# pranoyr/attention-models

Hardware: AMD Instinct MI355X
Metric: ViTVQGAN 256px train-step images/sec (higher is better)
Workload: dtype f32; 1 GPU; BASELINE.json configs[2]: ViTVQGAN dim=256 patch=8 img=256 depth=6+6 h=8 d=64 mlp=2048 (SwiGLU), codebook 8192x32; GAN train step (D phase + G phase, gradient penalty, per_loss_weight=0), Adam, clip 1.0; global_batch=32, batch_per_gpu=32, parallelism=dp1

## Files before the change

attention-models_amd/amk/lib.py:

```python
import ctypes
import os
import re

_HERE = os.path.dirname(os.path.abspath(__file__))
LIB_PATH = os.environ.get("AMK_LIB") or os.path.join(_HERE, "libamk.so")
HEADER_PATH = os.path.normpath(os.path.join(_HERE, "..", "..", "include", "amk.h"))

AMK_OK = 0

_c = ctypes
_P = _c.c_void_p
_I = _c.c_int
_L = _c.c_int64
_F = _c.c_float



class GemmDesc(_c.Structure):
    _fields_ = [("op", _c.c_int32), ("epilogue", _c.c_int32), ("m", _L),
                ("n", _c.c_int32), ("k", _c.c_int32), ("split", _c.c_int32), ("reserved", _c.c_int32),
                ("a", _P), ("a2", _P), ("w", _P), ("w2", _P), ("c", _P), ("c2", _P),
                ("lda", _L), ("lda2", _L), ("ldw", _L), ("ldw2", _L), ("ldc", _L), ("ldc2", _L),
                ("bias", _P), ("bias2", _P), ("resid", _P), ("ldr", _L),
                ("ln_mean", _P), ("ln_rstd", _P), ("ln_gamma", _P), ("ln_beta", _P),
                ("ab", _P), ("ldab", _L), ("gate", _P), ("ldg", _L), ("dbias", _P)]


GEMM_NT, GEMM_NN, GEMM_TN = 0, 1, 2
EPI_BIAS, EPI_RESID, EPI_SWIGLU, EPI_SWIGLU_BWD = 0, 1, 2, 3

SIGNATURES = {
    "amk_version": (_I, []),
    "amk_arch": (_c.c_char_p, []),
    "amk_last_error": (_c.c_char_p, []),
    "amk_attn_fwd": (_I, [_P] * 7 + [_I] * 5 + [_L] * 12 + [_F, _P]),
    "amk_attn_scores_bytes": (_L, [_I, _I, _I, _I]),
    "amk_attn_fwd_keep": (_I, [_P] * 8 + [_I] * 5 + [_L] * 12 + [_F, _P]),
    "amk_attn_fwd_x6_ws_bytes": (_L, [_I, _I, _I]),
    "amk_attn_fwd_x6": (_I, [_P] * 8 + [_I] * 5 + [_L] * 12 + [_F, _P]),
    "amk_attn_bwd_ws_floats": (_L, [_I, _I, _I, _I, _I]),
    "amk_attn_bwd": (_I, [_P] * 12 + [_I] * 5 + [_L] * 24 + [_F, _I, _P]),
    "amk_attn_bwd_kept": (_I, [_P] * 13 + [_I] * 5 + [_L] * 24 + [_F, _I, _P]),
    "amk_vq_num_partials": (_L, [_L]),
    "amk_vq_lookup_fwd": (_I, [_P, _P, _L, _I, _I, _I] + [_P] * 9 + [_P]),
    "amk_vq_lookup_bwd": (_I, [_P] * 7 + [_F, _L, _I, _I, _P, _P, _P]),
    "amk_vq_lookup_bwd_rows": (_I, [_P] * 7 + [_F, _L, _I, _I, _P, _P, _P]),
    "amk_vq_padded_codes": (_I, [_I, _I]),
    "amk_vq_gather": (_I, [_P, _P, _L, _I, _I, _P, _P, _P]),
    "amk_agent_num_chunks": (_I, [_I]),
    "amk_agent_ws_floats": (_L, [_I, _I, _I, _I, _I]),
    "amk_agent_num_chunks_dh": (_I, [_I, _I]),
    "amk_agent_ws_floats_dh": (_L, [_I, _I, _I, _I, _I, _I]),
    "amk_agent_attn_fwd": (_I, [_P] * 10 + [_I] * 5 + [_L] * 12 + [_F, _P]),
    "amk_agent_attn_bwd": (_I, [_P] * 14 + [_I] * 5 + [_L] * 21 + [_F, _P]),
    "amk_agent_conv_grad_reduce": (_I, [_P, _P, _L, _I, _P, _P, _P]),
    "amk_rowsum_num_partials": (_I, [_L]),
    "amk_add_layernorm_fwd": (_I, [_P, _P, _P, _P, _L, _I, _F, _P, _P, _P, _P, _P]),
    "amk_add_layernorm_bwd": (_I, [_P, _P, _P, _P, _P, _P, _L, _I, _P, _P, _P]),
    "amk_colsum": (_I, [_P, _L, _I, _P, _P]),
    "amk_swiglu_fwd": (_I, [_P, _L, _I, _P, _P]),
    "amk_swiglu_bwd": (_I, [_P, _P, _L, _I, _P, _P]),
    "amk_geglu_fwd": (_I, [_P, _L, _I, _P, _P]),
    "amk_geglu_bwd": (_I, [_P, _P, _L, _I, _P, _P]),
    "amk_opt_num_partials": (_I, []),
    "amk_sumsq_partials": (_I, [_P, _L, _P, _P]),
    "amk_adam_flat_step": (_I, [_P] * 4 + [_L, _P, _P, _P, _I] + [_F] * 6 + [_I, _P, _P]),
    "amk_adam_flat_step_shadow": (_I, [_P] * 4 + [_L, _P, _P, _P, _I] + [_F] * 6 + [_I, _P, _P, _P]),
    "amk_gemm_x6_planes_bytes": (_L, [_I, _I]),
    "amk_gemm_x6_split": (_I, [_P, _L, _I, _I, _P, _P]),
    "amk_gemm_x6_nt": (_I, [_P, _L, _P, _P, _P, _L, _I, _I, _I, _P]),
    "amk_gemm_f32_ws_bytes": (_L, [_c.POINTER(GemmDesc)]),
    "amk_gemm_f32": (_I, [_c.POINTER(GemmDesc), _P, _L, _P]),
    "amk_row_stats": (_I, [_P, _L, _I, _F, _P, _P, _P]),
    "amk_attn_bf16_fwd": (_I, [_P] * 7 + [_I] * 5 + [_L] * 12 + [_F, _P]),
    "amk_attn_bf16_bwd_ws_floats": (_L, [_I, _I, _I, _I]),
    "amk_attn_bf16_bwd": (_I, [_P] * 12 + [_I] * 5 + [_L] * 24 + [_F, _P]),
    "amk_swiglu_bf16_fwd": (_I, [_P, _L, _I, _P, _P]),
    "amk_swiglu_bf16_bwd": (_I, [_P, _P, _L, _I, _P, _P]),
    "amk_add_layernorm_mixed_fwd": (_I, [_P, _I, _P, _P, _P, _L, _I, _F, _P, _P, _P, _P, _P]),
    "amk_add_layernorm_mixed_bwd": (_I, [_P, _I, _P, _P, _P, _P, _P, _L, _I, _P, _P, _P, _P]),
    "amk_gemm_bf16": (_I, [_I, _I, _P, _L, _P, _L, _P, _P, _L, _P, _L, _L, _I, _I, _P]),
    "amk_gemm_bf16_swiglu_bwd": (_I, [_P, _L, _P, _L, _P, _L, _P, _L, _L, _I, _I, _P]),
    "amk_gemm_tn_bf16_ws_bytes": (_L, [_L, _I, _I]),
    "amk_gemm_tn_bf16": (_I, [_P, _L, _P, _L, _P, _L, _P, _L, _I, _I, _P, _L, _P]),
    "amk_sample_step": (_I, [_P, _P, _F, _P, _c.c_uint64, _c.c_uint64, _F, _L, _I, _I, _P, _F, _P, _P, _P]),
    "amk_moe_route_ws_ints": (_L, [_L, _I, _I]),
    "amk_moe_route": (_I, [_P, _L, _I, _I] + [_P] * 8),
    "amk_grouped_gemm_nt": (_I, [_P, _L, _I, _P, _P, _P, _P, _L, _I, _I, _I, _P, _P]),
    "amk_grouped_gemm_nn": (_I, [_P, _L, _I, _P, _P, _P, _P, _L, _I, _I, _I, _P, _P]),
    "amk_grouped_gemm_nt_acc": (_I, [_P, _L, _I, _P, _P, _P, _P, _L, _I, _I, _I, _P, _I, _P]),
    "amk_grouped_gemm_nn_acc": (_I, [_P, _L, _I, _P, _P, _P, _P, _L, _I, _I, _I, _P, _I, _P]),
    "amk_grouped_gemm_wgrad": (_I, [_P, _L, _I, _P, _L, _I, _P, _P, _P, _L, _I, _I, _I, _P, _P, _P]),
    "amk_moe_combine": (_I, [_P, _P, _P, _L, _I, _I, _I, _P, _P]),
    "amk_moe_expert_sums": (_I, [_P, _L, _I, _P, _P, _L, _I, _I, _I, _P, _P]),
    "amk_moe_topk": (_I, [_P, _L, _I, _I, _P, _P, _P]),
    "amk_moe_route_distinct": (_I, [_P, _L, _I, _I, _P, _P, _P, _P]),
    "amk_moe_combine_rows": (_I, [_P, _P, _P, _L, _I, _I, _I, _I, _I, _P, _P]),
    "amk_moe_gate_grad_rows": (_I, [_P, _P, _P, _P, _L, _I, _I, _I, _I, _I, _P, _P]),
    "amk_moe_gate_grad": (_I, [_P, _P, _P, _P, _L, _I, _I, _I, _I, _P, _P]),
    "amk_bnact_ws_floats": (_L, [_I, _I, _L]),
    "amk_bnact_fwd": (_I, [_P, _P, _P, _I, _I, _L, _F, _F, _F] + [_P] * 7),
    "amk_bnact_bwd": (_I, [_P] * 6 + [_I, _I, _L, _F] + [_P] * 6),
    "amk_bnact_bwd_bwd": (_I, [_P] * 10 + [_I, _I, _L, _F] + [_P] * 5),
}

_lib = None


def declared_symbols(header_path=HEADER_PATH):
    text = open(header_path).read()
    text = re.sub(r"/\*.*?\*/", "", text, flags=re.S)
    return sorted(set(re.findall(r"\b(amk_[a-z0-9_]+)\s*\(", text)))


def load():
    global _lib
    if _lib is not None:
        return _lib
    if not os.path.exists(LIB_PATH):
        raise RuntimeError(
            f"{LIB_PATH} is missing: build it with `python -c 'import __graft_entry__ as g; g.build()'` "
            "(hipcc --offload-arch=gfx950). amk has no CPU or eager fallback."
        )
    lib = ctypes.CDLL(LIB_PATH)
    for name, (res, args) in SIGNATURES.items():
        fn = getattr(lib, name)
        fn.restype = res
        fn.argtypes = args
    arch = lib.amk_arch().decode()
    if arch != "gfx950":
        raise RuntimeError(f"libamk.so was built for {arch}, expected gfx950")
    _lib = lib
    return lib


def check(rc, what):
    if rc != AMK_OK:
        msg = load().amk_last_error().decode()
        raise RuntimeError(f"{what} failed with code {rc}: {msg}")
```

attention-models_amd/amk/models/discriminator.py:

```python
import contextlib

import torch
import torch.nn as nn
import torch.nn.functional as F
from torch.nn.grad import conv2d_input, conv2d_weight

from .. import ops

_INPUT_GRAD_ONLY = False


@contextlib.contextmanager
def input_grad_only():
    global _INPUT_GRAD_ONLY
    old, _INPUT_GRAD_ONLY = _INPUT_GRAD_ONLY, True
    try:
        yield
    finally:
        _INPUT_GRAD_ONLY = old


def input_grad_only_active():
    return _INPUT_GRAD_ONLY


class _ConvDataGrad(torch.autograd.Function):

    @staticmethod
    def forward(ctx, gy, weight, x_shape, stride, padding):
        ctx.save_for_backward(gy, weight)
        ctx.cfg = (stride, padding)
        return conv2d_input(x_shape, weight, gy, stride=stride, padding=padding)

    @staticmethod
    def backward(ctx, ggx):
        gy, weight = ctx.saved_tensors
        stride, padding = ctx.cfg
        ggx = ggx.contiguous()
        ggy = F.conv2d(ggx, weight, None, stride, padding) if ctx.needs_input_grad[0] else None
        gw = conv2d_weight(ggx, weight.shape, gy, stride=stride, padding=padding) if ctx.needs_input_grad[1] else None
        return ggy, gw, None, None, None


class _Conv(torch.autograd.Function):
    @staticmethod
    def forward(ctx, x, weight, bias, stride, padding):
        ctx.save_for_backward(x, weight)
        ctx.cfg = (stride, padding, bias is not None)
        return F.conv2d(x, weight, bias, stride, padding)

    @staticmethod
    def backward(ctx, gy):
        x, weight = ctx.saved_tensors
        stride, padding, has_bias = ctx.cfg
        gy = gy.contiguous()
        gx = _ConvDataGrad.apply(gy, weight, x.shape, stride, padding) if ctx.needs_input_grad[0] else None
        gw = gb = None
        if not _INPUT_GRAD_ONLY:
            if ctx.needs_input_grad[1]:
                gw = conv2d_weight(x, weight.shape, gy, stride=stride, padding=padding)
            if has_bias and ctx.needs_input_grad[2]:
                gb = gy.sum((0, 2, 3))
        return gx, gw, gb, None, None


class Conv2d(nn.Conv2d):

    def forward(self, x):
        if self.groups != 1 or self.dilation != (1, 1) or self.padding_mode != "zeros" or isinstance(self.padding, str):
            return super().forward(x)
        if torch.is_autocast_enabled():
            if self.in_channels < 8 and x.is_cuda:
                with torch.autocast("cuda", enabled=False):
                    return _Conv.apply(x.float(), self.weight, self.bias, self.stride, self.padding)
            return super().forward(x)
        return _Conv.apply(x, self.weight, self.bias, self.stride, self.padding)


class NLayerDiscriminator(nn.Module):
    def __init__(self, input_nc=3, ndf=64, n_layers=3):
        super().__init__()
        widths = [ndf * min(2 ** i, 8) for i in range(n_layers + 1)]
        layers = [Conv2d(input_nc, widths[0], 4, stride=2, padding=1), nn.LeakyReLU(0.2, True)]
        for i in range(1, n_layers + 1):
            stride = 2 if i < n_layers else 1
            layers += [
                Conv2d(widths[i - 1], widths[i], 4, stride=stride, padding=1, bias=False),
                nn.BatchNorm2d(widths[i]),
                nn.LeakyReLU(0.2, True),
            ]
        layers.append(Conv2d(widths[-1], 1, 4, stride=1, padding=1))
        self.model = nn.Sequential(*layers)

    def forward(self, x):
        if ops.discr_norm_mode() != "amk":
            return self.model(x)
        layers = list(self.model)
        i = 0
        while i < len(layers):
            m = layers[i]
            nxt = layers[i + 1] if i + 1 < len(layers) else None
            if isinstance(m, nn.BatchNorm2d) and isinstance(nxt, nn.LeakyReLU) and ops.bn_leaky_relu_ok(m, x):
                x = ops.bn_leaky_relu(x, m, nxt.negative_slope)
                i += 2
            else:
                x = m(x)
                i += 1
        return x
```

attention-models_amd/amk/ops.py:

```python
import ctypes
import os
import weakref

import torch
from torch.autograd.function import once_differentiable

from . import lib as _lib

_NULL = ctypes.c_void_p(0)


def _ptr(t):
    return ctypes.c_void_p(t.data_ptr()) if t is not None else _NULL


def _stream():
    return ctypes.c_void_p(torch.cuda.current_stream().cuda_stream)


KERNEL_EVENTS = None


class _timed:

    def __init__(self, name):
        self.name = name

    def __enter__(self):
        if KERNEL_EVENTS is not None:
            self.a = torch.cuda.Event(enable_timing=True)
            self.b = torch.cuda.Event(enable_timing=True)
            self.a.record()
        return self

    def __exit__(self, *exc):
        if KERNEL_EVENTS is not None:
            self.b.record()
            KERNEL_EVENTS.setdefault(self.name, []).append((self.a, self.b))
        return False


def kernel_event_summary(events):
    out = {}
    for name, pairs in events.items():
        ms = [a.elapsed_time(b) for a, b in pairs]
        out[name] = (len(ms), sum(ms) / len(ms))
    return out


def _require_device(*tensors):
    for t in tensors:
        if t is None:
            continue
        if not t.is_cuda:
            raise RuntimeError(
                "amk ops run only on MI355X (HIP) tensors; got a CPU tensor. There is no CPU fallback."
            )
        if t.is_floating_point() and t.dtype != torch.float32:
            raise RuntimeError(f"amk kernels compute in fp32; got {t.dtype}")


def _strides4(t):
    return (t.stride(0), t.stride(2), t.stride(1))


def _kernel_view_ok(t):
    return (
        t.stride(3) == 1
        and t.data_ptr() % 16 == 0
        and all(s % 4 == 0 for s in (t.stride(0), t.stride(1), t.stride(2)))
    )


def _as_kernel_view(t):
    if _kernel_view_ok(t):
        return t
    B, H, T, D = t.shape
    return t.permute(0, 2, 1, 3).contiguous().permute(0, 2, 1, 3)


def _new_bthd(B, H, T, D, like):
    return torch.empty((B, T, H, D), device=like.device, dtype=torch.float32).permute(0, 2, 1, 3)


def _mask_u8(mask, shape, what):
    if mask is None:
        return None
    m = mask
    while m.dim() > len(shape) and m.shape[0] == 1:
        m = m[0]
    if m.dim() != len(shape):
        raise RuntimeError(f"{what} must have {len(shape)} dims (got shape {tuple(mask.shape)})")
    m = m.expand(*shape)
    return m.to(torch.uint8).contiguous()


ATTENTION_FORWARD = os.environ.get("AMK_ATTENTION_FORWARD", "f32")

ATTENTION_KEEP_SCORES = os.environ.get("AMK_ATTN_KEEP_SCORES", "1") == "1"
ATTENTION_KEEP_SCORES_MAX_BYTES = 8 << 30
ATTENTION_KEEP_SCORES_BUDGET_BYTES = int(os.environ.get("AMK_ATTN_KEEP_BUDGET", "0")) or None
_kept_scores_bytes = [0]


def _keep_budget(device):
    if ATTENTION_KEEP_SCORES_BUDGET_BYTES is not None:
        return ATTENTION_KEEP_SCORES_BUDGET_BYTES
    return torch.cuda.get_device_properties(device).total_memory // 4


def _release_kept(nbytes):
    _kept_scores_bytes[0] -= nbytes
ATTENTION_BACKWARD_KEYS = int(os.environ.get("AMK_ATTN_BWD_KEYS", "0"))


def _attn_forward(q, k, v, key_mask, causal_mask, scale, keep_scores=False):
    B, H, I, D = q.shape
    J = k.shape[2]
    _require_device(q, k, v, key_mask, causal_mask)
    if k.shape != (B, H, J, D) or v.shape != (B, H, J, D):
        raise RuntimeError(f"attention shapes disagree: q {tuple(q.shape)} k {tuple(k.shape)} v {tuple(v.shape)}")
    q, k, v = _as_kernel_view(q), _as_kernel_view(k), _as_kernel_view(v)
    o = _new_bthd(B, H, I, D, q)
    stats = torch.empty((B, H, I, 2), device=q.device, dtype=torch.float32)
    L = _lib.load()
    x6 = ATTENTION_FORWARD == "bf16x6" and D == 64
    ws = torch.empty((L.amk_attn_fwd_x6_ws_bytes(B, H, J),), device=q.device, dtype=torch.uint8) if x6 else None
    scores = None
    det = DETERMINISTIC_ATTENTION_BACKWARD or torch.are_deterministic_algorithms_enabled()
    keepable = D == 64 or (D == 128 and key_mask is None and causal_mask is None and not det)
    if (keep_scores and keepable and not x6 and ATTENTION_KEEP_SCORES
            and not ATTENTION_BACKWARD_TWO_KERNEL):
        nbytes = L.amk_attn_scores_bytes(B, H, I, J)
        if nbytes <= ATTENTION_KEEP_SCORES_MAX_BYTES and _kept_scores_bytes[0] + nbytes <= _keep_budget(q.device):
            scores = torch.empty((nbytes // 4,), device=q.device, dtype=torch.float32)
            _kept_scores_bytes[0] += nbytes
            weakref.finalize(scores.untyped_storage(), _release_kept, nbytes)
    with _timed("attn_fwd_keep_kernel" if scores is not None else "attn_fwd_kernel"):
        if scores is not None:
            rc = L.amk_attn_fwd_keep(
                _ptr(q), _ptr(k), _ptr(v), _ptr(o), _ptr(stats), _ptr(scores), _ptr(key_mask), _ptr(causal_mask),
                B, H, I, J, D, *_strides4(q), *_strides4(k), *_strides4(v), *_strides4(o),
                float(scale), _stream(),
            )
        elif x6:
            rc = L.amk_attn_fwd_x6(
                _ptr(q), _ptr(k), _ptr(v), _ptr(o), _ptr(stats), _ptr(ws), _ptr(key_mask), _ptr(causal_mask),
                B, H, I, J, D, *_strides4(q), *_strides4(k), *_strides4(v), *_strides4(o),
                float(scale), _stream(),
            )
        else:
            rc = L.amk_attn_fwd(
                _ptr(q), _ptr(k), _ptr(v), _ptr(o), _ptr(stats), _ptr(key_mask), _ptr(causal_mask),
                B, H, I, J, D, *_strides4(q), *_strides4(k), *_strides4(v), *_strides4(o),
                float(scale), _stream(),
            )
    _lib.check(rc, "amk_attn_fwd")
    return q, k, v, o, stats, scores


DETERMINISTIC_ATTENTION_BACKWARD = os.environ.get("AMK_DETERMINISTIC", "0") == "1"
ATTENTION_BACKWARD_TWO_KERNEL = False


def _attn_backward(q, k, v, o, stats, d_o, dq, dk, dv, key_mask, causal_mask, scale, stages=None, delta=None,
                   scores=None):
    if stages is None:
        det = DETERMINISTIC_ATTENTION_BACKWARD or torch.are_deterministic_algorithms_enabled()
        stages = 7 if ATTENTION_BACKWARD_TWO_KERNEL else (73 if det else 9)
    if stages & 8 and not stages & 48:
        stages |= {128: 16, 256: 32}.get(ATTENTION_BACKWARD_KEYS, 0)
    if not stages & 8:
        scores = None
    B, H, I, D = q.shape
    if D != 64 and stages & 64:
        scores = None
    J = k.shape[2]
    d_o = _as_kernel_view(d_o)
    L = _lib.load()
    need = L.amk_attn_bwd_ws_floats(B, H, I, J, int(stages))
    if delta is None or delta.numel() < need:
        delta = torch.empty((need,), device=q.device, dtype=torch.float32)

    def call(st):
        fn, head = (L.amk_attn_bwd_kept, (_ptr(scores),)) if scores is not None and st & 8 else (L.amk_attn_bwd, ())
        rc = fn(
            *head, _ptr(q), _ptr(k), _ptr(v), _ptr(o), _ptr(stats), _ptr(d_o),
            _ptr(dq), _ptr(dk), _ptr(dv), _ptr(delta), _ptr(key_mask), _ptr(causal_mask),
            B, H, I, J, D,
            *_strides4(q), *_strides4(k), *_strides4(v), *_strides4(o), *_strides4(d_o),
            *_strides4(dq), *_strides4(dk), *_strides4(dv),
            float(scale), int(st), _stream(),
        )
        _lib.check(rc, "amk_attn_bwd")

    if KERNEL_EVENTS is not None and (stages & 1) and (stages & ~1):
        call(1)
        name = "attn_bwd_dkdv+dq" if not stages & 8 else ("attn_bwd_fused_kernel(kept scores)" if scores is not None
                                                            else "attn_bwd_fused_kernel")
        with _timed(name):
            call(stages & ~1)
    else:
        call(stages)


_amp_fwd = torch.amp.custom_fwd(device_type="cuda", cast_inputs=torch.float32)
_amp_bwd = torch.amp.custom_bwd(device_type="cuda")


class _AttnCore(torch.autograd.Function):

    @staticmethod
    @_amp_fwd
    def forward(ctx, q, k, v, key_mask, causal_mask, scale):
        need = any(ctx.needs_input_grad[:3])
        q, k, v, o, stats, scores = _attn_forward(q, k, v, key_mask, causal_mask, scale, keep_scores=need)
        ctx.save_for_backward(q, k, v, o, stats, key_mask, causal_mask, scores)
        ctx.scale = scale
        return o

    @staticmethod
    @once_differentiable
    @_amp_bwd
    def backward(ctx, d_o):
        q, k, v, o, stats, key_mask, causal_mask, scores = ctx.saved_tensors
        B, H, I, D = q.shape
        J = k.shape[2]
        dq = _new_bthd(B, H, I, D, q)
        dk = _new_bthd(B, H, J, D, q)
        dv = _new_bthd(B, H, J, D, q)
        _attn_backward(q, k, v, o, stats, d_o, dq, dk, dv, key_mask, causal_mask, ctx.scale, scores=scores)
        return dq, dk, dv, None, None, None


class _AttnFusedKV(torch.autograd.Function):

    @staticmethod
    @_amp_fwd
    def forward(ctx, q2, kv2, key_mask, causal_mask, H, D, scale):
        B, I, _ = q2.shape
        J = kv2.shape[1]
        q2 = q2.contiguous()
        kv2 = kv2.contiguous()
        q = q2.view(B, I, H, D).permute(0, 2, 1, 3)
        kv = kv2.view(B, J, 2, H, D)
        k = kv[:, :, 0].permute(0, 2, 1, 3)
        v = kv[:, :, 1].permute(0, 2, 1, 3)
        need = any(ctx.needs_input_grad[:2])
        q, k, v, o, stats, scores = _attn_forward(q, k, v, key_mask, causal_mask, scale, keep_scores=need)
        ctx.save_for_backward(q, k, v, o, stats, key_mask, causal_mask, scores)
        ctx.scale = scale
        return o.permute(0, 2, 1, 3).reshape(B, I, H * D)

    @staticmethod
    @once_differentiable
    @_amp_bwd
    def backward(ctx, d_o2):
        q, k, v, o, stats, key_mask, causal_mask, scores = ctx.saved_tensors
        B, H, I, D = q.shape
        J = k.shape[2]
        d_o = d_o2.contiguous().view(B, I, H, D).permute(0, 2, 1, 3)
        dq2 = torch.empty((B, I, H * D), device=q.device, dtype=torch.float32)
        dkv2 = torch.empty((B, J, 2 * H * D), device=q.device, dtype=torch.float32)
        dq = dq2.view(B, I, H, D).permute(0, 2, 1, 3)
        dkv = dkv2.view(B, J, 2, H, D)
        dk = dkv[:, :, 0].permute(0, 2, 1, 3)
        dv = dkv[:, :, 1].permute(0, 2, 1, 3)
        _attn_backward(q, k, v, o, stats, d_o, dq, dk, dv, key_mask, causal_mask, ctx.scale, scores=scores)
        return dq2, dkv2, None, None, None, None, None


ATTENTION_BF16 = os.environ.get("AMK_ATTENTION_BF16", "1") == "1"


class _AttnFusedKVBF16(torch.autograd.Function):

    @staticmethod
    @torch.amp.custom_fwd(device_type="cuda")
    def forward(ctx, q2, kv2, H, scale, key_mask=None, causal_mask=None):
        B, I, _ = q2.shape
        J = kv2.shape[1]
        D = 64
        q2 = q2.contiguous()
        kv2 = kv2.contiguous()
        o2 = torch.empty((B, I, H * D), device=q2.device, dtype=torch.bfloat16)
        stats = torch.empty((B, H, I, 2), device=q2.device, dtype=torch.float32)
        L = _lib.load()
        qs, kvs = (I * H * D, H * D, D), (J * 2 * H * D, 2 * H * D, D)
        masked = key_mask is not None or causal_mask is not None
        with _timed("attn_bf16_fwd_kernel<masked>" if masked else "attn_bf16_fwd_kernel"):
            rc = L.amk_attn_bf16_fwd(_ptr(q2), _ptr(kv2), ctypes.c_void_p(kv2.data_ptr() + 2 * H * D), _ptr(o2), _ptr(stats),
                                     _ptr(key_mask), _ptr(causal_mask),
                                     B, H, I, J, D, *qs, *kvs, *kvs, *qs, float(scale), _stream())
        _lib.check(rc, "amk_attn_bf16_fwd")
        ctx.save_for_backward(q2, kv2, o2, stats, key_mask, causal_mask)
        ctx.cfg = (H, scale)
        return o2

    @staticmethod
    @once_differentiable
    @_amp_bwd
    def backward(ctx, d_o2):
        q2, kv2, o2, stats, key_mask, causal_mask = ctx.saved_tensors
        H, scale = ctx.cfg
        B, I, _ = q2.shape
        J = kv2.shape[1]
        D = 64
        d_o2 = d_o2.to(torch.bfloat16).contiguous()
        dq2 = torch.empty_like(q2)
        dkv2 = torch.empty_like(kv2)
        L = _lib.load()
        ws = torch.empty((L.amk_attn_bf16_bwd_ws_floats(B, H, I, J),), device=q2.device, dtype=torch.float32)
        qs, kvs = (I * H * D, H * D, D), (J * 2 * H * D, 2 * H * D, D)
        masked = key_mask is not None or causal_mask is not None
        with _timed("attn_bf16_bwd_kernel<masked>" if masked else "attn_bf16_bwd_kernel"):
            rc = L.amk_attn_bf16_bwd(_ptr(q2), _ptr(kv2), ctypes.c_void_p(kv2.data_ptr() + 2 * H * D), _ptr(o2), _ptr(stats), _ptr(d_o2),
                                     _ptr(dq2), _ptr(dkv2), ctypes.c_void_p(dkv2.data_ptr() + 2 * H * D), _ptr(ws),
                                     _ptr(key_mask), _ptr(causal_mask),
                                     B, H, I, J, D, *qs, *kvs, *kvs, *qs, *qs, *qs, *kvs, *kvs, float(scale), _stream())
        _lib.check(rc, "amk_attn_bf16_bwd")
        return dq2, dkv2, None, None, None, None


def attention(q, k, v, scale, key_mask=None, causal_mask=None):
    B, H, I, D = q.shape
    J = k.shape[2]
    km = _mask_u8(key_mask, (B, J), "context_mask")
    cm = _mask_u8(causal_mask, (I, J), "causal_mask")
    return _AttnCore.apply(q, k, v, km, cm, scale)


def attention_fused_kv(q2, kv2, num_heads, dim_head, scale, key_mask=None, causal_mask=None):
    B, I, _ = q2.shape
    J = kv2.shape[1]
    km = _mask_u8(key_mask, (B, J), "context_mask")
    cm = _mask_u8(causal_mask, (I, J), "causal_mask")
    if ATTENTION_BF16 and q2.dtype == torch.bfloat16 and kv2.dtype == torch.bfloat16 and q2.is_cuda and dim_head == 64:
        return _AttnFusedKVBF16.apply(q2, kv2, num_heads, scale, km, cm)
    return _AttnFusedKV.apply(q2, kv2, km, cm, num_heads, dim_head, scale)


CHECK_INDICES = os.environ.get("AMK_CHECK_INDICES", "1") == "1"


def vq_nsplit(N, K):
    row_blocks = (N + 127) // 128
    nsplit = 1
    while row_blocks * nsplit < 4096 and K // (2 * nsplit) >= 1024:
        nsplit *= 2
    return nsplit


class _VQLookup(torch.autograd.Function):
    @staticmethod
    @_amp_fwd
    def forward(ctx, z, codebook, beta):
        _require_device(z, codebook)
        C = z.shape[-1]
        K = codebook.shape[0]
        zf = z.contiguous().view(-1, C)
        cb = codebook.contiguous()
        N = zf.shape[0]
        dev = z.device
        L = _lib.load()
        nsplit = vq_nsplit(N, K)
        f32 = dict(device=dev, dtype=torch.float32)
        kp = L.amk_vq_padded_codes(K, nsplit)
        en = torch.empty((kp, C), **f32)
        ee = torch.empty((kp,), **f32)
        pmin = torch.empty((N, nsplit), **f32)
        pidx = torch.empty((N, nsplit), device=dev, dtype=torch.int32)
        idx = torch.empty((N,), device=dev, dtype=torch.int64)
        out = torch.empty((N, C), **f32)
        zq = torch.empty((N, C), **f32)
        zn = torch.empty((N, C), **f32)
        partial = torch.empty((L.amk_vq_num_partials(N),), **f32)
        with _timed("vq_lookup_fwd"):
            rc = L.amk_vq_lookup_fwd(
                _ptr(zf), _ptr(cb), N, K, C, nsplit, _ptr(en), _ptr(ee), _ptr(pmin), _ptr(pidx),
                _ptr(idx), _ptr(out), _ptr(zq), _ptr(zn), _ptr(partial), _stream(),
            )
        _lib.check(rc, "amk_vq_lookup_fwd")
        mean_sq = partial.sum() / float(N * C)
        loss = beta * mean_sq + mean_sq
        ctx.save_for_backward(zf, cb, zn, zq, idx)
        ctx.beta = beta
        ctx.z_shape = z.shape
        idx_v = idx.view(z.shape[:-1])
        ctx.mark_non_differentiable(idx_v)
        return out.view(z.shape), idx_v, loss

    @staticmethod
    @once_differentiable
    @_amp_bwd
    def backward(ctx, g_out, _g_idx, g_loss):
        zf, cb, zn, zq, idx = ctx.saved_tensors
        N, C = zf.shape
        K = cb.shape[0]
        if g_out is None:
            g_out = torch.zeros_like(zf)
        if g_loss is None:
            g_loss = torch.zeros((), device=zf.device, dtype=torch.float32)
        g_out = g_out.contiguous().view(N, C)
        g_loss = g_loss.contiguous().to(torch.float32)
        dz = torch.empty_like(zf)
        L = _lib.load()
        if DETERMINISTIC_ATTENTION_BACKWARD or torch.are_deterministic_algorithms_enabled():
            ge = torch.empty_like(zf)
            rc = L.amk_vq_lookup_bwd_rows(
                _ptr(zf), _ptr(cb), _ptr(zn), _ptr(zq), _ptr(idx), _ptr(g_out), _ptr(g_loss),
                float(ctx.beta), N, K, C, _ptr(dz), _ptr(ge), _stream(),
            )
            _lib.check(rc, "amk_vq_lookup_bwd_rows")
            flat_idx = idx.clamp(0, K - 1)
            srt, order = torch.sort(flat_idx, stable=True)
            bounds = torch.searchsorted(srt, torch.arange(K + 1, device=srt.device, dtype=srt.dtype))
            dcb = torch.segment_reduce(ge.index_select(0, order), "sum", offsets=bounds, axis=0, unsafe=True)
            return dz.view(ctx.z_shape), dcb, None
        dcb = torch.empty_like(cb)
        rc = L.amk_vq_lookup_bwd(
            _ptr(zf), _ptr(cb), _ptr(zn), _ptr(zq), _ptr(idx), _ptr(g_out), _ptr(g_loss),
            float(ctx.beta), N, K, C, _ptr(dz), _ptr(dcb), _stream(),
        )
        _lib.check(rc, "amk_vq_lookup_bwd")
        return dz.view(ctx.z_shape), dcb, None


def vq_lookup(z, codebook, beta):
    return _VQLookup.apply(z, codebook, beta)


def vq_gather(indices, codebook):
    _require_device(indices, codebook)
    K, C = codebook.shape
    flat = indices.contiguous().view(-1).to(torch.int64)
    N = flat.shape[0]
    out = torch.empty((N, C), device=codebook.device, dtype=torch.float32)
    bad = torch.zeros((1,), device=codebook.device, dtype=torch.int32)
    L = _lib.load()
    rc = L.amk_vq_gather(_ptr(flat), _ptr(codebook.detach().contiguous()), N, K, C, _ptr(out), _ptr(bad), _stream())
    _lib.check(rc, "amk_vq_gather")
    if CHECK_INDICES and int(bad.item()):
        raise IndexError(f"vq_gather: {int(bad.item())} of {N} indices are outside the codebook [0, {K})")
    return out.view(*indices.shape, C)


_SAMPLE_CALLS = 0


def sample_step(logits, ids, mask=None, null_logits=None, cfg_scale=3.0, tau=1.0, p=0.9, gumbel=None, seed=None,
                unmasked_score=None, generator=None):
    import math

    global _SAMPLE_CALLS
    _require_device(logits, null_logits, gumbel)
    B, T, V = logits.shape
    logits = logits.contiguous()
    null_logits = null_logits.contiguous() if null_logits is not None else None
    gumbel = gumbel.contiguous() if gumbel is not None else None
    if ids.dtype != torch.int64 or not ids.is_contiguous():
        raise RuntimeError("sample_step: ids must be a contiguous int64 tensor (updated in place)")
    m8 = mask.to(torch.uint8).contiguous() if mask is not None else None
    scores = torch.empty((B, T), device=logits.device, dtype=torch.float32)
    if seed is not None:
        _SAMPLE_CALLS += 1
        offset = _SAMPLE_CALLS
    else:
        gen = generator if generator is not None else torch.cuda.default_generators[logits.device.index or 0]
        seed = int(gen.initial_seed()) & ((1 << 63) - 1)
        offset = int(gen.get_offset())
        gen.set_offset(offset + 4 * ((B * T * V + 3) // 4))
    L = _lib.load()
    rc = L.amk_sample_step(_ptr(logits), _ptr(null_logits), float(cfg_scale), _ptr(gumbel), seed, offset, float(tau),
                           B * T, V, math.ceil((1 - p) * V), _ptr(m8), -1.0 if unmasked_score is None else float(unmasked_score),
                           _ptr(ids), _ptr(scores), _stream())
    _lib.check(rc, "amk_sample_step")
    return scores


def _i32(n, dev):
    return torch.empty((n,), device=dev, dtype=torch.int32)


def moe_route(logits2, k):
    _require_device(logits2)
    U, E = logits2.shape
    dev = logits2.device
    ids = torch.empty((U, k), device=dev, dtype=torch.int64)
    gate = torch.empty((U, k), device=dev, dtype=torch.float32)
    L = _lib.load()
    counts, rank = _i32(E, dev), _i32(U * k, dev)
    blockhist = _i32(L.amk_moe_route_ws_ints(U, E, k), dev)
    offsets, perm = _i32(E + 1, dev), _i32(U * k, dev)
    rc = L.amk_moe_route(_ptr(logits2.contiguous()), U, E, k, _ptr(ids), _ptr(gate), _ptr(counts), _ptr(rank),
                         _ptr(blockhist), _ptr(offsets), _ptr(perm), _stream())
    _lib.check(rc, "amk_moe_route")
    return dict(ids=ids, gate=gate, offsets=offsets, perm=perm)


MOE_SUM_IN_GEMM = os.environ.get("AMK_MOE_SUM_IN_GEMM", "0") == "1"


MOE_DENSE_Z = os.environ.get("AMK_MOE_DENSE_Z", "1") != "0"


def _moe_dense_z(width, depth, fan, E):
    return MOE_DENSE_Z and E <= 2 * fan and width >= 256 and width >= 4 * depth and depth % 4 == 0


def _expert_sums(a2, a_div, ids, scale, G, fan, E, d):
    Z = torch.empty((G, E * d), device=a2.device, dtype=torch.float32)
    with _timed(f"moe_expert_sums G{G} fan{fan} E{E} d{d}"):
        rc = _lib.load().amk_moe_expert_sums(_ptr(a2), a2.stride(0), a_div, _ptr(ids), scale, G, fan, E, d, _ptr(Z), _stream())
    _lib.check(rc, "amk_moe_expert_sums")
    return Z


def _moe_sum_in_gemm(width, depth, fan):
    if not MOE_SUM_IN_GEMM or DETERMINISTIC_ATTENTION_BACKWARD or torch.are_deterministic_algorithms_enabled():
        return False
    return fan >= 4 and width >= 128 and depth % 32 == 0


class _RoutedLinear(torch.autograd.Function):

    @staticmethod
    @_amp_fwd
    def forward(ctx, x2, logits2, W, bias, k, x_div, weighted, outer):
        _require_device(x2, logits2, W, bias)
        x2 = x2.contiguous()
        W = W.contiguous()
        U, E = logits2.shape
        N, Kd = W.shape[1], W.shape[2]
        P = U * k
        dev = x2.device
        if x2.shape != (P // x_div, Kd) or U % outer:
            raise RuntimeError(f"routed linear shapes disagree: x {tuple(x2.shape)} U {U} k {k} x_div {x_div} W {tuple(W.shape)}")
        with _timed(f"moe_route U{U} E{E} k{k}"):
            r = moe_route(logits2.detach(), k)
        L = _lib.load()
        G = U // outer
        if not weighted and bias is None and _moe_dense_z(N, Kd, outer * k, E):
            Y = None
            Z = _expert_sums(x2, x_div, r["ids"], _NULL, G, outer * k, E, Kd)
            with _timed(f"dense_z_gemm M{G} N{N} K{E * Kd}"):
                out = Z @ W.permute(0, 2, 1).reshape(E * Kd, N)
        elif not weighted and _moe_sum_in_gemm(N, Kd, outer * k):
            Y = None
            out = torch.zeros((G, N), device=dev, dtype=torch.float32)
            with _timed(f"grouped_nt_acc P{P} N{N} K{Kd}"):
                rc = L.amk_grouped_gemm_nt_acc(_ptr(x2), Kd, x_div, _ptr(W), _ptr(bias), _ptr(r["offsets"]), _ptr(r["perm"]),
                                               P, E, N, Kd, _ptr(out), outer * k, _stream())
            _lib.check(rc, "amk_grouped_gemm_nt_acc")
        else:
            Y = torch.empty((P, N), device=dev, dtype=torch.float32)
            with _timed(f"grouped_nt P{P} N{N} K{Kd}"):
                rc = L.amk_grouped_gemm_nt(_ptr(x2), Kd, x_div, _ptr(W), _ptr(bias), _ptr(r["offsets"]), _ptr(r["perm"]),
                                           P, E, N, Kd, _ptr(Y), _stream())
            _lib.check(rc, "amk_grouped_gemm_nt")
            out = torch.empty((G, N), device=dev, dtype=torch.float32)
            with _timed(f"moe_combine G{G} N{N} x{outer * k}"):
                rc = L.amk_moe_combine(_ptr(Y), _ptr(r["ids"]), _ptr(r["gate"]) if weighted else _NULL, G, outer, k, N,
                                       _ptr(out), _stream())
            _lib.check(rc, "amk_moe_combine")
        ctx.save_for_backward(x2, W, Y, r["ids"], r["gate"], r["offsets"], r["perm"])
        ctx.cfg = (k, x_div, weighted, outer, E, bias is not None)
        ctx.mark_non_differentiable(r["ids"])
        ctx.set_materialize_grads(False)
        return out, r["ids"]

    @staticmethod
    @once_differentiable
    @_amp_bwd
    def backward(ctx, d_out, _d_ids):
        if d_out is None:
            return (None,) * 8
        x2, W, Y, ids, gate, offsets, perm = ctx.saved_tensors
        k, x_div, weighted, outer, E, has_bias = ctx.cfg
        N, Kd = W.shape[1], W.shape[2]
        P = ids.numel()
        U = P // k
        dev = x2.device
        d_out = d_out.contiguous()
        g_div = outer * k
        scale = _ptr(gate) if weighted else _NULL
        L = _lib.load()
        dlogits = None
        if weighted:
            dlogits = torch.empty((U, E), device=dev, dtype=torch.float32)
            rc = L.amk_moe_gate_grad(_ptr(d_out), _ptr(Y), _ptr(ids), _ptr(gate), P, k, E, N, g_div, _ptr(dlogits), _stream())
            _lib.check(rc, "amk_moe_gate_grad")
        if not ctx.needs_input_grad[0]:
            dx = None
        elif _moe_dense_z(Kd, N, x_div, E):
            Z = _expert_sums(d_out, g_div, ids, scale, x2.shape[0], x_div, E, N)
            with _timed(f"dense_z_gemm M{x2.shape[0]} N{Kd} K{E * N}"):
                dx = Z @ W.view(E * N, Kd)
        elif _moe_sum_in_gemm(Kd, N, x_div):
            dx = torch.zeros_like(x2)
            with _timed(f"grouped_nn_acc P{P} N{N} K{Kd}"):
                rc = L.amk_grouped_gemm_nn_acc(_ptr(d_out), N, g_div, _ptr(W), scale, _ptr(offsets), _ptr(perm), P, E, N, Kd,
                                               _ptr(dx), x_div, _stream())
            _lib.check(rc, "amk_grouped_gemm_nn_acc")
        else:
            dxp = torch.empty((P, Kd), device=dev, dtype=torch.float32)
            with _timed(f"grouped_nn P{P} N{N} K{Kd}"):
                rc = L.amk_grouped_gemm_nn(_ptr(d_out), N, g_div, _ptr(W), scale, _ptr(offsets), _ptr(perm), P, E, N, Kd,
                                           _ptr(dxp), _stream())
            _lib.check(rc, "amk_grouped_gemm_nn")
            dx = torch.empty_like(x2)
            rc = L.amk_moe_combine(_ptr(dxp), _ptr(ids), _NULL, x2.shape[0], x_div // k, k, Kd, _ptr(dx), _stream())
            _lib.check(rc, "amk_moe_combine")
        dW = torch.empty_like(W)
        db = torch.empty((E, N), device=dev, dtype=torch.float32) if has_bias else None
        with _timed(f"grouped_wgrad P{P} N{N} K{Kd}"):
            rc = L.amk_grouped_gemm_wgrad(_ptr(d_out), N, g_div, _ptr(x2), Kd, x_div, scale, _ptr(offsets), _ptr(perm),
                                          P, E, N, Kd, _ptr(dW), _ptr(db), _stream())
        _lib.check(rc, "amk_grouped_gemm_wgrad")
        return dx, dlogits, dW, db, None, None, None, None


def routed_linear(x2, logits2, W, bias, k, x_div, weighted=True, outer=1):
    return _RoutedLinear.apply(x2, logits2, W, bias, k, x_div, weighted, outer)


def _topk(logits2, k):
    U, E = logits2.shape
    ids = torch.empty((U, k), device=logits2.device, dtype=torch.int64)
    gate = torch.empty((U, k), device=logits2.device, dtype=torch.float32)
    _lib.check(_lib.load().amk_moe_topk(_ptr(logits2.contiguous()), U, E, k, _ptr(ids), _ptr(gate), _stream()), "amk_moe_topk")
    return ids, gate


def _route_distinct(ids, G, fan, E):
    dev = ids.device
    mask = torch.empty((G,), device=dev, dtype=torch.int64)
    offsets, perm = _i32(E + 1, dev), _i32(G * min(fan, E), dev)
    _lib.check(_lib.load().amk_moe_route_distinct(_ptr(ids), G, fan, E, _ptr(mask), _ptr(offsets), _ptr(perm), _stream()),
               "amk_moe_route_distinct")
    return offsets, perm


def distinct_experts_ok(dim, d, fan, E, *weights):
    return E <= 64 and _moe_dense_z(dim, d, fan, E) and dim % 4 == 0 and all(w.is_cuda for w in weights)


class _SharedRowExperts(torch.autograd.Function):

    @staticmethod
    @_amp_fwd
    def forward(ctx, x2, logits2, W, k, H):
        _require_device(x2, logits2, W)
        x2, W = x2.contiguous(), W.contiguous()
        U, E = logits2.shape
        N, Kd = W.shape[1], W.shape[2]
        G, fan = U // H, H * k
        if x2.shape != (G, Kd) or U % H:
            raise RuntimeError(f"shared-row experts: shapes disagree: x {tuple(x2.shape)} U {U} H {H} W {tuple(W.shape)}")
        L = _lib.load()
        with _timed(f"moe_topk U{U} E{E} k{k} + distinct lists"):
            ids, gate = _topk(logits2.detach(), k)
            offsets, perm = _route_distinct(ids, G, fan, E)
        V = torch.empty((G * E, N), device=x2.device, dtype=torch.float32)
        with _timed(f"grouped_nt P{U * k} N{N} K{Kd} (distinct rows)"):
            _lib.check(L.amk_grouped_gemm_nt(_ptr(x2), Kd, E, _ptr(W), _NULL, _ptr(offsets), _ptr(perm), G * E, E, N, Kd, _ptr(V),
                                             _stream()), "amk_grouped_gemm_nt")
        out = torch.empty((U, N), device=x2.device, dtype=torch.float32)
        _lib.check(L.amk_moe_combine_rows(_ptr(V), _ptr(ids), _ptr(gate), U, 1, k, N, fan, E, _ptr(out), _stream()),
                   "amk_moe_combine_rows")
        ctx.save_for_backward(x2, W, V, ids, gate, offsets, perm)
        ctx.cfg = (k, H)
        ctx.mark_non_differentiable(ids)
        ctx.set_materialize_grads(False)
        return out, ids

    @staticmethod
    @once_differentiable
    @_amp_bwd
    def backward(ctx, d_out, _d_ids):
        if d_out is None:
            return (None,) * 5
        x2, W, V, ids, gate, offsets, perm = ctx.saved_tensors
        k, H = ctx.cfg
        E, N, Kd = W.shape
        G, fan = x2.shape[0], H * k
        U = G * H
        d_out = d_out.contiguous()
        L = _lib.load()
        dlogits = torch.empty((U, E), device=x2.device, dtype=torch.float32)
        _lib.check(L.amk_moe_gate_grad_rows(_ptr(d_out), _ptr(V), _ptr(ids), _ptr(gate), U * k, k, E, N, k, fan, _ptr(dlogits),
                                            _stream()), "amk_moe_gate_grad_rows")
        Z = _expert_sums(d_out, k, ids, _ptr(gate), G, fan, E, N)
        dx = None
        if ctx.needs_input_grad[0]:
            with _timed(f"dense_z_gemm M{G} N{Kd} K{E * N}"):
                dx = Z @ W.view(E * N, Kd)
        dW = torch.empty_like(W)
        with _timed(f"grouped_wgrad P{U * k} N{N} K{Kd} (distinct rows)"):
            _lib.check(L.amk_grouped_gemm_wgrad(_ptr(Z), N, 1, _ptr(x2), Kd, E, _NULL, _ptr(offsets), _ptr(perm), G * E, E, N, Kd,
                                                _ptr(dW), _NULL, _stream()), "amk_grouped_gemm_wgrad")
        return dx, dlogits, dW, None, None


class _SummedExperts(torch.autograd.Function):

    @staticmethod
    @_amp_fwd
    def forward(ctx, a2, logits2, W, k, H):
        _require_device(a2, logits2, W)
        a2, W = a2.contiguous(), W.contiguous()
        U, E = logits2.shape
        N, Kd = W.shape[1], W.shape[2]
        G, fan = U // H, H * k
        if a2.shape != (U, Kd) or U % H:
            raise RuntimeError(f"summed experts: shapes disagree: a {tuple(a2.shape)} U {U} H {H} W {tuple(W.shape)}")
        with _timed(f"moe_topk U{U} E{E} k{k}"):
            ids, _gate = _topk(logits2.detach(), k)
        Z = _expert_sums(a2, k, ids, _NULL, G, fan, E, Kd)
        with _timed(f"dense_z_gemm M{G} N{N} K{E * Kd}"):
            out = Z @ W.permute(0, 2, 1).reshape(E * Kd, N)
        ctx.save_for_backward(W, Z, ids)
        ctx.cfg = (k, H)
        ctx.mark_non_differentiable(ids)
        ctx.set_materialize_grads(False)
        return out, ids

    @staticmethod
    @once_differentiable
    @_amp_bwd
    def backward(ctx, d_out, _d_ids):
        if d_out is None:
            return (None,) * 5
        W, Z, ids = ctx.saved_tensors
        k, H = ctx.cfg
        E, N, Kd = W.shape
        G, fan = Z.shape[0], H * k
        U = G * H
        d_out = d_out.contiguous()
        L = _lib.load()
        offsets, perm = _route_distinct(ids, G, fan, E)
        da = None
        if ctx.needs_input_grad[0]:
            D = torch.empty((G * E, Kd), device=W.device, dtype=torch.float32)
            with _timed(f"grouped_nn P{U * k} N{N} K{Kd} (distinct rows)"):
                _lib.check(L.amk_grouped_gemm_nn(_ptr(d_out), N, E, _ptr(W), _NULL, _ptr(offsets), _ptr(perm), G * E, E, N, Kd, _ptr(D),
                                                 _stream()), "amk_grouped_gemm_nn")
            da = torch.empty((U, Kd), device=W.device, dtype=torch.float32)
            _lib.check(L.amk_moe_combine_rows(_ptr(D), _ptr(ids), _NULL, U, 1, k, Kd, fan, E, _ptr(da), _stream()),
                       "amk_moe_combine_rows")
        dW = torch.empty_like(W)
        with _timed(f"grouped_wgrad P{U * k} N{N} K{Kd} (distinct rows)"):
            _lib.check(L.amk_grouped_gemm_wgrad(_ptr(d_out), N, E, _ptr(Z), Kd, 1, _NULL, _ptr(offsets), _ptr(perm), G * E, E, N, Kd,
                                                _ptr(dW), _NULL, _stream()), "amk_grouped_gemm_wgrad")
        return da, None, dW, None, None


def shared_row_experts(x2, logits2, W, k, H):
    return _SharedRowExperts.apply(x2, logits2, W, k, H)


def summed_experts(a2, logits2, W, k, H):
    return _SummedExperts.apply(a2, logits2, W, k, H)


class _AgentAttn(torch.autograd.Function):

    @staticmethod
    @_amp_fwd
    def forward(ctx, qkv2, conv_w, conv_b, H, D, P, scale):
        _require_device(qkv2, conv_w, conv_b)
        B, T, _ = qkv2.shape
        qkv2 = qkv2.contiguous()
        qkv = qkv2.view(B, T, 3, H, D)
        q, k, v = (qkv[:, :, j].permute(0, 2, 1, 3) for j in range(3))
        dev = qkv2.device
        o = _new_bthd(B, H, T, D, qkv2)
        agents = torch.empty((B, H, P, D), device=dev, dtype=torch.float32)
        vagent = torch.empty_like(agents)
        stats1 = torch.empty((B, H, P, 2), device=dev, dtype=torch.float32)
        cw, cb = conv_w.contiguous(), conv_b.contiguous()
        L = _lib.load()
        ws = torch.empty((max(L.amk_agent_ws_floats_dh(B, H, T, P, D, 0), 1),), device=dev, dtype=torch.float32)
        rc = L.amk_agent_attn_fwd(_ptr(q), _ptr(k), _ptr(v), _ptr(cw), _ptr(cb), _ptr(o), _ptr(agents), _ptr(vagent),
                                  _ptr(stats1), _ptr(ws), B, H, T, D, P, *_strides4(q), *_strides4(k), *_strides4(v), *_strides4(o),
                                  float(scale), _stream())
        _lib.check(rc, "amk_agent_attn_fwd")
        ctx.save_for_backward(qkv2, cw, agents, vagent, stats1)
        ctx.cfg = (H, D, P, scale)
        return o.permute(0, 2, 1, 3).reshape(B, T, H * D)

    @staticmethod
    @once_differentiable
    @_amp_bwd
    def backward(ctx, d_o2):
        qkv2, cw, agents, vagent, stats1 = ctx.saved_tensors
        H, D, P, scale = ctx.cfg
        B, T, _ = qkv2.shape
        dev = qkv2.device
        qkv = qkv2.view(B, T, 3, H, D)
        q, k, v = (qkv[:, :, j].permute(0, 2, 1, 3) for j in range(3))
        d_o = d_o2.contiguous().view(B, T, H, D).permute(0, 2, 1, 3)
        dqkv2 = torch.empty_like(qkv2)
        dqkv = dqkv2.view(B, T, 3, H, D)
        dq, dk, dv = (dqkv[:, :, j].permute(0, 2, 1, 3) for j in range(3))
        L = _lib.load()
        cells = B * H * L.amk_agent_num_chunks_dh(T, D)
        ws = torch.empty((max(L.amk_agent_ws_floats_dh(B, H, T, P, D, 1), 1),), device=dev, dtype=torch.float32)
        dw_part = torch.empty((cells, 9, D), device=dev, dtype=torch.float32)
        db_part = torch.empty((cells, D), device=dev, dtype=torch.float32)
        rc = L.amk_agent_attn_bwd(_ptr(q), _ptr(k), _ptr(v), _ptr(cw), _ptr(d_o), _ptr(agents), _ptr(vagent), _ptr(stats1),
                                  _ptr(dq), _ptr(dk), _ptr(dv), _ptr(ws), _ptr(dw_part), _ptr(db_part),
                                  B, H, T, D, P, *_strides4(q), *_strides4(k), *_strides4(v), *_strides4(d_o),
                                  *_strides4(dq), *_strides4(dk), *_strides4(dv), float(scale), _stream())
        _lib.check(rc, "amk_agent_attn_bwd")
        dconv_w = torch.empty((D, 1, 3, 3), device=dev, dtype=torch.float32)
        dconv_b = torch.empty((D,), device=dev, dtype=torch.float32)
        _lib.check(L.amk_agent_conv_grad_reduce(_ptr(dw_part), _ptr(db_part), cells, D, _ptr(dconv_w), _ptr(dconv_b), _stream()),
                   "amk_agent_conv_grad_reduce")
        return dqkv2, dconv_w, dconv_b, None, None, None, None


def agent_attention(qkv2, conv_w, conv_b, num_heads, dim_head, pool, scale):
    return _AgentAttn.apply(qkv2, conv_w, conv_b, num_heads, dim_head, pool, scale)


class _SwiGLU(torch.autograd.Function):
    FWD, BWD = "amk_swiglu_fwd", "amk_swiglu_bwd"

    @classmethod
    def forward(cls, ctx, ab):
        _require_device(ab)
        H = ab.shape[-1] // 2
        ab2 = ab.contiguous().view(-1, 2 * H)
        M = ab2.shape[0]
        out = torch.empty((M, H), device=ab.device, dtype=torch.float32)
        L = _lib.load()
        _lib.check(getattr(L, cls.FWD)(_ptr(ab2), M, H, _ptr(out), _stream()), cls.FWD)
        ctx.save_for_backward(ab2)
        ctx.shape = ab.shape
        return out.view(*ab.shape[:-1], H)

    @classmethod
    def backward(cls, ctx, d_out):
        (ab2,) = ctx.saved_tensors
        M, H2 = ab2.shape
        d_out = d_out.contiguous().view(M, H2 // 2)
        d_ab = torch.empty_like(ab2)
        L = _lib.load()
        _lib.check(getattr(L, cls.BWD)(_ptr(ab2), _ptr(d_out), M, H2 // 2, _ptr(d_ab), _stream()), cls.BWD)
        return d_ab.view(ctx.shape)


class _GEGLU(_SwiGLU):
    FWD, BWD = "amk_geglu_fwd", "amk_geglu_bwd"


def _f32_outside_autocast(fn, x):
    if torch.is_autocast_enabled():
        with torch.autocast("cuda", enabled=False):
            return fn(x.float())
    return fn(x)


class _SwiGLUBF16(torch.autograd.Function):

    @staticmethod
    def forward(ctx, ab):
        H = ab.shape[-1] // 2
        ab2 = ab.contiguous().view(-1, 2 * H)
        M = ab2.shape[0]
        out = torch.empty((M, H), device=ab.device, dtype=torch.bfloat16)
        _lib.check(_lib.load().amk_swiglu_bf16_fwd(_ptr(ab2), M, H, _ptr(out), _stream()), "amk_swiglu_bf16_fwd")
        ctx.save_for_backward(ab2)
        ctx.shape = ab.shape
        return out.view(*ab.shape[:-1], H)

    @staticmethod
    @once_differentiable
    def backward(ctx, d_out):
        (ab2,) = ctx.saved_tensors
        M, H2 = ab2.shape
        d_out = d_out.to(torch.bfloat16).contiguous().view(M, H2 // 2)
        d_ab = torch.empty_like(ab2)
        _lib.check(_lib.load().amk_swiglu_bf16_bwd(_ptr(ab2), _ptr(d_out), M, H2 // 2, _ptr(d_ab), _stream()), "amk_swiglu_bf16_bwd")
        return d_ab.view(ctx.shape)


MIXED_ELEMENTWISE = os.environ.get("AMK_MIXED_ELEMENTWISE", "1") == "1"


def swiglu(ab):
    if MIXED_ELEMENTWISE and ab.dtype == torch.bfloat16 and ab.is_cuda and ab.shape[-1] % 8 == 0:
        with torch.autocast("cuda", enabled=False):
            return _SwiGLUBF16.apply(ab)
    return _f32_outside_autocast(_SwiGLU.apply, ab)


def geglu(ab):
    return _f32_outside_autocast(_GEGLU.apply, ab)


def _ln_supported(D):
    return 0 < D <= 4096 and D % 4 == 0


def _ln_param_grads(part, params):
    weight, bias = params if params is not None else (None, None)
    (wr, wv), (br, bv) = _claim_late(weight), _claim_late(bias)
    if wv is None and bv is None:
        dgb = part.sum(0)
        return dgb[0], dgb[1]
    dw = db = None
    if wv is not None:
        torch.sum(part[:, 0], dim=0, out=wv)
        wr.wrote(weight)
    else:
        dw = part[:, 0].sum(0)
    if bv is not None:
        torch.sum(part[:, 1], dim=0, out=bv)
        br.wrote(bias)
    else:
        db = part[:, 1].sum(0)
    return dw, db


def _claim_late(p):
    return _claim(p)


def _ln_backward(dy, h, dh_in, weight, mean, rstd, params=None):
    M, D = h.shape
    L = _lib.load()
    dh = torch.empty_like(h)
    part = torch.empty((L.amk_rowsum_num_partials(M), 2, D), device=h.device, dtype=torch.float32)
    _lib.check(L.amk_add_layernorm_bwd(_ptr(dy), _ptr(h), _ptr(dh_in), _ptr(weight), _ptr(mean), _ptr(rstd),
                                       M, D, _ptr(dh), _ptr(part), _stream()), "amk_add_layernorm_bwd")
    dw, db = _ln_param_grads(part, params)
    return dh, dw, db


class _LayerNorm(torch.autograd.Function):
    @staticmethod
    @_amp_fwd
    def forward(ctx, x, weight, bias, eps):
        _require_device(x, weight, bias)
        D = x.shape[-1]
        x2 = x.contiguous().view(-1, D)
        M = x2.shape[0]
        y = torch.empty_like(x2)
        mean = torch.empty((M,), device=x.device, dtype=torch.float32)
        rstd = torch.empty_like(mean)
        w, b = weight.contiguous(), bias.contiguous()
        L = _lib.load()
        _lib.check(L.amk_add_layernorm_fwd(_ptr(x2), _NULL, _ptr(w), _ptr(b), M, D, float(eps), _NULL, _ptr(y),
                                           _ptr(mean), _ptr(rstd), _stream()), "amk_add_layernorm_fwd")
        ctx.save_for_backward(x2, w, mean, rstd)
        ctx.shape = x.shape
        ctx.params = (weight, bias)
        return y.view(x.shape)

    @staticmethod
    @once_differentiable
    @_amp_bwd
    def backward(ctx, dy):
        x2, w, mean, rstd = ctx.saved_tensors
        dx, dw, db = _ln_backward(dy.contiguous().view(x2.shape), x2, None, w, mean, rstd, ctx.params)
        return dx.view(ctx.shape), dw, db, None


class _AddLayerNorm(torch.autograd.Function):

    @staticmethod
    @_amp_fwd
    def forward(ctx, x, res, weight, bias, eps):
        _require_device(x, res, weight, bias)
        D = x.shape[-1]
        x2 = x.contiguous().view(-1, D)
        r2 = res.contiguous().view(-1, D)
        M = x2.shape[0]
        h = torch.empty_like(x2)
        y = torch.empty_like(x2)
        mean = torch.empty((M,), device=x.device, dtype=torch.float32)
        rstd = torch.empty_like(mean)
        w, b = weight.contiguous(), bias.contiguous()
        L = _lib.load()
        _lib.check(L.amk_add_layernorm_fwd(_ptr(x2), _ptr(r2), _ptr(w), _ptr(b), M, D, float(eps), _ptr(h), _ptr(y),
                                           _ptr(mean), _ptr(rstd), _stream()), "amk_add_layernorm_fwd")
        ctx.save_for_backward(h, w, mean, rstd)
        ctx.shape = x.shape
        ctx.params = (weight, bias)
        ctx.set_materialize_grads(False)
        return h.view(x.shape), y.view(x.shape)

    @staticmethod
    @once_differentiable
    @_amp_bwd
    def backward(ctx, dh_in, dy):
        h, w, mean, rstd = ctx.saved_tensors
        if dy is None:
            if dh_in is None:
                return None, None, None, None, None
            return dh_in, dh_in, None, None, None
        dh2 = dh_in.contiguous().view(h.shape) if dh_in is not None else None
        dh, dw, db = _ln_backward(dy.contiguous().view(h.shape), h, dh2, w, mean, rstd, ctx.params)
        dh = dh.view(ctx.shape)
        return dh, dh, dw, db, None


class _AddLayerNormMixed(torch.autograd.Function):

    @staticmethod
    def forward(ctx, x, res, weight, bias, eps):
        _require_device(res, weight, bias)
        D = x.shape[-1]
        x2 = x.contiguous().view(-1, D)
        M = x2.shape[0]
        xb = x2.dtype == torch.bfloat16
        if not xb and x2.dtype != torch.float32:
            raise RuntimeError(f"mixed LayerNorm takes f32 or bf16 inputs, got {x2.dtype}")
        r2 = res.contiguous().view(-1, D) if res is not None else None
        need_h = r2 is not None or xb
        h = torch.empty((M, D), device=x.device, dtype=torch.float32) if need_h else None
        y = torch.empty((M, D), device=x.device, dtype=torch.bfloat16)
        mean = torch.empty((M,), device=x.device, dtype=torch.float32)
        rstd = torch.empty_like(mean)
        w, b = weight.contiguous(), bias.contiguous()
        _lib.check(_lib.load().amk_add_layernorm_mixed_fwd(_ptr(x2), 1 if xb else 0, _ptr(r2), _ptr(w), _ptr(b), M, D, float(eps),
                                                          _ptr(h), _ptr(y), _ptr(mean), _ptr(rstd), _stream()),
                   "amk_add_layernorm_mixed_fwd")
        hs = h if need_h else x2
        ctx.save_for_backward(hs, w, mean, rstd)
        ctx.cfg = (x.shape, xb, res is not None)
        ctx.params = (weight, bias)
        ctx.set_materialize_grads(False)
        return hs.view(x.shape), y.view(x.shape)

    @staticmethod
    @once_differentiable
    def backward(ctx, dh_in, dy):
        h, w, mean, rstd = ctx.saved_tensors
        shape, xb, has_res = ctx.cfg
        M, D = h.shape
        if dy is None:
            if dh_in is None:
                return None, None, None, None, None
            dx = dh_in.to(torch.bfloat16) if xb else dh_in
            return dx, (dh_in if has_res else None), None, None, None
        dyb = dy.dtype == torch.bfloat16
        dy2 = (dy if dyb else dy.float()).contiguous().view(M, D)
        dh2 = dh_in.float().contiguous().view(M, D) if dh_in is not None else None
        L = _lib.load()
        dh = torch.empty((M, D), device=h.device, dtype=torch.float32)
        dh16 = torch.empty((M, D), device=h.device, dtype=torch.bfloat16) if xb else None
        part = torch.empty((L.amk_rowsum_num_partials(M), 2, D), device=h.device, dtype=torch.float32)
        _lib.check(L.amk_add_layernorm_mixed_bwd(_ptr(dy2), 1 if dyb else 0, _ptr(h), _ptr(dh2), _ptr(w), _ptr(mean), _ptr(rstd),
                                                 M, D, _ptr(dh), _ptr(dh16), _ptr(part), _stream()), "amk_add_layernorm_mixed_bwd")
        dw, db = _ln_param_grads(part, ctx.params)
        dhv = dh.view(shape)
        dx = dh16.view(shape) if xb else dhv
        return dx, (dhv if has_res else None), dw, db, None


def _mixed_ln():
    return (MIXED_ELEMENTWISE and torch.is_autocast_enabled() and torch.get_autocast_dtype("cuda") == torch.bfloat16)


def layer_norm(x, weight, bias, eps=1e-5, branch=False):
    if not _ln_supported(x.shape[-1]) or x.numel() == 0 or not x.is_cuda:
        return torch.nn.functional.layer_norm(x, (x.shape[-1],), weight, bias, eps)
    if branch and _mixed_ln():
        with torch.autocast("cuda", enabled=False):
            return _AddLayerNormMixed.apply(x, None, weight, bias, eps)[1]
    return _LayerNorm.apply(x, weight, bias, eps)


def add_layer_norm(x, res, weight, bias, eps=1e-5, branch=False):
    if not _ln_supported(x.shape[-1]) or x.numel() == 0 or not x.is_cuda:
        h = x + res
        return h, torch.nn.functional.layer_norm(h, (h.shape[-1],), weight, bias, eps)
    if branch and _mixed_ln():
        with torch.autocast("cuda", enabled=False):
            return _AddLayerNormMixed.apply(x, res.float(), weight, bias, eps)
    return _AddLayerNorm.apply(x, res, weight, bias, eps)


def colsum(x2):
    M, N = x2.shape
    if N % 4 != 0 or N > 1024:
        return x2.sum(0)
    L = _lib.load()
    part = torch.empty((L.amk_rowsum_num_partials(M), N), device=x2.device, dtype=torch.float32)
    _lib.check(L.amk_colsum(_ptr(x2), M, N, _ptr(part), _stream()), "amk_colsum")
    return part.sum(0)


class _BiasLinear(torch.autograd.Function):

    @staticmethod
    def forward(ctx, x, weight, bias):
        _require_device(x, weight, bias)
        ctx.save_for_backward(x, weight)
        return torch.nn.functional.linear(x, weight, bias)

    @staticmethod
    @once_differentiable
    def backward(ctx, dy):
        x, weight = ctx.saved_tensors
        dy2 = dy.contiguous().view(-1, dy.shape[-1])
        dx = dy2.mm(weight).view(x.shape) if ctx.needs_input_grad[0] else None
        dw = dy2.t().mm(x.reshape(-1, x.shape[-1])) if ctx.needs_input_grad[1] else None
        db = colsum(dy2) if ctx.needs_input_grad[2] else None
        return dx, dw, db


GEMM_MODE = os.environ.get("AMK_GEMM", "f32")


def gemm_x6_nt(a2, b2, bias=None):
    _require_device(a2, b2, bias)
    if a2.stride(1) != 1:
        a2 = a2.contiguous()
    if b2.stride(1) != 1:
        b2 = b2.contiguous()
    M, K = a2.shape
    N = b2.shape[0]
    L = _lib.load()
    planes = torch.empty((L.amk_gemm_x6_planes_bytes(N, K),), device=a2.device, dtype=torch.uint8)
    c = torch.empty((M, N), device=a2.device, dtype=torch.float32)
    with _timed(f"gemm_x6_nt M{M} N{N} K{K}"):
        _lib.check(L.amk_gemm_x6_split(_ptr(b2), b2.stride(0), N, K, _ptr(planes), _stream()), "amk_gemm_x6_split")
        rc = L.amk_gemm_x6_nt(_ptr(a2), a2.stride(0), _ptr(planes), _ptr(bias), _ptr(c), N, M, N, K, _stream())
    _lib.check(rc, "amk_gemm_x6_nt")
    return c


def _x6_ok(x, weight):
    K = weight.shape[1]
    if K % 4 or x.numel() == 0 or x.data_ptr() % 16 or weight.data_ptr() % 16:
        return False
    if x.stride(-1) != 1 or (x.dim() >= 2 and x.stride(-2) % 4):
        return False
    return x.numel() * 4 < 0x7ffffff0 and weight.numel() * 8 < 0x7ffffff0


class _LinearX6(torch.autograd.Function):

    @staticmethod
    def forward(ctx, x, weight, bias):
        _require_device(x, weight, bias)
        x2 = x.reshape(-1, x.shape[-1])
        ctx.save_for_backward(x2, weight)
        ctx.x_shape = x.shape
        ctx.has_bias = bias is not None
        return gemm_x6_nt(x2, weight, bias).view(*x.shape[:-1], weight.shape[0])

    @staticmethod
    @once_differentiable
    def backward(ctx, dy):
        x2, weight = ctx.saved_tensors
        dy2 = dy.contiguous().view(-1, dy.shape[-1])
        dx = dw = db = None
        if ctx.needs_input_grad[0]:
            N = weight.shape[0]
            if N % 4 == 0:
                dx = gemm_x6_nt(dy2, weight.t().contiguous()).view(ctx.x_shape)
            else:
                dx = dy2.mm(weight).view(ctx.x_shape)
        if ctx.needs_input_grad[1]:
            dw = dy2.t().mm(x2)
        if ctx.has_bias and ctx.needs_input_grad[2]:
            db = colsum(dy2)
        return dx, dw, db


DENSE_MODE = os.environ.get("AMK_DENSE", "auto")


DENSE_AUTO_MAX_K = int(os.environ.get("AMK_DENSE_MAX_K", "512"))


def _dense_ok(x, *weights):
    if DENSE_MODE == "lib" or torch.is_autocast_enabled() or not x.is_cuda or x.dtype != torch.float32 or x.numel() == 0:
        return False
    if x.shape[-1] % 4 or x.shape[-1] < 128:
        return False
    if DENSE_MODE == "auto" and x.shape[-1] > DENSE_AUTO_MAX_K:
        return False
    return all(w.dtype == torch.float32 and w.shape[0] % 4 == 0 and w.shape[0] >= 128 and w.is_contiguous() for w in weights)


def _nn_plain(dy2, weight):
    from . import dense

    if DENSE_MODE == "amk":
        return dense.gemm_nn(dy2, weight)
    return dy2.mm(weight)


def _claim(p):
    ref = getattr(p, "_amk_reducer", None) if p is not None else None
    red = ref() if ref is not None else None
    if red is None:
        return None, None
    view = red.claim(p)
    return (red, view) if view is not None else (None, None)


class _DenseLinear(torch.autograd.Function):

    @staticmethod
    def forward(ctx, x, weight, bias):
        from . import dense

        x2 = x.reshape(-1, x.shape[-1])
        ctx.save_for_backward(x2, weight)
        ctx.x_shape = x.shape
        ctx.has_bias = bias is not None
        ctx.params = (weight, bias)
        if DENSE_MODE == "auto" and weight.shape[0] < 512:
            return torch.nn.functional.linear(x, weight, bias)
        return dense.gemm_nt(x2, weight, bias).view(*x.shape[:-1], weight.shape[0])

    @staticmethod
    @once_differentiable
    def backward(ctx, dy):
        from . import dense

        x2, weight = ctx.saved_tensors
        dy2 = dy.reshape(-1, dy.shape[-1])
        dx = dw = db = None
        if ctx.needs_input_grad[0]:
            dx = _nn_plain(dy2, weight).view(ctx.x_shape)
        if ctx.needs_input_grad[1] or (ctx.has_bias and ctx.needs_input_grad[2]):
            want_b = ctx.has_bias and ctx.needs_input_grad[2]
            (wr, wv), (br, bv) = _claim(ctx.params[0]), (_claim(ctx.params[1]) if want_b else (None, None))
            dw, _, db = dense.gemm_tn(dy2, x2, want_bias=want_b, out=wv, bias_out=bv)
            if wv is not None:
                wr.wrote(ctx.params[0])
                dw = None
            if bv is not None:
                br.wrote(ctx.params[1])
                db = None
        return dx, dw, db


def _tn_into(tn, y, x, weight, bias):
    (wr, wv), (br, bv) = _claim(weight), _claim(bias)
    res = tn(y, x, want_bias=bias is not None, out=wv, bias_out=bv)
    dw, db = res[0], res[-1]
    if wv is not None:
        wr.wrote(weight)
        dw = None
    if bv is not None:
        br.wrote(bias)
        db = None
    return dw, db


class _DenseLinear2(torch.autograd.Function):

    @staticmethod
    def forward(ctx, x, wa, wb):
        from . import dense

        x2 = x.reshape(-1, x.shape[-1])
        ctx.save_for_backward(x2, wa, wb)
        ctx.x_shape = x.shape
        ctx.params = (wa, wb)
        a, b = dense.gemm_nt(x2, wa, None, w2=wb)
        return a.view(*x.shape[:-1], wa.shape[0]), b.view(*x.shape[:-1], wb.shape[0])

    @staticmethod
    @once_differentiable
    def backward(ctx, da, db_):
        from . import dense

        x2, wa, wb = ctx.saved_tensors
        da2 = da.reshape(-1, da.shape[-1])
        db2 = db_.reshape(-1, db_.shape[-1])
        dx = dense.gemm_nn(da2, wa, a2=db2, w2=wb).view(ctx.x_shape) if ctx.needs_input_grad[0] else None
        dwa = dwb = None
        if ctx.needs_input_grad[1] or ctx.needs_input_grad[2]:
            (ar, av), (br, bv) = _claim(ctx.params[0]), _claim(ctx.params[1])
            dwa, dwb, _ = dense.gemm_tn(da2, x2, y2=db2, out=av, out2=bv)
            if av is not None:
                ar.wrote(ctx.params[0])
                dwa = None
            if bv is not None:
                br.wrote(ctx.params[1])
                dwb = None
        return dx, dwa, dwb


class _SwiGLUFFN(torch.autograd.Function):

    @staticmethod
    def forward(ctx, x, w12, b12, w3, b3):
        from . import dense

        x2 = x.reshape(-1, x.shape[-1])
        need = any(ctx.needs_input_grad)
        gate, ab = dense.gemm_nt_swiglu(x2, w12, b12, keep_ab=need)
        out = dense.gemm_nt(gate, w3, b3)
        if need:
            ctx.save_for_backward(x2, w12, w3, ab, gate)
        ctx.x_shape = x.shape
        ctx.has_bias = (b12 is not None, b3 is not None)
        ctx.params = (w12, b12, w3, b3)
        return out.view(*x.shape[:-1], w3.shape[0])

    @staticmethod
    @once_differentiable
    def backward(ctx, dout):
        from . import dense

        x2, w12, w3, ab, gate = ctx.saved_tensors
        d2 = dout.reshape(-1, dout.shape[-1])
        d_ab = dense.gemm_nn(d2, w3, swiglu_ab=ab)
        dw3, db3 = _tn_into(dense.gemm_tn, d2, gate, ctx.params[2], ctx.params[3] if ctx.has_bias[1] else None)
        dx = _nn_plain(d_ab, w12).view(ctx.x_shape) if ctx.needs_input_grad[0] else None
        dw12, db12 = _tn_into(dense.gemm_tn, d_ab, x2, ctx.params[0], ctx.params[1] if ctx.has_bias[0] else None)
        return dx, dw12, db12, dw3, db3


MIXED_WGRAD = os.environ.get("AMK_MIXED_WGRAD", "1") == "1"


def _w16(t):
    if t is None:
        return None
    shadow = getattr(t, "_amk_bf16", None)
    if shadow is not None and t._version == t._amk_bf16_version:
        return shadow
    return t.to(torch.bfloat16)


class _LinearMixed(torch.autograd.Function):

    @staticmethod
    def forward(ctx, x, weight, bias):
        x16, w16 = x.to(torch.bfloat16), _w16(weight)
        ctx.save_for_backward(x16, w16)
        ctx.has_bias, ctx.x_dtype = bias is not None, x.dtype
        ctx.params = (weight, bias)
        return torch.nn.functional.linear(x16, w16, _w16(bias))

    @staticmethod
    @once_differentiable
    def backward(ctx, dy):
        from . import dense

        x16, w16 = ctx.saved_tensors
        dy2 = dy.reshape(-1, dy.shape[-1])
        dx = dy2.mm(w16).view(x16.shape).to(ctx.x_dtype) if ctx.needs_input_grad[0] else None
        dw, db = _tn_into(dense.gemm_tn_bf16, dy2, x16.reshape(-1, x16.shape[-1]), ctx.params[0], ctx.params[1])
        return dx, dw, db


def _mixed_linear_ok(x, weight):
    return (MIXED_WGRAD and x.is_cuda and torch.get_autocast_dtype("cuda") == torch.bfloat16 and torch.is_grad_enabled()
            and weight.requires_grad and weight.dtype == torch.float32 and x.dtype in (torch.float32, torch.bfloat16)
            and weight.shape[0] % 8 == 0 and weight.shape[1] % 8 == 0 and x.numel() > 0)


def linear(x, weight, bias=None):
    if torch.is_autocast_enabled():
        if _mixed_linear_ok(x, weight):
            return _LinearMixed.apply(x, weight, bias)
        return torch.nn.functional.linear(x, weight, bias)
    if GEMM_MODE == "bf16x6" and _x6_ok(x, weight):
        return _LinearX6.apply(x, weight, bias)
    if _dense_ok(x, weight):
        return _DenseLinear.apply(x, weight, bias)
    if bias is None:
        return torch.nn.functional.linear(x, weight)
    return _BiasLinear.apply(x, weight, bias)


def linear2(x, wa, wb):
    if GEMM_MODE != "bf16x6" and _dense_ok(x, wa, wb) and wa.shape[0] % 128 == 0:
        return _DenseLinear2.apply(x, wa, wb)
    return linear(x, wa), linear(x, wb)


class _SwiGLUFFNMixed(torch.autograd.Function):

    @staticmethod
    def forward(ctx, x, w12, b12, w3, b3):
        from . import dense

        x16 = x.to(torch.bfloat16).reshape(-1, x.shape[-1])
        w12h, w3h = _w16(w12), _w16(w3)
        g, ab = dense.gemm_nt_swiglu_bf16(x16, w12h, b12)
        y = torch.nn.functional.linear(g, w3h, _w16(b3))
        ctx.save_for_backward(x16, ab, g, w12h, w3h)
        ctx.x_shape, ctx.x_dtype, ctx.bias = x.shape, x.dtype, (b12 is not None, b3 is not None)
        ctx.params = (w12, b12, w3, b3)
        return y.view(*x.shape[:-1], w3.shape[0])

    @staticmethod
    @once_differentiable
    def backward(ctx, dy):
        from . import dense

        x16, ab, g, w12h, w3h = ctx.saved_tensors
        dy2 = dy.reshape(-1, dy.shape[-1])
        dw3, db3 = _tn_into(dense.gemm_tn_bf16, dy2, g, ctx.params[2], ctx.params[3])
        dab = dense.gemm_nn_swiglu_bwd_bf16(dy2, w3h, ab)
        dw12, db12 = _tn_into(dense.gemm_tn_bf16, dab, x16, ctx.params[0], ctx.params[1])
        dx = dab.mm(w12h).view(ctx.x_shape).to(ctx.x_dtype) if ctx.needs_input_grad[0] else None
        return dx, dw12, db12, dw3, db3


def swiglu_ffn(x, w12, b12, w3, b3):
    if torch.is_autocast_enabled() and w12.shape[0] % 16 == 0 and w12.shape[0] >= 1024:
        if _mixed_linear_ok(x, w12) and _mixed_linear_ok(x, w3) and w3.requires_grad:
            with torch.autocast("cuda", enabled=False):
                return _SwiGLUFFNMixed.apply(x, w12, b12, w3, b3)
        no_grad = not torch.is_grad_enabled() or not any(
            t is not None and t.requires_grad for t in (x, w12, b12, w3, b3))
        if (MIXED_WGRAD and no_grad and x.is_cuda and torch.get_autocast_dtype("cuda") == torch.bfloat16
                and w12.dtype == torch.float32 and x.dtype in (torch.float32, torch.bfloat16) and w12.shape[1] % 8 == 0 and x.numel()):
            from . import dense

            g, _ = dense.gemm_nt_swiglu_bf16(x.to(torch.bfloat16).reshape(-1, x.shape[-1]), _w16(w12), b12, keep_ab=False)
            return torch.nn.functional.linear(g, _w16(w3), _w16(b3)).view(*x.shape[:-1], w3.shape[0])
    if GEMM_MODE != "bf16x6" and _dense_ok(x, w12) and w3.shape[1] % 4 == 0 and w3.shape[0] % 4 == 0 and w3.is_contiguous():
        return _SwiGLUFFN.apply(x, w12, b12, w3, b3)
    ab = linear(x, w12, b12)
    if ab.shape[-1] % 8 == 0:
        return linear(swiglu(ab), w3, b3)
    a, b = ab.chunk(2, dim=-1)
    return linear(torch.nn.functional.silu(a) * b, w3, b3)


def discr_norm_mode():
    return os.environ.get("AMK_DISCR_NORM", "amk")


def _bn_aligned(t):
    t = t.contiguous()
    return t if t.data_ptr() % 16 == 0 else t.clone()


def _bn_dims(x):
    N, C, H, W = x.shape
    return N, C, H * W


def _bn_ws(x):
    N, C, HW = _bn_dims(x)
    return torch.empty(int(_lib.load().amk_bnact_ws_floats(N, C, HW)), device=x.device, dtype=torch.float32)


class _BNActGrad(torch.autograd.Function):

    @staticmethod
    def forward(ctx, gz, x, weight, bias, mean, rstd, slope):
        gz = _bn_aligned(gz)
        N, C, HW = _bn_dims(x)
        L = _lib.load()
        gx = torch.empty_like(x)
        sums = torch.empty((2, C), device=x.device, dtype=torch.float32)
        dw = torch.empty_like(weight)
        db = torch.empty_like(bias)
        _lib.check(L.amk_bnact_bwd(_ptr(gz), _ptr(x), _ptr(weight), _ptr(bias), _ptr(mean), _ptr(rstd), N, C, HW,
                                   float(slope), _ptr(gx), _ptr(sums), _ptr(dw), _ptr(db), _ptr(_bn_ws(x)), _stream()),
                   "amk_bnact_bwd")
        ctx.save_for_backward(gz, x, weight, bias, mean, rstd, sums)
        ctx.slope = slope
        ctx.set_materialize_grads(False)
        return gx, dw, db

    @staticmethod
    @once_differentiable
    def backward(ctx, ggx, ggw, ggb):
        gz, x, weight, bias, mean, rstd, sums = ctx.saved_tensors
        if ggx is None and ggw is None and ggb is None:
            return None, None, None, None, None, None, None
        ggx = torch.zeros_like(x) if ggx is None else _bn_aligned(ggx)
        N, C, HW = _bn_dims(x)
        g_gz = torch.empty_like(x)
        g_x = torch.empty_like(x)
        g_w = torch.empty_like(weight) if ctx.needs_input_grad[2] else None
        _lib.check(_lib.load().amk_bnact_bwd_bwd(
            _ptr(ggx), _ptr(ggw.contiguous() if ggw is not None else None), _ptr(ggb.contiguous() if ggb is not None else None),
            _ptr(gz), _ptr(x), _ptr(weight), _ptr(bias), _ptr(mean), _ptr(rstd), _ptr(sums), N, C, HW, float(ctx.slope),
            _ptr(g_gz), _ptr(g_x), _ptr(g_w), _ptr(_bn_ws(x)), _stream()), "amk_bnact_bwd_bwd")
        return (g_gz if ctx.needs_input_grad[0] else None, g_x if ctx.needs_input_grad[1] else None, g_w,
                None, None, None, None)


class _BNAct(torch.autograd.Function):

    @staticmethod
    def forward(ctx, x, weight, bias, running_mean, running_var, eps, momentum, slope):
        N, C, HW = _bn_dims(x)
        L = _lib.load()
        z = torch.empty_like(x)
        mean = torch.empty(C, device=x.device, dtype=torch.float32)
        rstd = torch.empty(C, device=x.device, dtype=torch.float32)
        _lib.check(L.amk_bnact_fwd(_ptr(x), _ptr(weight), _ptr(bias), N, C, HW, float(eps), float(momentum), float(slope),
                                   _ptr(z), _ptr(mean), _ptr(rstd), _ptr(running_mean), _ptr(running_var),
                                   _ptr(_bn_ws(x)), _stream()), "amk_bnact_fwd")
        ctx.save_for_backward(x, weight, bias, mean, rstd)
        ctx.slope = slope
        ctx.set_materialize_grads(False)
        return z

    @staticmethod
    def backward(ctx, gz):
        if gz is None:
            return (None,) * 8
        x, weight, bias, mean, rstd = ctx.saved_tensors
        from .models.discriminator import input_grad_only_active

        gx, dw, db = _BNActGrad.apply(gz, x, weight, bias, mean, rstd, ctx.slope)
        if input_grad_only_active():
            dw = db = None
        return (gx if ctx.needs_input_grad[0] else None, dw if ctx.needs_input_grad[1] else None,
                db if ctx.needs_input_grad[2] else None, None, None, None, None, None)


def bn_leaky_relu_ok(bn, x):
    return (bn.training and bn.track_running_stats and bn.affine and bn.momentum is not None
            and bn.running_mean is not None and x.is_cuda and x.dtype == torch.float32 and x.dim() == 4
            and x.is_contiguous() and x.numel() > 0 and x.shape[0] * x.shape[2] * x.shape[3] > 1
            and not torch.is_autocast_enabled() and bn.weight.dtype == torch.float32)


def bn_leaky_relu(x, bn, slope):
    _require_device(x, bn.weight, bn.bias)
    if bn.num_batches_tracked is not None:
        bn.num_batches_tracked.add_(1)
    return _BNAct.apply(_bn_aligned(x), bn.weight, bn.bias, bn.running_mean, bn.running_var, bn.eps, bn.momentum,
                        float(slope))
```

attention-models_amd/amk/train.py:

```python
import math

import torch
import torch.nn.functional as F

from .dp import GradReducer
from .models.discriminator import input_grad_only
from .optim import FlatAdam


def set_requires_grad(module, flag):
    for p in module.parameters():
        p.requires_grad_(flag)


def hinge_d_loss(fake, real):
    return 0.5 * (F.relu(1.0 - real).mean() + F.relu(1.0 + fake).mean())


def g_nonsaturating_loss(fake):
    return F.softplus(-fake).mean()


def cosine_warmup_lr(step, base_lr, t_initial, warmup_t, warmup_lr_init=1e-6, lr_min=5e-5):
    if step < warmup_t:
        return warmup_lr_init + step * (base_lr - warmup_lr_init) / warmup_t
    t = min(step, t_initial)
    return lr_min + 0.5 * (base_lr - lr_min) * (1.0 + math.cos(math.pi * t / t_initial))


def cosine_with_warmup_factor(step, num_warmup_steps, num_training_steps, num_cycles=0.5):
    if step < num_warmup_steps:
        return float(step) / float(max(1, num_warmup_steps))
    progress = float(step - num_warmup_steps) / float(max(1, num_training_steps - num_warmup_steps))
    return max(0.0, 0.5 * (1.0 + math.cos(math.pi * float(num_cycles) * 2.0 * progress)))


def constant_with_warmup_factor(step, num_warmup_steps):
    if step < num_warmup_steps:
        return float(step) / float(max(1.0, num_warmup_steps))
    return 1.0


class SupervisedTrainStep:

    def __init__(self, model, lr=1e-4, betas=(0.9, 0.999), weight_decay=0.01, no_decay=(), decoupled=True,
                 schedule="cosine_with_warmup", warmup_steps=0, total_steps=1, max_grad_norm=1.0, accum_steps=1,
                 autocast=None, capturable=False, bucket_bytes=32 << 20, fused_optimizer=None, direct_grads=None,
                 communicate_when_alone=False, overlap=True):
        self.model = model
        self.base_lr, self.schedule = float(lr), schedule
        self.warmup_steps, self.total_steps = int(warmup_steps), int(total_steps)
        self.max_grad_norm, self.accum_steps, self.autocast = max_grad_norm, int(accum_steps), autocast
        named = [(n, p) for n, p in model.named_parameters() if p.requires_grad]
        on_gpu = named[0][1].is_cuda
        self.red = GradReducer([p for _, p in named], bucket_bytes, communicate_when_alone=communicate_when_alone,
                               overlap=overlap, direct_grads=on_gpu if direct_grads is None else bool(direct_grads))
        skip = [p for n, p in named if any(frag in n for frag in no_decay)]
        self.fused_optimizer = on_gpu if fused_optimizer is None else bool(fused_optimizer)
        if self.fused_optimizer:
            self.optim = FlatAdam(self.red, lr=lr, betas=betas, weight_decay=weight_decay, decoupled=decoupled,
                                  capturable=capturable, bf16_shadow=autocast == torch.bfloat16, no_decay=skip)
        else:
            ids = {id(p) for p in skip}
            groups = [dict(params=[p for _, p in named if id(p) not in ids], weight_decay=weight_decay),
                      dict(params=skip, weight_decay=0.0)]
            cls = torch.optim.AdamW if decoupled else torch.optim.Adam
            kw = dict(capturable=True) if capturable else {}
            self.optim = cls([g for g in groups if g["params"]], betas=betas,
                             lr=torch.tensor(float(lr), device=named[0][1].device) if capturable else lr, **kw)
        self.red.broadcast_parameters()
        if self.fused_optimizer:
            self.optim.refresh_shadow()
        self.global_step = 0
        self._micro = 0
        self._lr_arg = 0
        self._graph = None
        self._accum_graph = None
        self.last_lr = None

    def _loss(self, *batch):
        raise NotImplementedError

    def lr_factor(self, step):
        if self.schedule == "cosine_with_warmup":
            return cosine_with_warmup_factor(step, self.warmup_steps, self.total_steps)
        if self.schedule == "constant_with_warmup":
            return constant_with_warmup_factor(step, self.warmup_steps)
        if self.schedule in (None, "constant"):
            return 1.0
        raise ValueError(f"unknown schedule {self.schedule!r}")

    def _set_lr(self):
        lr = self.last_lr = self.base_lr * self.lr_factor(self._lr_arg)
        if isinstance(self.optim, FlatAdam):
            self.optim.lr = lr
            return
        for g in self.optim.param_groups:
            if torch.is_tensor(g["lr"]):
                g["lr"].fill_(lr)
            else:
                g["lr"] = lr

    def _amp(self):
        import contextlib

        if self.autocast is None:
            return contextlib.nullcontext()
        dev = "cuda" if self.red.on_gpu else "cpu"
        return torch.autocast(dev, dtype=self.autocast)

    def step_body(self, sync, *batch):
        self.red.begin(sync)
        loss = self._loss(*batch)
        (loss if self.accum_steps == 1 else loss / self.accum_steps).backward()
        self.red.finish()
        if sync:
            if isinstance(self.optim, FlatAdam):
                self.optim.step(max_norm=self.max_grad_norm)
            else:
                if self.max_grad_norm:
                    torch.nn.utils.clip_grad_norm_(self.red.params, self.max_grad_norm)
                self.optim.step()
                self.red.zero_grad()
        return loss.detach()

    def step(self, *batch):
        self._micro += 1
        sync = self._micro % self.accum_steps == 0
        if sync:
            self._set_lr()
        g = self._graph
        if g is not None and sync and self.accum_steps == 1 and len(batch) == len(g.static_inputs) and all(
                a.shape == b.shape for a, b in zip(batch, g.static_inputs)):
            loss = g.replay(*batch)
        else:
            loss = self.step_body(sync, *batch)
        if sync:
            self._lr_arg = self.global_step
        self.global_step += 1
        return loss

    def _tick(self):
        self._micro += 1
        self._set_lr()
        self._lr_arg = self.global_step
        self.global_step += 1

    def capture(self, *batch, warmup=2):
        from .graphs import GraphedStep

        if self.accum_steps != 1:
            raise RuntimeError("capture(): gradient accumulation steps run eagerly")
        if not self.red.alone and not self.red.avg_in_collective:
            raise RuntimeError("capture(): only RCCL (backend 'nccl') collectives can be captured into a HIP graph")
        self._graph = None
        self._graph = GraphedStep(lambda *b: self.step_body(True, *b), list(batch), warmup=warmup, before_each=self._tick)

    def release_graph(self):
        self._graph = None
        self._accum_graph = None

    def _accum_body(self, k):
        n = self.accum_steps

        def body(*xs):
            for i in range(n - 1):
                self.step_body(False, *xs[i * k:(i + 1) * k])
            return self.step_body(True, *xs[(n - 1) * k:])
        return body

    def _tick_accum(self):
        n = self.accum_steps
        self._micro += n
        self._set_lr()
        self._lr_arg = self.global_step + n - 1
        self.global_step += n

    def capture_accumulated(self, micro_batches, warmup=2):
        from .graphs import GraphedStep

        if len(micro_batches) != self.accum_steps:
            raise ValueError(f"capture_accumulated: {len(micro_batches)} micro-batches for accum_steps={self.accum_steps}")
        if not self.red.alone and not self.red.avg_in_collective:
            raise RuntimeError("capture_accumulated(): only RCCL (backend 'nccl') collectives can be captured into a HIP graph")
        k = len(micro_batches[0])
        self._accum_graph = None
        self._accum_graph = GraphedStep(self._accum_body(k), [t for mb in micro_batches for t in mb], warmup=warmup,
                                        before_each=self._tick_accum)

    def step_accumulated(self, micro_batches):
        n = self.accum_steps
        if len(micro_batches) != n or self._micro % n != 0:
            raise ValueError("step_accumulated: pass accum_steps micro-batches, starting on an optimizer-step boundary")
        flat = [t for mb in micro_batches for t in mb]
        self._micro += n
        self._set_lr()
        g = getattr(self, "_accum_graph", None)
        if g is not None and len(flat) == len(g.static_inputs) and all(a.shape == b.shape for a, b in zip(flat, g.static_inputs)):
            loss = g.replay(*flat)
        else:
            loss = self._accum_body(len(micro_batches[0]))(*flat)
        self._lr_arg = self.global_step + n - 1
        self.global_step += n
        return loss

    def save_ckpt(self, path, config=None):
        import torch.distributed as dist

        if dist.is_initialized() and dist.get_rank() != 0:
            return
        torch.save({"step": self.global_step, "config": config,
                    "state_dict": {k: v.detach().cpu() for k, v in self.model.state_dict().items()}}, path)


    def resume_from_checkpoint(self, path):
        ckpt = torch.load(path, map_location="cpu", weights_only=True)
        self.global_step = int(ckpt["step"])
        self.model.load_state_dict(ckpt["state_dict"])
        self.red.broadcast_parameters()
        if self.fused_optimizer:
            self.optim.refresh_shadow()
        return ckpt.get("config")


class ClassifierTrainStep(SupervisedTrainStep):

    def _loss(self, imgs, target):
        with self._amp():
            out = self.model(imgs)
        return F.cross_entropy(out, target)


class MaskedTokenTrainStep(SupervisedTrainStep):

    NO_DECAY = ("bias", "layer_norm.weight", "embeddings.weight")

    def __init__(self, model, weight_decay=0.0, no_decay=NO_DECAY, schedule="constant_with_warmup", **kw):
        super().__init__(model, weight_decay=weight_decay, no_decay=no_decay, schedule=schedule, **kw)

    def _loss(self, *batch):
        with self._amp():
            return self.model(*batch)


class VQGANTrainStep:
    def __init__(self, model, discr, lr=1e-4, betas=(0.9, 0.999), weight_decay=0.0,
                 adv_loss_weight=0.1, logit_laplace_weight=1.0, max_grad_norm=1.0,
                 warmup_steps=50000, decay_steps=100000, gp_lambda=10.0, bucket_bytes=32 << 20,
                 share_forward=False, capturable=False, fused_optimizer=None, autocast=None, communicate_when_alone=False,
                 overlap=True):
        self.model, self.discr = model, discr
        self._autocast = autocast
        self.adv_w, self.laplace_w = adv_loss_weight, logit_laplace_weight
        self.max_grad_norm, self.gp_lambda = max_grad_norm, gp_lambda
        self.base_lr, self.warmup_steps, self.decay_steps = lr, warmup_steps, decay_steps
        fused = next(model.parameters()).is_cuda
        self.g_red = GradReducer(model.parameters(), bucket_bytes, direct_grads=fused, communicate_when_alone=communicate_when_alone,
                                 overlap=overlap)
        self.d_red = GradReducer(discr.parameters(), bucket_bytes, communicate_when_alone=communicate_when_alone, overlap=overlap)
        self.fused_optimizer = fused if fused_optimizer is None else bool(fused_optimizer)
        okw = dict(betas=betas, weight_decay=weight_decay, fused=fused)
        self._graph = None
        self._accum_graph = None
        if self.fused_optimizer:
            self.g_optim = FlatAdam(self.g_red, lr=lr, betas=betas, weight_decay=weight_decay, capturable=capturable,
                                    bf16_shadow=autocast == torch.bfloat16)
            self.d_optim = FlatAdam(self.d_red, lr=lr, betas=betas, weight_decay=weight_decay, capturable=capturable)
        elif capturable:
            dev = next(model.parameters()).device
            okw.update(capturable=True)
            self.g_optim = torch.optim.Adam(model.parameters(), lr=torch.tensor(float(lr), device=dev), **okw)
            self.d_optim = torch.optim.Adam(discr.parameters(), lr=torch.tensor(float(lr), device=dev), **okw)
        else:
            self.g_optim = torch.optim.Adam(model.parameters(), lr=lr, **okw)
            self.d_optim = torch.optim.Adam(discr.parameters(), lr=lr, **okw)
        self.g_red.broadcast_parameters()
        self.d_red.broadcast_parameters()
        if self.fused_optimizer:
            self.g_optim.refresh_shadow()
        self.global_step = 0
        self.share_forward = bool(share_forward)

    @property
    def autocast(self):
        return self._autocast

    @autocast.setter
    def autocast(self, dtype):
        self._autocast = dtype
        if self.fused_optimizer:
            if dtype == torch.bfloat16:
                self.g_optim.enable_shadow()
            else:
                self.g_optim.disable_shadow()

    def _amp(self):
        import contextlib

        if self.autocast is None:
            return contextlib.nullcontext()
        return torch.autocast("cuda", dtype=self.autocast)

    def gradient_penalty(self, real, fake, eta=None):
        if eta is None:
            eta = torch.rand(real.shape[0], 1, 1, 1, device=real.device)
        mixed = (eta * real + (1.0 - eta) * fake).detach().requires_grad_(True)
        pred = self.discr(mixed)
        with input_grad_only():
            (grad,) = torch.autograd.grad(pred, mixed, grad_outputs=torch.ones_like(pred),
                                          create_graph=True, retain_graph=True)
        return ((grad.norm(2, dim=1) - 1.0) ** 2).mean() * self.gp_lambda

    def _set_lr(self):
        lr = cosine_warmup_lr(max(self.global_step - 1, 0), self.base_lr, self.decay_steps, self.warmup_steps)
        for opt in (self.g_optim, self.d_optim):
            if isinstance(opt, FlatAdam):
                opt.lr = lr
                continue
            for g in opt.param_groups:
                if torch.is_tensor(g["lr"]):
                    g["lr"].fill_(lr)
                else:
                    g["lr"] = lr

    def step(self, img, sync=True, accum_steps=1, eta=None):
        self._set_lr()
        if self._graph is not None and sync and accum_steps == 1 and eta is None and img.shape == self._graph.static_inputs[0].shape:
            logs = self._graph.replay(img)
        else:
            logs = self.step_body(img, sync, accum_steps, eta)
        self.global_step += 1
        return logs

    def capture(self, img, warmup=2):
        from .graphs import GraphedStep

        self._check_capturable("capture")
        self._graph = None
        self._graph = GraphedStep(lambda x: self.step_body(x), [img], warmup=warmup, before_each=self._tick)

    def _check_capturable(self, what):
        for red in (self.g_red, self.d_red):
            if not red.alone and not red.avg_in_collective:
                raise RuntimeError(f"VQGANTrainStep.{what}: only RCCL (backend 'nccl') collectives can be captured into a "
                                   "HIP graph; over gloo the data-parallel step runs eagerly")

    def release_graph(self):
        self._graph = None
        self._accum_graph = None

    def capture_accumulated(self, micro_batches, warmup=2):
        from .graphs import GraphedStep

        self._check_capturable("capture_accumulated")
        n = len(micro_batches)

        def body(*xs):
            for x in xs[:-1]:
                self.step_body(x, False, n, None)
            return self.step_body(xs[-1], True, n, None)

        self._accum_graph = None
        self._accum_graph = GraphedStep(body, list(micro_batches), warmup=warmup, before_each=lambda: self._tick(n))

    def _tick(self, n=1):
        self.global_step += n - 1
        self._set_lr()
        self.global_step += 1

    def step_accumulated(self, micro_batches):
        self.global_step += len(micro_batches) - 1
        self._set_lr()
        self.global_step -= len(micro_batches) - 1
        g = getattr(self, "_accum_graph", None)
        if g is not None and len(micro_batches) == len(g.static_inputs) and all(
                a.shape == b.shape for a, b in zip(micro_batches, g.static_inputs)):
            logs = g.replay(*micro_batches)
        else:
            n = len(micro_batches)
            for x in micro_batches[:-1]:
                self.step_body(x, False, n, None)
            logs = self.step_body(micro_batches[-1], True, n, None)
        self.global_step += len(micro_batches)
        return logs

    def _optim_step(self, opt, red, module):
        if isinstance(opt, FlatAdam):
            opt.step(max_norm=self.max_grad_norm)
            return
        if self.max_grad_norm:
            torch.nn.utils.clip_grad_norm_(module.parameters(), self.max_grad_norm)
        opt.step()
        red.zero_grad()

    def d_phase(self, img, sync=True, accum_steps=1, eta=None, rec=None):
        model, discr = self.model, self.discr
        if rec is None:
            set_requires_grad(model, False)
        set_requires_grad(discr, True)
        self.d_red.begin(sync)
        with self._amp():
            if rec is None:
                rec, _ = model(img)
            d_loss = hinge_d_loss(discr(rec), discr(img)) + self.gradient_penalty(img, rec, eta)
        (d_loss if accum_steps == 1 else d_loss / accum_steps).backward()
        self.d_red.finish()
        if sync:
            self._optim_step(self.d_optim, self.d_red, discr)
        return d_loss.detach()

    def g_phase(self, img, sync=True, accum_steps=1, shared=None):
        model, discr = self.model, self.discr
        set_requires_grad(model, True)
        set_requires_grad(discr, False)
        self.g_red.begin(sync)
        with self._amp():
            rec, codebook_loss = shared if shared is not None else model(img)
            l1 = F.l1_loss(rec, img)
            l2 = F.mse_loss(rec, img)
            g_loss = g_nonsaturating_loss(discr(rec))
            loss = codebook_loss + self.adv_w * g_loss + self.laplace_w * l1 + l2
        (loss if accum_steps == 1 else loss / accum_steps).backward()
        self.g_red.finish()
        if sync:
            self._optim_step(self.g_optim, self.g_red, model)
        return dict(g_loss=g_loss.detach(), l1=l1.detach(), l2=l2.detach(),
                    codebook_loss=codebook_loss.detach(), loss=loss.detach())

    def step_body(self, img, sync=True, accum_steps=1, eta=None):
        shared = None
        if self.share_forward:
            set_requires_grad(self.model, True)
            with self._amp():
                shared = self.model(img)
        d_loss = self.d_phase(img, sync, accum_steps, eta, rec=shared[0].detach() if shared is not None else None)
        logs = self.g_phase(img, sync, accum_steps, shared)
        logs["d_loss"] = d_loss
        return logs

    def save_ckpt(self, path, config=None):
        import torch.distributed as dist

        if dist.is_initialized() and dist.get_rank() != 0:
            return
        ckpt = {"step": self.global_step,
                "state_dict": {k: v.detach().cpu() for k, v in self.model.state_dict().items()},
                "config": config}
        torch.save(ckpt, path)

    def resume_from_checkpoint(self, path):
        import pickle

        try:
            ckpt = torch.load(path, map_location="cpu", weights_only=True)
        except pickle.UnpicklingError as e:
            raise RuntimeError(
                f"{path}: not loadable with weights_only=True ({e}). A reference-written checkpoint must have its "
                "'config' entry converted to a plain dict (or dropped) first; only tensors and plain containers "
                "are loaded here.") from e
        self.global_step = int(ckpt["step"])
        self.model.load_state_dict(ckpt["state_dict"])
        self.g_red.broadcast_parameters()
        if self.fused_optimizer:
            self.g_optim.refresh_shadow()
        return ckpt.get("config")
```

attention-models_amd/csrc/discr_norm.hip:

```cpp
#include "amk_common.h"

namespace amk_bn {

constexpr int BLOCK = 256;
constexpr int WAVES = BLOCK / 64;
constexpr int64_t SEG = 4096;

struct Geo {
  int N, C;
  int64_t HW;
  int PP;
  int Q;
  int64_t L;
  int S;
};

static Geo make_geo(int N, int C, int64_t HW) {
  Geo g;
  g.N = N; g.C = C; g.HW = HW;
  if (HW <= SEG) {
    g.PP = (int)(SEG / HW);
    if (g.PP > N) g.PP = N;
    g.Q = 1; g.L = HW;
    g.S = (N + g.PP - 1) / g.PP;
  } else {
    g.PP = 1;
    g.Q = (int)((HW + SEG - 1) / SEG);
    g.L = (((HW + g.Q - 1) / g.Q) + 3) & ~(int64_t)3;
    g.S = N * g.Q;
  }
  return g;
}

struct Seg {
  int p0, p1;
  int64_t e0, e1;
};

__device__ __forceinline__ Seg seg_of(const Geo& g, int s) {
  Seg r;
  if (g.Q == 1) {
    r.p0 = s * g.PP; r.p1 = min(g.N, r.p0 + g.PP);
    r.e0 = 0; r.e1 = g.HW;
  } else {
    r.p0 = s / g.Q; r.p1 = r.p0 + 1;
    r.e0 = min(g.HW, (int64_t)(s % g.Q) * g.L);
    r.e1 = min(g.HW, r.e0 + g.L);
  }
  return r;
}

__device__ __forceinline__ float seg_count(const Geo& g, int s) {
  const Seg r = seg_of(g, s);
  return (float)((int64_t)(r.p1 - r.p0) * (r.e1 - r.e0));
}

template <int W> struct Width { static constexpr int value = W; };

template <int W>
__device__ __forceinline__ void ld(const float* p, float (&v)[W]) {
  if constexpr (W == 4) {
    const float4 t = *reinterpret_cast<const float4*>(p);
    v[0] = t.x; v[1] = t.y; v[2] = t.z; v[3] = t.w;
  } else {
    v[0] = *p;
  }
}

template <int W>
__device__ __forceinline__ void st(float* p, const float (&v)[W]) {
  if constexpr (W == 4) *reinterpret_cast<float4*>(p) = make_float4(v[0], v[1], v[2], v[3]);
  else *p = v[0];
}

template <class F>
__device__ __forceinline__ void seg_walk(const Geo& g, int c, int s, F&& f) {
  const Seg r = seg_of(g, s);
  const int64_t len = r.e1 - r.e0;
  const int t = threadIdx.x;
  for (int p = r.p0; p < r.p1; ++p) {
    const int64_t base = ((int64_t)p * g.C + c) * g.HW + r.e0;
    const int head = (int)min((int64_t)((4 - (base & 3)) & 3), len);
    const int64_t nv = (len - head) >> 2;
    const int tail = (int)(len - head - 4 * nv);
    for (int64_t i = t; i < nv; i += BLOCK) f(Width<4>{}, base + head + 4 * i);
    if (t < head) f(Width<1>{}, base + t);
    else if (t < head + tail) f(Width<1>{}, base + 4 * nv + t);
  }
}

struct Sum {
  template <int K>
  __device__ __forceinline__ void operator()(float (&a)[K], const float (&b)[K]) const {
#pragma unroll
    for (int k = 0; k < K; ++k) a[k] += b[k];
  }
};

struct Chan {
  __device__ __forceinline__ void operator()(float (&a)[3], const float (&b)[3]) const {
    const float n = a[0] + b[0];
    if (b[0] == 0.f) return;
    if (a[0] == 0.f) { a[0] = b[0]; a[1] = b[1]; a[2] = b[2]; return; }
    const float d = b[1] - a[1], f = b[0] / n;
    a[1] += d * f;
    a[2] += b[2] + d * d * a[0] * f;
    a[0] = n;
  }
};

template <int K, class Op>
__device__ __forceinline__ void block_reduce(float (&v)[K], Op op, float* lds) {
  const int lane = threadIdx.x & 63, wave = threadIdx.x >> 6;
#pragma unroll
  for (int o = 32; o >= 1; o >>= 1) {
    float w[K];
#pragma unroll
    for (int k = 0; k < K; ++k) w[k] = __shfl_xor(v[k], o, 64);
    op(v, w);
  }
  if (lane == 0) {
#pragma unroll
    for (int k = 0; k < K; ++k) lds[wave * K + k] = v[k];
  }
  __syncthreads();
#pragma unroll
  for (int k = 0; k < K; ++k) v[k] = lds[k];
#pragma unroll
  for (int w = 1; w < WAVES; ++w) {
    float u[K];
#pragma unroll
    for (int k = 0; k < K; ++k) u[k] = lds[w * K + k];
    op(v, u);
  }
  __syncthreads();
}

template <int K>
__device__ __forceinline__ void fold_sums(const float* __restrict__ part, const Geo& g, int c, float (&v)[K],
                                          float* lds) {
#pragma unroll
  for (int k = 0; k < K; ++k) v[k] = 0.f;
  for (int j = threadIdx.x; j < g.S; j += BLOCK) {
#pragma unroll
    for (int k = 0; k < K; ++k) v[k] += part[((int64_t)c * g.S + j) * K + k];
  }
  block_reduce<K>(v, Sum{}, lds);
}

__global__ __launch_bounds__(BLOCK) void stats_kernel(const float* __restrict__ x, Geo g, float* __restrict__ part) {
  __shared__ float lds[WAVES * 3];
  const int s = blockIdx.x, c = blockIdx.y;
  float v[1] = {0.f};
  seg_walk(g, c, s, [&](auto w, int64_t off) {
    constexpr int W = decltype(w)::value;
    float xv[W];
    ld<W>(x + off, xv);
#pragma unroll
    for (int k = 0; k < W; ++k) v[0] += xv[k];
  });
  block_reduce<1>(v, Sum{}, lds);
  const float cnt = seg_count(g, s);
  const float mean = cnt > 0.f ? v[0] / cnt : 0.f;
  float q[1] = {0.f};
  seg_walk(g, c, s, [&](auto w, int64_t off) {
    constexpr int W = decltype(w)::value;
    float xv[W];
    ld<W>(x + off, xv);
#pragma unroll
    for (int k = 0; k < W; ++k) { const float d = xv[k] - mean; q[0] += d * d; }
  });
  block_reduce<1>(q, Sum{}, lds);
  if (threadIdx.x == 0) {
    part[((int64_t)c * g.S + s) * 2] = mean;
    part[((int64_t)c * g.S + s) * 2 + 1] = q[0];
  }
}

__global__ __launch_bounds__(BLOCK) void fwd_apply_kernel(
    const float* __restrict__ x, const float* __restrict__ gamma, const float* __restrict__ beta, Geo g,
    const float* __restrict__ part, float eps, float momentum, float slope, float* __restrict__ z,
    float* __restrict__ mean_out, float* __restrict__ rstd_out, float* __restrict__ run_mean,
    float* __restrict__ run_var) {
  __shared__ float lds[WAVES * 3];
  const int s = blockIdx.x, c = blockIdx.y;
  float a[3] = {0.f, 0.f, 0.f};
  for (int j = threadIdx.x; j < g.S; j += BLOCK) {
    const float b[3] = {seg_count(g, j), part[((int64_t)c * g.S + j) * 2], part[((int64_t)c * g.S + j) * 2 + 1]};
    Chan{}(a, b);
  }
  block_reduce<3>(a, Chan{}, lds);
  const float n = a[0], mu = a[1], var = a[2] / n;
  const float r = rsqrtf(var + eps);
  const float scale = gamma[c] * r, shift = beta[c] - mu * scale;
  if (s == 0 && threadIdx.x == 0) {
    mean_out[c] = mu;
    rstd_out[c] = r;
    if (run_mean) run_mean[c] = (1.f - momentum) * run_mean[c] + momentum * mu;
    if (run_var) run_var[c] = (1.f - momentum) * run_var[c] + momentum * (a[2] / (n - 1.f));
  }
  seg_walk(g, c, s, [&](auto w, int64_t off) {
    constexpr int W = decltype(w)::value;
    float xv[W];
    ld<W>(x + off, xv);
#pragma unroll
    for (int k = 0; k < W; ++k) {
      const float y = fmaf(xv[k], scale, shift);
      xv[k] = y > 0.f ? y : slope * y;
    }
    st<W>(z + off, xv);
  });
}

struct Chn {
  float mu, r, scale, shift;
};

__device__ __forceinline__ Chn chn(const float* gamma, const float* beta, const float* mean, const float* rstd, int c) {
  Chn h;
  h.mu = mean[c]; h.r = rstd[c];
  h.scale = gamma[c] * h.r;
  h.shift = beta[c] - h.mu * h.scale;
  return h;
}

__global__ __launch_bounds__(BLOCK) void bwd_reduce_kernel(
    const float* __restrict__ gz, const float* __restrict__ x, const float* __restrict__ gamma,
    const float* __restrict__ beta, const float* __restrict__ mean, const float* __restrict__ rstd, Geo g, float slope,
    float* __restrict__ part) {
  __shared__ float lds[WAVES * 3];
  const int s = blockIdx.x, c = blockIdx.y;
  const Chn h = chn(gamma, beta, mean, rstd, c);
  float v[2] = {0.f, 0.f};
  seg_walk(g, c, s, [&](auto w, int64_t off) {
    constexpr int W = decltype(w)::value;
    float xv[W], gv[W];
    ld<W>(x + off, xv);
    ld<W>(gz + off, gv);
#pragma unroll
    for (int k = 0; k < W; ++k) {
      const float gy = fmaf(xv[k], h.scale, h.shift) > 0.f ? gv[k] : slope * gv[k];
      v[0] += gy;
      v[1] += gy * ((xv[k] - h.mu) * h.r);
    }
  });
  block_reduce<2>(v, Sum{}, lds);
  if (threadIdx.x == 0) {
    part[((int64_t)c * g.S + s) * 2] = v[0];
    part[((int64_t)c * g.S + s) * 2 + 1] = v[1];
  }
}

__global__ __launch_bounds__(BLOCK) void bwd_apply_kernel(
    const float* __restrict__ gz, const float* __restrict__ x, const float* __restrict__ gamma,
    const float* __restrict__ beta, const float* __restrict__ mean, const float* __restrict__ rstd, Geo g, float slope,
    const float* __restrict__ part, float* __restrict__ gx, float* __restrict__ sums, float* __restrict__ dgamma,
    float* __restrict__ dbeta) {
  __shared__ float lds[WAVES * 3];
  const int s = blockIdx.x, c = blockIdx.y;
  const Chn h = chn(gamma, beta, mean, rstd, c);
  float v[2];
  fold_sums<2>(part, g, c, v, lds);
  if (s == 0 && threadIdx.x == 0) {
    sums[c] = v[0];
    sums[g.C + c] = v[1];
    if (dbeta) dbeta[c] = v[0];
    if (dgamma) dgamma[c] = v[1];
  }
  const float inv_n = 1.f / (float)((double)g.N * (double)g.HW);
  const float A = v[0] * inv_n, B = v[1] * inv_n;
  seg_walk(g, c, s, [&](auto w, int64_t off) {
    constexpr int W = decltype(w)::value;
    float xv[W], gv[W];
    ld<W>(x + off, xv);
    ld<W>(gz + off, gv);
#pragma unroll
    for (int k = 0; k < W; ++k) {
      const float gy = fmaf(xv[k], h.scale, h.shift) > 0.f ? gv[k] : slope * gv[k];
      const float xh = (xv[k] - h.mu) * h.r;
      xv[k] = h.scale * (gy - A - xh * B);
    }
    st<W>(gx + off, xv);
  });
}

__global__ __launch_bounds__(BLOCK) void bwd_bwd_reduce_kernel(
    const float* __restrict__ ggx, const float* __restrict__ gz, const float* __restrict__ x,
    const float* __restrict__ gamma, const float* __restrict__ beta, const float* __restrict__ mean,
    const float* __restrict__ rstd, Geo g, float slope, float* __restrict__ part) {
  __shared__ float lds[WAVES * 3];
  const int s = blockIdx.x, c = blockIdx.y;
  const Chn h = chn(gamma, beta, mean, rstd, c);
  float v[3] = {0.f, 0.f, 0.f};
  seg_walk(g, c, s, [&](auto w, int64_t off) {
    constexpr int W = decltype(w)::value;
    float xv[W], gv[W], qv[W];
    ld<W>(x + off, xv);
    ld<W>(gz + off, gv);
    ld<W>(ggx + off, qv);
#pragma unroll
    for (int k = 0; k < W; ++k) {
      const float gy = fmaf(xv[k], h.scale, h.shift) > 0.f ? gv[k] : slope * gv[k];
      v[0] += qv[k];
      v[1] += qv[k] * ((xv[k] - h.mu) * h.r);
      v[2] += qv[k] * gy;
    }
  });
  block_reduce<3>(v, Sum{}, lds);
  if (threadIdx.x == 0) {
#pragma unroll
    for (int k = 0; k < 3; ++k) part[((int64_t)c * g.S + s) * 3 + k] = v[k];
  }
}

__global__ __launch_bounds__(BLOCK) void bwd_bwd_apply_kernel(
    const float* __restrict__ ggx, const float* __restrict__ gg_gamma, const float* __restrict__ gg_beta,
    const float* __restrict__ gz, const float* __restrict__ x, const float* __restrict__ gamma,
    const float* __restrict__ beta, const float* __restrict__ mean, const float* __restrict__ rstd,
    const float* __restrict__ sums, Geo g, float slope, const float* __restrict__ part, float* __restrict__ g_gz,
    float* __restrict__ g_x, float* __restrict__ g_gamma) {
  __shared__ float lds[WAVES * 3];
  const int s = blockIdx.x, c = blockIdx.y;
  const Chn h = chn(gamma, beta, mean, rstd, c);
  float v[3];
  fold_sums<3>(part, g, c, v, lds);
  const float n = (float)((double)g.N * (double)g.HW), inv_n = 1.f / n;
  const float A = sums[c] * inv_n, B = sums[g.C + c] * inv_n;
  const float Cc = v[0] * inv_n, D = v[1] * inv_n, E = v[2] * inv_n;
  const float ggg = gg_gamma ? gg_gamma[c] : 0.f, ggb = gg_beta ? gg_beta[c] : 0.f;
  if (s == 0 && threadIdx.x == 0 && g_gamma) g_gamma[c] = n * h.r * (E - A * Cc - B * D);
  const float k1 = E - A * Cc - 3.f * B * D;
  const float gr2 = h.scale * h.r;
  const float gr = ggg * h.r;
  seg_walk(g, c, s, [&](auto w, int64_t off) {
    constexpr int W = decltype(w)::value;
    float xv[W], gv[W], qv[W];
    ld<W>(x + off, xv);
    ld<W>(gz + off, gv);
    ld<W>(ggx + off, qv);
#pragma unroll
    for (int k = 0; k < W; ++k) {
      const bool pos = fmaf(xv[k], h.scale, h.shift) > 0.f;
      const float gy = pos ? gv[k] : slope * gv[k];
      const float xh = (xv[k] - h.mu) * h.r;
      const float q = qv[k] - Cc;
      const float t = h.scale * (q - xh * D) + ggg * xh + ggb;
      gv[k] = pos ? t : slope * t;
      xv[k] = gr * (gy - A - xh * B) - gr2 * (xh * k1 + B * q + D * (gy - A));
    }
    st<W>(g_gz + off, gv);
    st<W>(g_x + off, xv);
  });
}

}

using namespace amk_bn;

static bool a16(const void* p) { return (reinterpret_cast<uintptr_t>(p) & 15) == 0; }

#define AMK_BN_SHAPE(what)                                                                       \
  AMK_CHECK_ARG(N > 0 && C > 0 && HW > 0, what ": non-positive size");                           \
  AMK_CHECK_SUPPORTED(C <= 65535 && (int64_t)N * HW <= ((int64_t)1 << 31),                       \
                      what ": shape N %d C %d HW %lld not supported", N, C, (long long)HW)

extern "C" int64_t amk_bnact_ws_floats(int N, int C, int64_t HW) {
  if (N <= 0 || C <= 0 || HW <= 0) return 0;
  return (int64_t)C * make_geo(N, C, HW).S * 3;
}

extern "C" int amk_bnact_fwd(const float* x, const float* gamma, const float* beta, int N, int C, int64_t HW,
                             float eps, float momentum, float slope, float* z, float* mean, float* rstd,
                             float* running_mean, float* running_var, float* ws, void* stream) {
  AMK_CHECK_ARG(x && gamma && beta && z && mean && rstd && ws, "amk_bnact_fwd: null pointer");
  AMK_BN_SHAPE("amk_bnact_fwd");
  AMK_CHECK_ARG(N * HW > 1, "amk_bnact_fwd: a channel needs more than one value");
  AMK_CHECK_ARG(a16(x) && a16(z), "amk_bnact_fwd: x and z must be 16-byte aligned");
  hipStream_t st = static_cast<hipStream_t>(stream);
  const Geo g = make_geo(N, C, HW);
  const dim3 grid(g.S, C), block(BLOCK);
  hipLaunchKernelGGL(stats_kernel, grid, block, 0, st, x, g, ws);
  hipLaunchKernelGGL(fwd_apply_kernel, grid, block, 0, st, x, gamma, beta, g, ws, eps, momentum, slope, z, mean, rstd,
                     running_mean, running_var);
  AMK_CHECK_LAUNCH("amk_bnact_fwd");
  return AMK_OK;
}

extern "C" int amk_bnact_bwd(const float* gz, const float* x, const float* gamma, const float* beta,
                             const float* mean, const float* rstd, int N, int C, int64_t HW, float slope, float* gx,
                             float* sums, float* dgamma, float* dbeta, float* ws, void* stream) {
  AMK_CHECK_ARG(gz && x && gamma && beta && mean && rstd && gx && sums && ws, "amk_bnact_bwd: null pointer");
  AMK_BN_SHAPE("amk_bnact_bwd");
  AMK_CHECK_ARG(a16(gz) && a16(x) && a16(gx), "amk_bnact_bwd: gz, x and gx must be 16-byte aligned");
  hipStream_t st = static_cast<hipStream_t>(stream);
  const Geo g = make_geo(N, C, HW);
  const dim3 grid(g.S, C), block(BLOCK);
  hipLaunchKernelGGL(bwd_reduce_kernel, grid, block, 0, st, gz, x, gamma, beta, mean, rstd, g, slope, ws);
  hipLaunchKernelGGL(bwd_apply_kernel, grid, block, 0, st, gz, x, gamma, beta, mean, rstd, g, slope, ws, gx, sums,
                     dgamma, dbeta);
  AMK_CHECK_LAUNCH("amk_bnact_bwd");
  return AMK_OK;
}

extern "C" int amk_bnact_bwd_bwd(const float* ggx, const float* gg_gamma, const float* gg_beta, const float* gz,
                                 const float* x, const float* gamma, const float* beta, const float* mean,
                                 const float* rstd, const float* sums, int N, int C, int64_t HW, float slope,
                                 float* g_gz, float* g_x, float* g_gamma, float* ws, void* stream) {
  AMK_CHECK_ARG(ggx && gz && x && gamma && beta && mean && rstd && sums && g_gz && g_x && ws,
                "amk_bnact_bwd_bwd: null pointer");
  AMK_BN_SHAPE("amk_bnact_bwd_bwd");
  AMK_CHECK_ARG(a16(ggx) && a16(gz) && a16(x) && a16(g_gz) && a16(g_x),
                "amk_bnact_bwd_bwd: ggx, gz, x, g_gz and g_x must be 16-byte aligned");
  hipStream_t st = static_cast<hipStream_t>(stream);
  const Geo g = make_geo(N, C, HW);
  const dim3 grid(g.S, C), block(BLOCK);
  hipLaunchKernelGGL(bwd_bwd_reduce_kernel, grid, block, 0, st, ggx, gz, x, gamma, beta, mean, rstd, g, slope, ws);
  hipLaunchKernelGGL(bwd_bwd_apply_kernel, grid, block, 0, st, ggx, gg_gamma, gg_beta, gz, x, gamma, beta, mean, rstd,
                     sums, g, slope, ws, g_gz, g_x, g_gamma);
  AMK_CHECK_LAUNCH("amk_bnact_bwd_bwd");
  return AMK_OK;
}
```

include/amk.h:

```cpp
#ifndef AMK_H_
#define AMK_H_

#include <stdint.h>

#ifdef __cplusplus
extern "C" {
#endif

#define AMK_VERSION 140

enum {
  AMK_OK = 0,
  AMK_EINVAL = -1,
  AMK_EUNSUPPORTED = -2,
  AMK_ELAUNCH = -3
};

int amk_version(void);
const char* amk_arch(void);
const char* amk_last_error(void);

int amk_attn_fwd(const float* q, const float* k, const float* v, float* o, float* stats,
                 const uint8_t* key_mask, const uint8_t* causal_mask,
                 int B, int H, int I, int J, int D,
                 int64_t q_sb, int64_t q_st, int64_t q_sh,
                 int64_t k_sb, int64_t k_st, int64_t k_sh,
                 int64_t v_sb, int64_t v_st, int64_t v_sh,
                 int64_t o_sb, int64_t o_st, int64_t o_sh,
                 float scale, void* stream);

int64_t amk_attn_scores_bytes(int B, int H, int I, int J);
int amk_attn_fwd_keep(const float* q, const float* k, const float* v, float* o, float* stats, float* scores,
                      const uint8_t* key_mask, const uint8_t* causal_mask,
                      int B, int H, int I, int J, int D,
                      int64_t q_sb, int64_t q_st, int64_t q_sh,
                      int64_t k_sb, int64_t k_st, int64_t k_sh,
                      int64_t v_sb, int64_t v_st, int64_t v_sh,
                      int64_t o_sb, int64_t o_st, int64_t o_sh,
                      float scale, void* stream);

int64_t amk_attn_fwd_x6_ws_bytes(int B, int H, int J);
int amk_attn_fwd_x6(const float* q, const float* k, const float* v, float* o, float* stats, void* ws,
                    const uint8_t* key_mask, const uint8_t* causal_mask,
                    int B, int H, int I, int J, int D,
                    int64_t q_sb, int64_t q_st, int64_t q_sh,
                    int64_t k_sb, int64_t k_st, int64_t k_sh,
                    int64_t v_sb, int64_t v_st, int64_t v_sh,
                    int64_t o_sb, int64_t o_st, int64_t o_sh,
                    float scale, void* stream);

#define AMK_ATTN_BWD_DELTA 1
#define AMK_ATTN_BWD_DKDV 2
#define AMK_ATTN_BWD_DQ 4
#define AMK_ATTN_BWD_FUSED 8
#define AMK_ATTN_BWD_ALL 7
#define AMK_ATTN_BWD_FAST 9
#define AMK_ATTN_BWD_KEYS128 16
#define AMK_ATTN_BWD_KEYS256 32
#define AMK_ATTN_BWD_DQ_REPRO 64
#define AMK_ATTN_BWD_FAST_REPRO 73
int64_t amk_attn_bwd_ws_floats(int B, int H, int I, int J, int stages);
int amk_attn_bwd(const float* q, const float* k, const float* v, const float* o,
                 const float* stats, const float* d_o,
                 float* dq, float* dk, float* dv, float* delta_ws,
                 const uint8_t* key_mask, const uint8_t* causal_mask,
                 int B, int H, int I, int J, int D,
                 int64_t q_sb, int64_t q_st, int64_t q_sh,
                 int64_t k_sb, int64_t k_st, int64_t k_sh,
                 int64_t v_sb, int64_t v_st, int64_t v_sh,
                 int64_t o_sb, int64_t o_st, int64_t o_sh,
                 int64_t do_sb, int64_t do_st, int64_t do_sh,
                 int64_t dq_sb, int64_t dq_st, int64_t dq_sh,
                 int64_t dk_sb, int64_t dk_st, int64_t dk_sh,
                 int64_t dv_sb, int64_t dv_st, int64_t dv_sh,
                 float scale, int stages, void* stream);
int amk_attn_bwd_kept(const float* scores, const float* q, const float* k, const float* v, const float* o,
                      const float* stats, const float* d_o,
                      float* dq, float* dk, float* dv, float* delta_ws,
                      const uint8_t* key_mask, const uint8_t* causal_mask,
                      int B, int H, int I, int J, int D,
                      int64_t q_sb, int64_t q_st, int64_t q_sh,
                      int64_t k_sb, int64_t k_st, int64_t k_sh,
                      int64_t v_sb, int64_t v_st, int64_t v_sh,
                      int64_t o_sb, int64_t o_st, int64_t o_sh,
                      int64_t do_sb, int64_t do_st, int64_t do_sh,
                      int64_t dq_sb, int64_t dq_st, int64_t dq_sh,
                      int64_t dk_sb, int64_t dk_st, int64_t dk_sh,
                      int64_t dv_sb, int64_t dv_st, int64_t dv_sh,
                      float scale, int stages, void* stream);

int64_t amk_vq_num_partials(int64_t N);
int amk_vq_padded_codes(int K, int nsplit);
int amk_vq_lookup_fwd(const float* z, const float* codebook, int64_t N, int K, int C, int nsplit,
                      float* en_ws, float* ee_ws, float* pmin_ws, int32_t* pidx_ws,
                      int64_t* idx, float* out, float* zq, float* zn, float* sqerr_partial,
                      void* stream);

int amk_vq_lookup_bwd(const float* z, const float* codebook, const float* zn, const float* zq,
                      const int64_t* idx, const float* g_out, const float* g_loss, float beta,
                      int64_t N, int K, int C, float* dz, float* dcodebook, void* stream);

int amk_vq_lookup_bwd_rows(const float* z, const float* codebook, const float* zn, const float* zq,
                           const int64_t* idx, const float* g_out, const float* g_loss, float beta,
                           int64_t N, int K, int C, float* dz, float* ge_rows, void* stream);

int amk_vq_gather(const int64_t* idx, const float* codebook, int64_t N, int K, int C,
                  float* out, int32_t* bad_count, void* stream);


int64_t amk_moe_route_ws_ints(int64_t U, int E, int k);
int amk_moe_route(const float* logits, int64_t U, int E, int k,
                  int64_t* ids, float* gate, int32_t* counts, int32_t* rank, int32_t* blockhist,
                  int32_t* offsets, int32_t* perm, void* stream);

int amk_grouped_gemm_nt(const float* A, int64_t lda, int a_div, const float* W, const float* bias,
                        const int32_t* offsets, const int32_t* perm, int64_t P, int E, int N, int Kd,
                        float* Y, void* stream);

int amk_grouped_gemm_nn(const float* A, int64_t lda, int a_div, const float* W, const float* scale,
                        const int32_t* offsets, const int32_t* perm, int64_t P, int E, int N, int Kd,
                        float* Y, void* stream);

int amk_grouped_gemm_nt_acc(const float* A, int64_t lda, int a_div, const float* W, const float* bias,
                            const int32_t* offsets, const int32_t* perm, int64_t P, int E, int N, int Kd,
                            float* Y, int y_div, void* stream);
int amk_grouped_gemm_nn_acc(const float* A, int64_t lda, int a_div, const float* W, const float* scale,
                            const int32_t* offsets, const int32_t* perm, int64_t P, int E, int N, int Kd,
                            float* Y, int y_div, void* stream);

int amk_grouped_gemm_wgrad(const float* G, int64_t ldg, int g_div, const float* X, int64_t ldx, int x_div,
                           const float* scale, const int32_t* offsets, const int32_t* perm,
                           int64_t P, int E, int N, int Kd, float* dW, float* dbias, void* stream);

int amk_moe_combine(const float* Y, const int64_t* ids, const float* scale, int64_t G, int outer, int k,
                    int N, float* out, void* stream);

int amk_moe_topk(const float* logits, int64_t U, int E, int k, int64_t* ids, float* gate, void* stream);

int amk_moe_route_distinct(const int64_t* ids, int64_t G, int fan, int E, uint64_t* mask,
                           int32_t* offsets, int32_t* perm, void* stream);

int amk_moe_combine_rows(const float* Y, const int64_t* ids, const float* scale, int64_t G, int outer, int k,
                         int N, int v_div, int E, float* out, void* stream);
int amk_moe_gate_grad_rows(const float* d_out, const float* Y, const int64_t* ids, const float* gate,
                           int64_t P, int k, int E, int N, int g_div, int v_div, float* dlogits, void* stream);

int amk_moe_expert_sums(const float* A, int64_t lda, int a_div, const int64_t* ids, const float* scale,
                        int64_t G, int fan, int E, int d, float* Z, void* stream);

int amk_moe_gate_grad(const float* d_out, const float* Y, const int64_t* ids, const float* gate,
                      int64_t P, int k, int E, int N, int g_div, float* dlogits, void* stream);

int amk_agent_num_chunks(int T);
int64_t amk_agent_ws_floats(int B, int H, int T, int P, int backward);
int amk_agent_num_chunks_dh(int T, int D);
int64_t amk_agent_ws_floats_dh(int B, int H, int T, int P, int D, int backward);

int amk_agent_attn_fwd(const float* q, const float* k, const float* v, const float* conv_w, const float* conv_b,
                       float* o, float* agents, float* vagent, float* stats1, float* ws,
                       int B, int H, int T, int D, int P,
                       int64_t q_sb, int64_t q_st, int64_t q_sh, int64_t k_sb, int64_t k_st, int64_t k_sh,
                       int64_t v_sb, int64_t v_st, int64_t v_sh, int64_t o_sb, int64_t o_st, int64_t o_sh,
                       float scale, void* stream);

int amk_agent_attn_bwd(const float* q, const float* k, const float* v, const float* conv_w, const float* d_o,
                       const float* agents, const float* vagent, const float* stats1,
                       float* dq, float* dk, float* dv, float* ws, float* dconvw_part, float* dconvb_part,
                       int B, int H, int T, int D, int P,
                       int64_t q_sb, int64_t q_st, int64_t q_sh, int64_t k_sb, int64_t k_st, int64_t k_sh,
                       int64_t v_sb, int64_t v_st, int64_t v_sh, int64_t do_sb, int64_t do_st, int64_t do_sh,
                       int64_t dq_sb, int64_t dq_st, int64_t dq_sh, int64_t dk_sb, int64_t dk_st, int64_t dk_sh,
                       int64_t dv_sb, int64_t dv_st, int64_t dv_sh, float scale, void* stream);

int amk_agent_conv_grad_reduce(const float* dconvw_part, const float* dconvb_part, int64_t rows, int D,
                               float* dconvw, float* dconvb, void* stream);

int amk_rowsum_num_partials(int64_t M);
int amk_add_layernorm_fwd(const float* x, const float* res, const float* gamma, const float* beta,
                          int64_t M, int D, float eps, float* h, float* y, float* mean, float* rstd, void* stream);
int amk_add_layernorm_bwd(const float* dy, const float* h, const float* dh_in, const float* gamma,
                          const float* mean, const float* rstd, int64_t M, int D, float* dh, float* dgb_part,
                          void* stream);
int amk_colsum(const float* x, int64_t M, int N, float* part, void* stream);

int amk_swiglu_fwd(const float* ab, int64_t M, int H, float* out, void* stream);
int amk_swiglu_bwd(const float* ab, const float* d_out, int64_t M, int H, float* d_ab, void* stream);

int amk_geglu_fwd(const float* ab, int64_t M, int H, float* out, void* stream);
int amk_geglu_bwd(const float* ab, const float* d_out, int64_t M, int H, float* d_ab, void* stream);

int amk_opt_num_partials(void);
int amk_sumsq_partials(const float* x, int64_t n, float* partials, void* stream);
int amk_adam_flat_step(float* param, float* grad, float* exp_avg, float* exp_avg_sq, int64_t n,
                       const int32_t* seg_param, const float* param_tab,
                       const float* partials, int n_partials,
                       float max_norm, float lr, float beta1, float beta2, float eps, float weight_decay,
                       int decoupled, float* norm_out, void* stream);
int amk_adam_flat_step_shadow(float* param, float* grad, float* exp_avg, float* exp_avg_sq, int64_t n,
                              const int32_t* seg_param, const float* param_tab,
                              const float* partials, int n_partials,
                              float max_norm, float lr, float beta1, float beta2, float eps, float weight_decay,
                              int decoupled, float* norm_out, void* param_bf16, void* stream);

int amk_sample_step(const float* logits, const float* null_logits, float cfg_scale,
                    const float* gumbel, uint64_t seed, uint64_t offset, float tau,
                    int64_t R, int V, int keep, const uint8_t* mask, float unmasked_score,
                    int64_t* ids, float* scores, void* stream);

int64_t amk_gemm_x6_planes_bytes(int N, int K);
int amk_gemm_x6_split(const float* W, int64_t ldw, int N, int K, void* planes, void* stream);
int amk_gemm_x6_nt(const float* A, int64_t lda, const void* w_planes, const float* bias,
                   float* C, int64_t ldc, int M, int N, int K, void* stream);

enum { AMK_GEMM_NT = 0, AMK_GEMM_NN = 1, AMK_GEMM_TN = 2 };
enum { AMK_EPI_BIAS = 0, AMK_EPI_RESID = 1, AMK_EPI_SWIGLU = 2, AMK_EPI_SWIGLU_BWD = 3 };
typedef struct amk_gemm_desc {
  int32_t op, epilogue;
  int64_t m;
  int32_t n, k, split, reserved;
  const float *a, *a2, *w, *w2;
  float *c, *c2;
  int64_t lda, lda2, ldw, ldw2, ldc, ldc2;
  const float *bias, *bias2, *resid;
  int64_t ldr;
  const float *ln_mean, *ln_rstd, *ln_gamma, *ln_beta;
  const float* ab;
  int64_t ldab;
  float* gate;
  int64_t ldg;
  float* dbias;
} amk_gemm_desc;
int64_t amk_gemm_f32_ws_bytes(const amk_gemm_desc* d);
int amk_gemm_f32(const amk_gemm_desc* d, void* workspace, int64_t ws_bytes, void* stream);
int amk_row_stats(const float* x, int64_t M, int D, float eps, float* mean, float* rstd, void* stream);

int amk_attn_bf16_fwd(const void* q, const void* k, const void* v, void* o, float* stats,
                      const uint8_t* key_mask, const uint8_t* causal_mask,
                      int B, int H, int I, int J, int D,
                      int64_t q_sb, int64_t q_st, int64_t q_sh, int64_t k_sb, int64_t k_st, int64_t k_sh,
                      int64_t v_sb, int64_t v_st, int64_t v_sh, int64_t o_sb, int64_t o_st, int64_t o_sh,
                      float scale, void* stream);
int64_t amk_attn_bf16_bwd_ws_floats(int B, int H, int I, int J);
int amk_attn_bf16_bwd(const void* q, const void* k, const void* v, const void* o, const float* stats, const void* d_o,
                      void* dq, void* dk, void* dv, float* ws,
                      const uint8_t* key_mask, const uint8_t* causal_mask,
                      int B, int H, int I, int J, int D,
                      int64_t q_sb, int64_t q_st, int64_t q_sh, int64_t k_sb, int64_t k_st, int64_t k_sh,
                      int64_t v_sb, int64_t v_st, int64_t v_sh, int64_t o_sb, int64_t o_st, int64_t o_sh,
                      int64_t do_sb, int64_t do_st, int64_t do_sh, int64_t dq_sb, int64_t dq_st, int64_t dq_sh,
                      int64_t dk_sb, int64_t dk_st, int64_t dk_sh, int64_t dv_sb, int64_t dv_st, int64_t dv_sh,
                      float scale, void* stream);

int amk_swiglu_bf16_fwd(const void* ab, int64_t M, int H, void* out, void* stream);
int amk_swiglu_bf16_bwd(const void* ab, const void* d_out, int64_t M, int H, void* d_ab, void* stream);
int amk_add_layernorm_mixed_fwd(const void* x, int x_is_bf16, const float* res, const float* gamma, const float* beta,
                                int64_t M, int D, float eps, float* h, void* y_bf16, float* mean, float* rstd, void* stream);
int amk_add_layernorm_mixed_bwd(const void* dy, int dy_is_bf16, const float* h, const float* dh_in, const float* gamma,
                                const float* mean, const float* rstd, int64_t M, int D, float* dh, void* dh_bf16,
                                float* dgb_part, void* stream);

int64_t amk_gemm_tn_bf16_ws_bytes(int64_t M, int N, int K);
int amk_gemm_tn_bf16(const void* y, int64_t ldy, const void* x, int64_t ldx, float* c, int64_t ldc, float* dbias,
                     int64_t M, int N, int K, void* workspace, int64_t ws_bytes, void* stream);

int amk_gemm_bf16(int op, int epi, const void* a, int64_t lda, const void* w, int64_t ldw, const float* bias,
                  void* c, int64_t ldc, void* g, int64_t ldg, int64_t M, int N, int K, void* stream);

int amk_gemm_bf16_swiglu_bwd(const void* dy, int64_t lddy, const void* w3, int64_t ldw, const void* ab, int64_t ldab,
                             void* dab, int64_t lddab, int64_t M, int H, int K, void* stream);

int64_t amk_bnact_ws_floats(int N, int C, int64_t HW);
int amk_bnact_fwd(const float* x, const float* gamma, const float* beta, int N, int C, int64_t HW, float eps,
                  float momentum, float slope, float* z, float* mean, float* rstd, float* running_mean,
                  float* running_var, float* ws, void* stream);
int amk_bnact_bwd(const float* gz, const float* x, const float* gamma, const float* beta, const float* mean,
                  const float* rstd, int N, int C, int64_t HW, float slope, float* gx, float* sums, float* dgamma,
                  float* dbeta, float* ws, void* stream);
int amk_bnact_bwd_bwd(const float* ggx, const float* gg_gamma, const float* gg_beta, const float* gz, const float* x,
                      const float* gamma, const float* beta, const float* mean, const float* rstd, const float* sums,
                      int N, int C, int64_t HW, float slope, float* g_gz, float* g_x, float* g_gamma, float* ws,
                      void* stream);

#ifdef __cplusplus
}
#endif
#endif
```

Before: 307.0 images/s.

## Add channels-last discriminator head conv kernels, NHWC BN-act kernels, and skip leaf input grads

Adds custom HIP kernels for the discriminator's final 4x4 single-output-channel conv (forward, data grad, weight grad) that operate on channels-last inputs. It also adds NHWC variants of the fused BatchNorm+LeakyReLU forward, backward and double-backward kernels, and threads a layout flag through the custom conv autograd functions. By default only the head conv is routed to channels-last, replacing MIOpen calls for this thin conv across the gradient-penalty double-backward. During the D-phase backward, the input gradient of leaf inputs is skipped. The layout conversions this introduces add copies and could offset the kernel savings.

```diff
diff --git a/attention-models_amd/amk/lib.py b/attention-models_amd/amk/lib.py
--- a/attention-models_amd/amk/lib.py
+++ b/attention-models_amd/amk/lib.py
@@ -102,6 +102,14 @@
     "amk_bnact_fwd": (_I, [_P, _P, _P, _I, _I, _L, _F, _F, _F] + [_P] * 7),
     "amk_bnact_bwd": (_I, [_P] * 6 + [_I, _I, _L, _F] + [_P] * 6),
     "amk_bnact_bwd_bwd": (_I, [_P] * 10 + [_I, _I, _L, _F] + [_P] * 5),
+    "amk_bnact_nhwc_ws_floats": (_L, [_I, _I, _L]),
+    "amk_bnact_nhwc_fwd": (_I, [_P, _P, _P, _I, _I, _L, _F, _F, _F] + [_P] * 7),
+    "amk_bnact_nhwc_bwd": (_I, [_P] * 6 + [_I, _I, _L, _F] + [_P] * 6),
+    "amk_bnact_nhwc_bwd_bwd": (_I, [_P] * 10 + [_I, _I, _L, _F] + [_P] * 5),
+    "amk_conv_c1_ws_floats": (_L, [_I, _I, _I, _I]),
+    "amk_conv_c1_fwd": (_I, [_P, _P, _P, _I, _I, _I, _I, _P, _P, _P]),
+    "amk_conv_c1_bwd_data": (_I, [_P, _P, _I, _I, _I, _I, _P, _P]),
+    "amk_conv_c1_wgrad": (_I, [_P, _P, _I, _I, _I, _I, _P, _P, _P, _P]),
 }
 
 _lib = None
diff --git a/attention-models_amd/amk/models/discriminator.py b/attention-models_amd/amk/models/discriminator.py
--- a/attention-models_amd/amk/models/discriminator.py
+++ b/attention-models_amd/amk/models/discriminator.py
@@ -1,4 +1,5 @@
 import contextlib
+import os
 
 import torch
 import torch.nn as nn
@@ -8,6 +9,12 @@
 from .. import ops
 
 _INPUT_GRAD_ONLY = False
+_SKIP_LEAF_INPUT_GRAD = False
+_CL = torch.channels_last
+
+
+def discr_layout():
+    return os.environ.get("AMK_DISCR_LAYOUT", "head")
 
 
 @contextlib.contextmanager
@@ -24,44 +31,84 @@
     return _INPUT_GRAD_ONLY
 
 
+@contextlib.contextmanager
+def skip_leaf_input_grad():
+    global _SKIP_LEAF_INPUT_GRAD
+    old, _SKIP_LEAF_INPUT_GRAD = _SKIP_LEAF_INPUT_GRAD, True
+    try:
+        yield
+    finally:
+        _SKIP_LEAF_INPUT_GRAD = old
+
+
+def _as(t, nhwc):
+    return t.contiguous(memory_format=_CL) if nhwc else t.contiguous()
+
+
+def _head_ok(x_shape, weight, stride, padding):
+    return (tuple(weight.shape[2:]) == (4, 4) and weight.shape[0] == 1 and tuple(stride) == (1, 1)
+            and tuple(padding) == (1, 1) and ops.conv_c1_ok(x_shape))
+
+
 class _ConvDataGrad(torch.autograd.Function):
 
     @staticmethod
-    def forward(ctx, gy, weight, x_shape, stride, padding):
-        ctx.save_for_backward(gy, weight)
-        ctx.cfg = (stride, padding)
-        return conv2d_input(x_shape, weight, gy, stride=stride, padding=padding)
+    def forward(ctx, gy, weight, w_img, x_shape, stride, padding, nhwc):
+        gy = _as(gy, nhwc)
+        ctx.save_for_backward(gy, weight, w_img)
+        ctx.cfg = (stride, padding, nhwc, tuple(x_shape))
+        if nhwc and _head_ok(x_shape, weight, stride, padding):
+            return ops.conv_c1_bwd_data(gy, w_img, x_shape)
+        return _as(conv2d_input(x_shape, w_img, gy, stride=stride, padding=padding), nhwc)
 
     @staticmethod
     def backward(ctx, ggx):
-        gy, weight = ctx.saved_tensors
-        stride, padding = ctx.cfg
-        ggx = ggx.contiguous()
-        ggy = F.conv2d(ggx, weight, None, stride, padding) if ctx.needs_input_grad[0] else None
-        gw = conv2d_weight(ggx, weight.shape, gy, stride=stride, padding=padding) if ctx.needs_input_grad[1] else None
-        return ggy, gw, None, None, None
+        gy, weight, w_img = ctx.saved_tensors
+        stride, padding, nhwc, x_shape = ctx.cfg
+        ggx = _as(ggx, nhwc)
+        head = nhwc and _head_ok(x_shape, weight, stride, padding)
+        ggy = gw = None
+        if ctx.needs_input_grad[0]:
+            ggy = ops.conv_c1_fwd(ggx, w_img, None) if head else _as(F.conv2d(ggx, w_img, None, stride, padding), nhwc)
+        if ctx.needs_input_grad[1]:
+            gw = (ops.conv_c1_wgrad(ggx, gy, False)[0] if head
+                  else conv2d_weight(ggx, weight.shape, gy, stride=stride, padding=padding))
+        return ggy, gw, None, None, None, None, None
 
 
 class _Conv(torch.autograd.Function):
+
     @staticmethod
-    def forward(ctx, x, weight, bias, stride, padding):
-        ctx.save_for_backward(x, weight)
-        ctx.cfg = (stride, padding, bias is not None)
-        return F.conv2d(x, weight, bias, stride, padding)
+    def forward(ctx, x, weight, bias, stride, padding, nhwc):
+        ctx.x_leaf = x.is_leaf
+        if nhwc:
+            x = x.contiguous(memory_format=_CL)
+        w_img = weight.contiguous(memory_format=_CL) if nhwc else weight
+        ctx.save_for_backward(x, weight, w_img)
+        ctx.cfg = (stride, padding, bias is not None, nhwc)
+        if nhwc and _head_ok(x.shape, weight, stride, padding):
+            return ops.conv_c1_fwd(x, w_img, bias)
+        return _as(F.conv2d(x, w_img, bias, stride, padding), nhwc) if nhwc else F.conv2d(x, weight, bias, stride, padding)
 
     @staticmethod
     def backward(ctx, gy):
-        x, weight = ctx.saved_tensors
-        stride, padding, has_bias = ctx.cfg
-        gy = gy.contiguous()
-        gx = _ConvDataGrad.apply(gy, weight, x.shape, stride, padding) if ctx.needs_input_grad[0] else None
-        gw = gb = None
+        x, weight, w_img = ctx.saved_tensors
+        stride, padding, has_bias, nhwc = ctx.cfg
+        gy = _as(gy, nhwc)
+        gx = gw = gb = None
+        if ctx.needs_input_grad[0] and not (_SKIP_LEAF_INPUT_GRAD and ctx.x_leaf):
+            gx = _ConvDataGrad.apply(gy, weight, w_img, x.shape, stride, padding, nhwc)
         if not _INPUT_GRAD_ONLY:
-            if ctx.needs_input_grad[1]:
-                gw = conv2d_weight(x, weight.shape, gy, stride=stride, padding=padding)
-            if has_bias and ctx.needs_input_grad[2]:
-                gb = gy.sum((0, 2, 3))
-        return gx, gw, gb, None, None
+            want_b = has_bias and ctx.needs_input_grad[2]
+            if nhwc and _head_ok(x.shape, weight, stride, padding) and (ctx.needs_input_grad[1] or want_b):
+                gw, gb = ops.conv_c1_wgrad(x, gy, want_b)
+                gw = gw if ctx.needs_input_grad[1] else None
+            else:
+                if ctx.needs_input_grad[1]:
+                    gw = conv2d_weight(x, weight.shape, gy, stride=stride, padding=padding)
+                if want_b:
+                    gb = gy.sum((0, 2, 3))
+        return gx, gw, gb, None, None, None
 
 
 class Conv2d(nn.Conv2d):
@@ -72,9 +119,15 @@
         if torch.is_autocast_enabled():
             if self.in_channels < 8 and x.is_cuda:
                 with torch.autocast("cuda", enabled=False):
-                    return _Conv.apply(x.float(), self.weight, self.bias, self.stride, self.padding)
+                    return _Conv.apply(x.float(), self.weight, self.bias, self.stride, self.padding, False)
             return super().forward(x)
-        return _Conv.apply(x, self.weight, self.bias, self.stride, self.padding)
+        layout = discr_layout()
+        if layout == "nhwc":
+            os.environ.setdefault("PYTORCH_MIOPEN_SUGGEST_NHWC", "1")
+        nhwc = (self.training and x.is_cuda and x.dtype == torch.float32 and x.dim() == 4
+                and self.weight.dtype == torch.float32 and ops.discr_norm_mode() == "amk"
+                and (layout == "nhwc" or (layout == "head" and _head_ok(x.shape, self.weight, self.stride, self.padding))))
+        return _Conv.apply(x, self.weight, self.bias, self.stride, self.padding, nhwc)
 
 
 class NLayerDiscriminator(nn.Module):
diff --git a/attention-models_amd/amk/ops.py b/attention-models_amd/amk/ops.py
--- a/attention-models_amd/amk/ops.py
+++ b/attention-models_amd/amk/ops.py
@@ -1438,9 +1438,14 @@
     return os.environ.get("AMK_DISCR_NORM", "amk")
 
 
-def _bn_aligned(t):
-    t = t.contiguous()
-    return t if t.data_ptr() % 16 == 0 else t.clone()
+def _bn_nhwc(x):
+    return (x.dim() == 4 and x.shape[1] % 4 == 0 and not x.is_contiguous()
+            and x.is_contiguous(memory_format=torch.channels_last))
+
+
+def _bn_aligned(t, nhwc=False):
+    t = t.contiguous(memory_format=torch.channels_last if nhwc else torch.contiguous_format)
+    return t if t.data_ptr() % 16 == 0 else t.clone(memory_format=torch.preserve_format)
 
 
 def _bn_dims(x):
@@ -1448,25 +1453,29 @@
     return N, C, H * W
 
 
-def _bn_ws(x):
+def _bn_fn(name, nhwc):
+    return getattr(_lib.load(), ("amk_bnact_nhwc_" if nhwc else "amk_bnact_") + name)
+
+
+def _bn_ws(x, nhwc=False):
     N, C, HW = _bn_dims(x)
-    return torch.empty(int(_lib.load().amk_bnact_ws_floats(N, C, HW)), device=x.device, dtype=torch.float32)
+    return torch.empty(int(_bn_fn("ws_floats", nhwc)(N, C, HW)), device=x.device, dtype=torch.float32)
 
 
 class _BNActGrad(torch.autograd.Function):
 
     @staticmethod
     def forward(ctx, gz, x, weight, bias, mean, rstd, slope):
-        gz = _bn_aligned(gz)
+        nhwc = _bn_nhwc(x)
+        gz = _bn_aligned(gz, nhwc)
         N, C, HW = _bn_dims(x)
-        L = _lib.load()
         gx = torch.empty_like(x)
         sums = torch.empty((2, C), device=x.device, dtype=torch.float32)
         dw = torch.empty_like(weight)
         db = torch.empty_like(bias)
-        _lib.check(L.amk_bnact_bwd(_ptr(gz), _ptr(x), _ptr(weight), _ptr(bias), _ptr(mean), _ptr(rstd), N, C, HW,
-                                   float(slope), _ptr(gx), _ptr(sums), _ptr(dw), _ptr(db), _ptr(_bn_ws(x)), _stream()),
-                   "amk_bnact_bwd")
+        _lib.check(_bn_fn("bwd", nhwc)(_ptr(gz), _ptr(x), _ptr(weight), _ptr(bias), _ptr(mean), _ptr(rstd), N, C, HW,
+                                       float(slope), _ptr(gx), _ptr(sums), _ptr(dw), _ptr(db), _ptr(_bn_ws(x, nhwc)),
+                                       _stream()), "amk_bnact_bwd")
         ctx.save_for_backward(gz, x, weight, bias, mean, rstd, sums)
         ctx.slope = slope
         ctx.set_materialize_grads(False)
@@ -1478,15 +1487,16 @@
         gz, x, weight, bias, mean, rstd, sums = ctx.saved_tensors
         if ggx is None and ggw is None and ggb is None:
             return None, None, None, None, None, None, None
-        ggx = torch.zeros_like(x) if ggx is None else _bn_aligned(ggx)
+        nhwc = _bn_nhwc(x)
+        ggx = torch.zeros_like(x) if ggx is None else _bn_aligned(ggx, nhwc)
         N, C, HW = _bn_dims(x)
         g_gz = torch.empty_like(x)
         g_x = torch.empty_like(x)
         g_w = torch.empty_like(weight) if ctx.needs_input_grad[2] else None
-        _lib.check(_lib.load().amk_bnact_bwd_bwd(
+        _lib.check(_bn_fn("bwd_bwd", nhwc)(
             _ptr(ggx), _ptr(ggw.contiguous() if ggw is not None else None), _ptr(ggb.contiguous() if ggb is not None else None),
             _ptr(gz), _ptr(x), _ptr(weight), _ptr(bias), _ptr(mean), _ptr(rstd), _ptr(sums), N, C, HW, float(ctx.slope),
-            _ptr(g_gz), _ptr(g_x), _ptr(g_w), _ptr(_bn_ws(x)), _stream()), "amk_bnact_bwd_bwd")
+            _ptr(g_gz), _ptr(g_x), _ptr(g_w), _ptr(_bn_ws(x, nhwc)), _stream()), "amk_bnact_bwd_bwd")
         return (g_gz if ctx.needs_input_grad[0] else None, g_x if ctx.needs_input_grad[1] else None, g_w,
                 None, None, None, None)
 
@@ -1495,14 +1505,14 @@
 
     @staticmethod
     def forward(ctx, x, weight, bias, running_mean, running_var, eps, momentum, slope):
+        nhwc = _bn_nhwc(x)
         N, C, HW = _bn_dims(x)
-        L = _lib.load()
         z = torch.empty_like(x)
         mean = torch.empty(C, device=x.device, dtype=torch.float32)
         rstd = torch.empty(C, device=x.device, dtype=torch.float32)
-        _lib.check(L.amk_bnact_fwd(_ptr(x), _ptr(weight), _ptr(bias), N, C, HW, float(eps), float(momentum), float(slope),
-                                   _ptr(z), _ptr(mean), _ptr(rstd), _ptr(running_mean), _ptr(running_var),
-                                   _ptr(_bn_ws(x)), _stream()), "amk_bnact_fwd")
+        _lib.check(_bn_fn("fwd", nhwc)(_ptr(x), _ptr(weight), _ptr(bias), N, C, HW, float(eps), float(momentum),
+                                       float(slope), _ptr(z), _ptr(mean), _ptr(rstd), _ptr(running_mean),
+                                       _ptr(running_var), _ptr(_bn_ws(x, nhwc)), _stream()), "amk_bnact_fwd")
         ctx.save_for_backward(x, weight, bias, mean, rstd)
         ctx.slope = slope
         ctx.set_materialize_grads(False)
@@ -1525,7 +1535,7 @@
 def bn_leaky_relu_ok(bn, x):
     return (bn.training and bn.track_running_stats and bn.affine and bn.momentum is not None
             and bn.running_mean is not None and x.is_cuda and x.dtype == torch.float32 and x.dim() == 4
-            and x.is_contiguous() and x.numel() > 0 and x.shape[0] * x.shape[2] * x.shape[3] > 1
+            and (x.is_contiguous() or _bn_nhwc(x)) and x.numel() > 0 and x.shape[0] * x.shape[2] * x.shape[3] > 1
             and not torch.is_autocast_enabled() and bn.weight.dtype == torch.float32)
 
 
@@ -1533,5 +1543,50 @@
     _require_device(x, bn.weight, bn.bias)
     if bn.num_batches_tracked is not None:
         bn.num_batches_tracked.add_(1)
-    return _BNAct.apply(_bn_aligned(x), bn.weight, bn.bias, bn.running_mean, bn.running_var, bn.eps, bn.momentum,
-                        float(slope))
+    return _BNAct.apply(_bn_aligned(x, _bn_nhwc(x)), bn.weight, bn.bias, bn.running_mean, bn.running_var, bn.eps,
+                        bn.momentum, float(slope))
+
+
+def conv_c1_ok(x_shape):
+    N, C, H, W = x_shape
+    return C % 4 == 0 and 0 < C <= 512 and H >= 2 and W >= 2 and 0 < N <= 65535
+
+
+def _c1_image(t):
+    t = t.contiguous(memory_format=torch.channels_last)
+    return t if t.data_ptr() % 16 == 0 else t.clone(memory_format=torch.preserve_format)
+
+
+def _c1_ws(N, H, W, C, like):
+    return torch.empty(int(_lib.load().amk_conv_c1_ws_floats(N, H, W, C)), device=like.device, dtype=torch.float32)
+
+
+def conv_c1_fwd(x, w_img, bias):
+    _require_device(x, w_img, bias)
+    N, C, H, W = x.shape
+    x, w_img = _c1_image(x), _c1_image(w_img)
+    y = torch.empty((N, 1, H - 1, W - 1), device=x.device, dtype=torch.float32)
+    _lib.check(_lib.load().amk_conv_c1_fwd(_ptr(x), _ptr(w_img), _ptr(bias), N, H, W, C, _ptr(y),
+                                           _ptr(_c1_ws(N, H, W, C, x)), _stream()), "amk_conv_c1_fwd")
+    return y
+
+
+def conv_c1_bwd_data(gy, w_img, x_shape):
+    _require_device(gy, w_img)
+    N, C, H, W = x_shape
+    gy, w_img = gy.contiguous(), _c1_image(w_img)
+    gx = torch.empty((N, C, H, W), device=gy.device, dtype=torch.float32, memory_format=torch.channels_last)
+    _lib.check(_lib.load().amk_conv_c1_bwd_data(_ptr(gy), _ptr(w_img), N, H, W, C, _ptr(gx), _stream()),
+               "amk_conv_c1_bwd_data")
+    return gx
+
+
+def conv_c1_wgrad(x, gy, with_bias):
+    _require_device(x, gy)
+    N, C, H, W = x.shape
+    x, gy = _c1_image(x), gy.contiguous()
+    gw = torch.empty((1, C, 4, 4), device=x.device, dtype=torch.float32)
+    gb = torch.empty(1, device=x.device, dtype=torch.float32) if with_bias else None
+    _lib.check(_lib.load().amk_conv_c1_wgrad(_ptr(x), _ptr(gy), N, H, W, C, _ptr(gw), _ptr(gb),
+                                             _ptr(_c1_ws(N, H, W, C, x)), _stream()), "amk_conv_c1_wgrad")
+    return gw, gb
diff --git a/attention-models_amd/amk/train.py b/attention-models_amd/amk/train.py
--- a/attention-models_amd/amk/train.py
+++ b/attention-models_amd/amk/train.py
@@ -4,7 +4,7 @@
 import torch.nn.functional as F
 
 from .dp import GradReducer
-from .models.discriminator import input_grad_only
+from .models.discriminator import input_grad_only, skip_leaf_input_grad
 from .optim import FlatAdam
 
 
@@ -403,7 +403,8 @@
             if rec is None:
                 rec, _ = model(img)
             d_loss = hinge_d_loss(discr(rec), discr(img)) + self.gradient_penalty(img, rec, eta)
-        (d_loss if accum_steps == 1 else d_loss / accum_steps).backward()
+        with skip_leaf_input_grad():
+            (d_loss if accum_steps == 1 else d_loss / accum_steps).backward()
         self.d_red.finish()
         if sync:
             self._optim_step(self.d_optim, self.d_red, discr)
diff --git a/attention-models_amd/csrc/discr_head.hip b/attention-models_amd/csrc/discr_head.hip
--- /dev/null
+++ b/attention-models_amd/csrc/discr_head.hip
@@ -0,0 +1,278 @@
+#include "amk_common.h"
+
+namespace amk_head {
+
+constexpr int BLOCK = 256;
+constexpr int WAVES = BLOCK / 64;
+constexpr int TAPS = 16;
+constexpr int CHUNK = 256;
+constexpr int MAX_C = 512;
+constexpr int PIX_T = 64;
+constexpr int PIX_B = 32;
+constexpr int CQ = 8;
+constexpr int RT = BLOCK / CQ;
+
+__device__ __forceinline__ float4 ld4(const float* p) { return *reinterpret_cast<const float4*>(p); }
+__device__ __forceinline__ void st4(float* p, float4 v) { *reinterpret_cast<float4*>(p) = v; }
+
+__device__ __forceinline__ void taps_of(const float* __restrict__ gy_n, int i, int j, int Ho, int Wo,
+                                        float (&g)[TAPS]) {
+#pragma unroll
+  for (int ky = 0; ky < 4; ++ky) {
+    const int oi = i + 1 - ky;
+#pragma unroll
+    for (int kx = 0; kx < 4; ++kx) {
+      const int oj = j + 1 - kx;
+      const bool ok = oi >= 0 && oi < Ho && oj >= 0 && oj < Wo;
+      g[ky * 4 + kx] = ok ? gy_n[oi * Wo + oj] : 0.f;
+    }
+  }
+}
+
+template <int M>
+__device__ __forceinline__ void scatter_step(float (&v)[TAPS], int lane, int o) {
+  const bool hi = (lane & o) != 0;
+#pragma unroll
+  for (int i = 0; i < M / 2; ++i) {
+    const float send = hi ? v[i] : v[i + M / 2];
+    const float keep = hi ? v[i + M / 2] : v[i];
+    v[i] = keep + __shfl_xor(send, o, 64);
+  }
+}
+
+__device__ __forceinline__ float tap_reduce(float (&v)[TAPS], int lane) {
+  scatter_step<16>(v, lane, 1);
+  scatter_step<8>(v, lane, 2);
+  scatter_step<4>(v, lane, 4);
+  scatter_step<2>(v, lane, 8);
+  float s = v[0];
+  s += __shfl_xor(s, 16, 64);
+  s += __shfl_xor(s, 32, 64);
+  return s;
+}
+
+__device__ __forceinline__ int tap_of_lane(int lane) {
+  return ((lane & 1) << 3) | ((lane & 2) << 1) | ((lane & 4) >> 1) | ((lane & 8) >> 3);
+}
+
+__global__ __launch_bounds__(BLOCK) void tap_image_kernel(const float* __restrict__ x, const float* __restrict__ w,
+                                                          int64_t P, int C, int chunks, float* __restrict__ T) {
+  extern __shared__ float4 wl[];
+  const int lane = threadIdx.x & 63, wave = threadIdx.x >> 6;
+  for (int idx = threadIdx.x; idx < chunks * TAPS * 64; idx += BLOCK) {
+    const int ch = idx / (TAPS * 64), t = (idx / 64) % TAPS, c = ch * CHUNK + (idx % 64) * 4;
+    wl[idx] = c < C ? ld4(w + (int64_t)t * C + c) : make_float4(0.f, 0.f, 0.f, 0.f);
+  }
+  __syncthreads();
+  const int64_t p0 = (int64_t)blockIdx.x * PIX_T + wave * (PIX_T / WAVES);
+  const int tap = tap_of_lane(lane);
+  for (int k = 0; k < PIX_T / WAVES; k += 2) {
+    const int64_t pa = p0 + k, pb = pa + 1;
+    if (pa >= P) break;
+    float a[TAPS], b[TAPS];
+#pragma unroll
+    for (int t = 0; t < TAPS; ++t) a[t] = b[t] = 0.f;
+    for (int ch = 0; ch < chunks; ++ch) {
+      const int c = ch * CHUNK + lane * 4;
+      const float4 zero = make_float4(0.f, 0.f, 0.f, 0.f);
+      const float4 xa = c < C ? ld4(x + pa * C + c) : zero;
+      const float4 xb = (c < C && pb < P) ? ld4(x + pb * C + c) : zero;
+#pragma unroll
+      for (int t = 0; t < TAPS; ++t) {
+        const float4 w4 = wl[(ch * TAPS + t) * 64 + lane];
+        a[t] = fmaf(xa.w, w4.w, fmaf(xa.z, w4.z, fmaf(xa.y, w4.y, fmaf(xa.x, w4.x, a[t]))));
+        b[t] = fmaf(xb.w, w4.w, fmaf(xb.z, w4.z, fmaf(xb.y, w4.y, fmaf(xb.x, w4.x, b[t]))));
+      }
+    }
+    const float ra = tap_reduce(a, lane), rb = tap_reduce(b, lane);
+    if (lane < TAPS) {
+      T[pa * TAPS + tap] = ra;
+      if (pb < P) T[pb * TAPS + tap] = rb;
+    }
+  }
+}
+
+__global__ __launch_bounds__(BLOCK) void head_gather_kernel(const float* __restrict__ T, const float* __restrict__ bias,
+                                                            int N, int H, int W, float* __restrict__ y) {
+  const int Ho = H - 1, Wo = W - 1;
+  const int64_t idx = (int64_t)blockIdx.x * BLOCK + threadIdx.x;
+  if (idx >= (int64_t)N * Ho * Wo) return;
+  const int n = (int)(idx / (Ho * Wo)), rem = (int)(idx % (Ho * Wo)), oi = rem / Wo, oj = rem % Wo;
+  float s = bias ? bias[0] : 0.f;
+#pragma unroll
+  for (int ky = 0; ky < 4; ++ky) {
+    const int i = oi - 1 + ky;
+#pragma unroll
+    for (int kx = 0; kx < 4; ++kx) {
+      const int j = oj - 1 + kx;
+      if (i >= 0 && i < H && j >= 0 && j < W) s += T[(((int64_t)n * H + i) * W + j) * TAPS + ky * 4 + kx];
+    }
+  }
+  y[idx] = s;
+}
+
+__global__ __launch_bounds__(BLOCK) void head_bwd_data_kernel(const float* __restrict__ gy, const float* __restrict__ w,
+                                                              int N, int H, int W, int C, float* __restrict__ gx) {
+  extern __shared__ float4 wl[];
+  const int cq = C / 4, Ho = H - 1, Wo = W - 1;
+  for (int idx = threadIdx.x; idx < TAPS * cq; idx += BLOCK) wl[idx] = ld4(w + (int64_t)idx * 4);
+  __syncthreads();
+  const int64_t P = (int64_t)N * H * W, p0 = (int64_t)blockIdx.x * PIX_B;
+  const int np = (int)min((int64_t)PIX_B, P - p0);
+  for (int idx = threadIdx.x; idx < np * cq; idx += BLOCK) {
+    const int64_t p = p0 + idx / cq;
+    const int q = idx % cq;
+    const int n = (int)(p / (H * W)), rem = (int)(p % (H * W));
+    float g[TAPS];
+    taps_of(gy + (int64_t)n * Ho * Wo, rem / W, rem % W, Ho, Wo, g);
+    float4 a = make_float4(0.f, 0.f, 0.f, 0.f);
+#pragma unroll
+    for (int t = 0; t < TAPS; ++t) {
+      const float4 w4 = wl[t * cq + q];
+      a.x = fmaf(g[t], w4.x, a.x);
+      a.y = fmaf(g[t], w4.y, a.y);
+      a.z = fmaf(g[t], w4.z, a.z);
+      a.w = fmaf(g[t], w4.w, a.w);
+    }
+    st4(gx + p * C + (int64_t)q * 4, a);
+  }
+}
+
+__global__ __launch_bounds__(BLOCK) void head_wgrad_partial_kernel(const float* __restrict__ x,
+                                                                   const float* __restrict__ gy, int H, int W, int C,
+                                                                   float* __restrict__ part) {
+  __shared__ float lds[WAVES * CQ * TAPS * 4];
+  const int n = blockIdx.x, q = threadIdx.x % CQ, r = threadIdx.x / CQ;
+  const int lane = threadIdx.x & 63, wave = threadIdx.x >> 6;
+  const int c0 = (blockIdx.y * CQ + q) * 4, Ho = H - 1, Wo = W - 1;
+  const bool on = c0 < C;
+  float acc[TAPS][4];
+#pragma unroll
+  for (int t = 0; t < TAPS; ++t)
+#pragma unroll
+    for (int j = 0; j < 4; ++j) acc[t][j] = 0.f;
+  if (on) {
+    const float* gy_n = gy + (int64_t)n * Ho * Wo;
+    const float* x_n = x + (int64_t)n * H * W * C + c0;
+    for (int pix = r; pix < H * W; pix += RT) {
+      float g[TAPS];
+      taps_of(gy_n, pix / W, pix % W, Ho, Wo, g);
+      const float4 xv = ld4(x_n + (int64_t)pix * C);
+#pragma unroll
+      for (int t = 0; t < TAPS; ++t) {
+        acc[t][0] = fmaf(g[t], xv.x, acc[t][0]);
+        acc[t][1] = fmaf(g[t], xv.y, acc[t][1]);
+        acc[t][2] = fmaf(g[t], xv.z, acc[t][2]);
+        acc[t][3] = fmaf(g[t], xv.w, acc[t][3]);
+      }
+    }
+  }
+#pragma unroll
+  for (int o = 32; o >= CQ; o >>= 1)
+#pragma unroll
+    for (int t = 0; t < TAPS; ++t)
+#pragma unroll
+      for (int j = 0; j < 4; ++j) acc[t][j] += __shfl_xor(acc[t][j], o, 64);
+  if (lane < CQ) {
+#pragma unroll
+    for (int t = 0; t < TAPS; ++t)
+#pragma unroll
+      for (int j = 0; j < 4; ++j) lds[((wave * CQ + q) * TAPS + t) * 4 + j] = acc[t][j];
+  }
+  __syncthreads();
+  for (int idx = threadIdx.x; idx < CQ * TAPS * 4; idx += BLOCK) {
+    float s = lds[idx];
+#pragma unroll
+    for (int wv = 1; wv < WAVES; ++wv) s += lds[wv * CQ * TAPS * 4 + idx];
+    const int qq = idx / (TAPS * 4), t = (idx / 4) % TAPS, c = (blockIdx.y * CQ + qq) * 4 + idx % 4;
+    if (c < C) part[((int64_t)n * TAPS + t) * C + c] = s;
+  }
+}
+
+__global__ __launch_bounds__(BLOCK) void head_wgrad_fold_kernel(const float* __restrict__ part,
+                                                                const float* __restrict__ gy, int N, int C, int64_t ngy,
+                                                                float* __restrict__ gw, float* __restrict__ gb) {
+  __shared__ float lds[WAVES];
+  if (blockIdx.x == gridDim.x - 1) {
+    if (!gb) return;
+    float v = 0.f;
+    for (int64_t i = threadIdx.x; i < ngy; i += BLOCK) v += gy[i];
+#pragma unroll
+    for (int o = 32; o >= 1; o >>= 1) v += __shfl_xor(v, o, 64);
+    if ((threadIdx.x & 63) == 0) lds[threadIdx.x >> 6] = v;
+    __syncthreads();
+    if (threadIdx.x == 0) {
+      float s = lds[0];
+#pragma unroll
+      for (int wv = 1; wv < WAVES; ++wv) s += lds[wv];
+      gb[0] = s;
+    }
+    return;
+  }
+  const int idx = blockIdx.x * BLOCK + threadIdx.x;
+  if (idx >= TAPS * C) return;
+  const int t = idx / C, c = idx % C;
+  float s = 0.f;
+  for (int n = 0; n < N; ++n) s += part[((int64_t)n * TAPS + t) * C + c];
+  gw[(int64_t)c * TAPS + t] = s;
+}
+
+}
+
+using namespace amk_head;
+
+static bool aligned16(const void* p) { return (reinterpret_cast<uintptr_t>(p) & 15) == 0; }
+
+#define AMK_HEAD_SHAPE(what)                                                                             \
+  AMK_CHECK_ARG(N > 0 && H > 0 && W > 0 && C > 0, what ": non-positive size");                           \
+  AMK_CHECK_SUPPORTED(H >= 2 && W >= 2 && C % 4 == 0 && C <= MAX_C && (int64_t)N * H * W * C < ((int64_t)1 << 40) \
+                          && (int64_t)N * H * W <= ((int64_t)1 << 30) && N <= 65535,                     \
+                      what ": shape N %d H %d W %d C %d not supported", N, H, W, C)
+
+extern "C" int64_t amk_conv_c1_ws_floats(int N, int H, int W, int C) {
+  if (N <= 0 || H <= 0 || W <= 0 || C <= 0) return 0;
+  const int64_t taps = (int64_t)N * H * W * TAPS, part = (int64_t)N * TAPS * C;
+  return taps > part ? taps : part;
+}
+
+extern "C" int amk_conv_c1_fwd(const float* x, const float* w, const float* bias, int N, int H, int W, int C, float* y,
+                               float* ws, void* stream) {
+  AMK_CHECK_ARG(x && w && y && ws, "amk_conv_c1_fwd: null pointer");
+  AMK_HEAD_SHAPE("amk_conv_c1_fwd");
+  AMK_CHECK_ARG(aligned16(x) && aligned16(w), "amk_conv_c1_fwd: x and w must be 16-byte aligned");
+  hipStream_t st = static_cast<hipStream_t>(stream);
+  const int64_t P = (int64_t)N * H * W, ny = (int64_t)N * (H - 1) * (W - 1);
+  const int chunks = (C + CHUNK - 1) / CHUNK;
+  hipLaunchKernelGGL(tap_image_kernel, dim3((unsigned)((P + PIX_T - 1) / PIX_T)), dim3(BLOCK),
+                     (size_t)chunks * TAPS * 64 * sizeof(float4), st, x, w, P, C, chunks, ws);
+  hipLaunchKernelGGL(head_gather_kernel, dim3((unsigned)((ny + BLOCK - 1) / BLOCK)), dim3(BLOCK), 0, st, ws, bias, N, H,
+                     W, y);
+  AMK_CHECK_LAUNCH("amk_conv_c1_fwd");
+  return AMK_OK;
+}
+
+extern "C" int amk_conv_c1_bwd_data(const float* gy, const float* w, int N, int H, int W, int C, float* gx,
+                                    void* stream) {
+  AMK_CHECK_ARG(gy && w && gx, "amk_conv_c1_bwd_data: null pointer");
+  AMK_HEAD_SHAPE("amk_conv_c1_bwd_data");
+  AMK_CHECK_ARG(aligned16(gx) && aligned16(w), "amk_conv_c1_bwd_data: gx and w must be 16-byte aligned");
+  hipStream_t st = static_cast<hipStream_t>(stream);
+  const int64_t P = (int64_t)N * H * W;
+  hipLaunchKernelGGL(head_bwd_data_kernel, dim3((unsigned)((P + PIX_B - 1) / PIX_B)), dim3(BLOCK),
+                     (size_t)TAPS * C * sizeof(float), st, gy, w, N, H, W, C, gx);
+  AMK_CHECK_LAUNCH("amk_conv_c1_bwd_data");
+  return AMK_OK;
+}
+
+extern "C" int amk_conv_c1_wgrad(const float* x, const float* gy, int N, int H, int W, int C, float* gw, float* gb,
+                                 float* ws, void* stream) {
+  AMK_CHECK_ARG(x && gy && gw && ws, "amk_conv_c1_wgrad: null pointer");
+  AMK_HEAD_SHAPE("amk_conv_c1_wgrad");
+  AMK_CHECK_ARG(aligned16(x), "amk_conv_c1_wgrad: x must be 16-byte aligned");
+  hipStream_t st = static_cast<hipStream_t>(stream);
+  hipLaunchKernelGGL(head_wgrad_partial_kernel, dim3(N, (C / 4 + CQ - 1) / CQ), dim3(BLOCK), 0, st, x, gy, H, W, C, ws);
+  hipLaunchKernelGGL(head_wgrad_fold_kernel, dim3((TAPS * C + BLOCK - 1) / BLOCK + 1), dim3(BLOCK), 0, st, ws, gy, N, C,
+                     (int64_t)N * (H - 1) * (W - 1), gw, gb);
+  AMK_CHECK_LAUNCH("amk_conv_c1_wgrad");
+  return AMK_OK;
+}
diff --git a/attention-models_amd/csrc/discr_norm.hip b/attention-models_amd/csrc/discr_norm.hip
--- a/attention-models_amd/csrc/discr_norm.hip
+++ b/attention-models_amd/csrc/discr_norm.hip
@@ -353,6 +353,371 @@
   });
 }
 
+constexpr int CQ = 8;
+constexpr int RT = BLOCK / CQ;
+constexpr int MAX_S = 128;
+constexpr int MIN_RS = 256;
+
+struct GeoL {
+  int64_t R;
+  int C;
+  int RS;
+  int S;
+};
+
+static GeoL make_geo_l(int N, int C, int64_t HW) {
+  GeoL g;
+  g.R = (int64_t)N * HW;
+  g.C = C;
+  int64_t rs = (g.R + MAX_S - 1) / MAX_S;
+  if (rs < MIN_RS) rs = MIN_RS;
+  rs = (rs + RT - 1) / RT * RT;
+  g.RS = (int)rs;
+  g.S = (int)((g.R + rs - 1) / rs);
+  return g;
+}
+
+__device__ __forceinline__ float seg_rows(const GeoL& g, int s) {
+  const int64_t r0 = (int64_t)s * g.RS;
+  return (float)(min(g.R, r0 + g.RS) - r0);
+}
+
+struct Lane {
+  int r, c0;
+  bool on;
+};
+
+__device__ __forceinline__ Lane lane_of(const GeoL& g) {
+  Lane l;
+  l.r = threadIdx.x / CQ;
+  l.c0 = (blockIdx.y * CQ + threadIdx.x % CQ) * 4;
+  l.on = l.c0 < g.C;
+  return l;
+}
+
+template <class F>
+__device__ __forceinline__ void rows_walk(const GeoL& g, const Lane& l, int s, F&& f) {
+  if (!l.on) return;
+  const int64_t r0 = (int64_t)s * g.RS, r1 = min(g.R, r0 + g.RS);
+#pragma unroll 4
+  for (int64_t row = r0 + l.r; row < r1; row += RT) f(row * g.C + l.c0);
+}
+
+template <int K, class Op>
+__device__ __forceinline__ void rows_reduce(float (&v)[K][4], Op op, float* lds) {
+  const int lane = threadIdx.x & 63, wave = threadIdx.x >> 6, q = threadIdx.x % CQ;
+#pragma unroll
+  for (int o = 32; o >= CQ; o >>= 1) {
+#pragma unroll
+    for (int j = 0; j < 4; ++j) {
+      float a[K], b[K];
+#pragma unroll
+      for (int k = 0; k < K; ++k) { a[k] = v[k][j]; b[k] = __shfl_xor(v[k][j], o, 64); }
+      op(a, b);
+#pragma unroll
+      for (int k = 0; k < K; ++k) v[k][j] = a[k];
+    }
+  }
+  if (lane < CQ) {
+#pragma unroll
+    for (int k = 0; k < K; ++k)
+#pragma unroll
+      for (int j = 0; j < 4; ++j) lds[((wave * CQ + q) * K + k) * 4 + j] = v[k][j];
+  }
+  __syncthreads();
+#pragma unroll
+  for (int j = 0; j < 4; ++j) {
+    float a[K], b[K];
+#pragma unroll
+    for (int k = 0; k < K; ++k) a[k] = lds[(q * K + k) * 4 + j];
+#pragma unroll
+    for (int w = 1; w < WAVES; ++w) {
+#pragma unroll
+      for (int k = 0; k < K; ++k) b[k] = lds[((w * CQ + q) * K + k) * 4 + j];
+      op(a, b);
+    }
+#pragma unroll
+    for (int k = 0; k < K; ++k) v[k][j] = a[k];
+  }
+  __syncthreads();
+}
+
+template <int K>
+__device__ __forceinline__ void put_part(float* __restrict__ part, const GeoL& g, const Lane& l, int s,
+                                         const float (&v)[K][4]) {
+  if (l.r != 0 || !l.on) return;
+#pragma unroll
+  for (int k = 0; k < K; ++k) st<4>(part + ((int64_t)k * g.S + s) * g.C + l.c0, v[k]);
+}
+
+template <int K>
+__device__ __forceinline__ void fold_sums_l(const float* __restrict__ part, const GeoL& g, const Lane& l,
+                                            float (&v)[K][4], float* lds) {
+#pragma unroll
+  for (int k = 0; k < K; ++k)
+#pragma unroll
+    for (int j = 0; j < 4; ++j) v[k][j] = 0.f;
+  if (l.on) {
+    for (int s = l.r; s < g.S; s += RT) {
+#pragma unroll
+      for (int k = 0; k < K; ++k) {
+        float p[4];
+        ld<4>(part + ((int64_t)k * g.S + s) * g.C + l.c0, p);
+#pragma unroll
+        for (int j = 0; j < 4; ++j) v[k][j] += p[j];
+      }
+    }
+  }
+  rows_reduce<K>(v, Sum{}, lds);
+}
+
+constexpr int LDS_L = WAVES * CQ * 3 * 4;
+
+__global__ __launch_bounds__(BLOCK) void stats_nhwc_kernel(const float* __restrict__ x, GeoL g,
+                                                           float* __restrict__ part) {
+  __shared__ float lds[LDS_L];
+  const int s = blockIdx.x;
+  const Lane l = lane_of(g);
+  float v[1][4] = {{0.f, 0.f, 0.f, 0.f}};
+  rows_walk(g, l, s, [&](int64_t off) {
+    float xv[4];
+    ld<4>(x + off, xv);
+#pragma unroll
+    for (int j = 0; j < 4; ++j) v[0][j] += xv[j];
+  });
+  rows_reduce<1>(v, Sum{}, lds);
+  const float cnt = seg_rows(g, s);
+  float pm[2][4];
+#pragma unroll
+  for (int j = 0; j < 4; ++j) pm[0][j] = v[0][j] / cnt;
+  float q[1][4] = {{0.f, 0.f, 0.f, 0.f}};
+  rows_walk(g, l, s, [&](int64_t off) {
+    float xv[4];
+    ld<4>(x + off, xv);
+#pragma unroll
+    for (int j = 0; j < 4; ++j) { const float d = xv[j] - pm[0][j]; q[0][j] += d * d; }
+  });
+  rows_reduce<1>(q, Sum{}, lds);
+#pragma unroll
+  for (int j = 0; j < 4; ++j) pm[1][j] = q[0][j];
+  put_part<2>(part, g, l, s, pm);
+}
+
+__global__ __launch_bounds__(BLOCK) void fwd_apply_nhwc_kernel(
+    const float* __restrict__ x, const float* __restrict__ gamma, const float* __restrict__ beta, GeoL g,
+    const float* __restrict__ part, float eps, float momentum, float slope, float* __restrict__ z,
+    float* __restrict__ mean_out, float* __restrict__ rstd_out, float* __restrict__ run_mean,
+    float* __restrict__ run_var) {
+  __shared__ float lds[LDS_L];
+  const int s = blockIdx.x;
+  const Lane l = lane_of(g);
+  float a[3][4];
+#pragma unroll
+  for (int k = 0; k < 3; ++k)
+#pragma unroll
+    for (int j = 0; j < 4; ++j) a[k][j] = 0.f;
+  if (l.on) {
+    for (int t = l.r; t < g.S; t += RT) {
+      float m[4], m2[4];
+      ld<4>(part + (int64_t)t * g.C + l.c0, m);
+      ld<4>(part + ((int64_t)g.S + t) * g.C + l.c0, m2);
+      const float cnt = seg_rows(g, t);
+#pragma unroll
+      for (int j = 0; j < 4; ++j) {
+        float u[3] = {a[0][j], a[1][j], a[2][j]};
+        const float b[3] = {cnt, m[j], m2[j]};
+        Chan{}(u, b);
+        a[0][j] = u[0]; a[1][j] = u[1]; a[2][j] = u[2];
+      }
+    }
+  }
+  rows_reduce<3>(a, Chan{}, lds);
+  float scale[4] = {0.f, 0.f, 0.f, 0.f}, shift[4] = {0.f, 0.f, 0.f, 0.f};
+  if (l.on) {
+#pragma unroll
+    for (int j = 0; j < 4; ++j) {
+      const int c = l.c0 + j;
+      const float n = a[0][j], mu = a[1][j], var = a[2][j] / n;
+      const float r = rsqrtf(var + eps);
+      scale[j] = gamma[c] * r;
+      shift[j] = beta[c] - mu * scale[j];
+      if (s == 0 && l.r == 0) {
+        mean_out[c] = mu;
+        rstd_out[c] = r;
+        if (run_mean) run_mean[c] = (1.f - momentum) * run_mean[c] + momentum * mu;
+        if (run_var) run_var[c] = (1.f - momentum) * run_var[c] + momentum * (a[2][j] / (n - 1.f));
+      }
+    }
+  }
+  rows_walk(g, l, s, [&](int64_t off) {
+    float xv[4];
+    ld<4>(x + off, xv);
+#pragma unroll
+    for (int j = 0; j < 4; ++j) {
+      const float y = fmaf(xv[j], scale[j], shift[j]);
+      xv[j] = y > 0.f ? y : slope * y;
+    }
+    st<4>(z + off, xv);
+  });
+}
+
+struct Chn4 {
+  float mu[4], r[4], scale[4], shift[4];
+};
+
+__device__ __forceinline__ Chn4 chn4(const float* gamma, const float* beta, const float* mean, const float* rstd,
+                                     const Lane& l) {
+  Chn4 h;
+#pragma unroll
+  for (int j = 0; j < 4; ++j) {
+    const Chn t = l.on ? chn(gamma, beta, mean, rstd, l.c0 + j) : Chn{0.f, 0.f, 0.f, 0.f};
+    h.mu[j] = t.mu; h.r[j] = t.r; h.scale[j] = t.scale; h.shift[j] = t.shift;
+  }
+  return h;
+}
+
+__global__ __launch_bounds__(BLOCK) void bwd_reduce_nhwc_kernel(
+    const float* __restrict__ gz, const float* __restrict__ x, const float* __restrict__ gamma,
+    const float* __restrict__ beta, const float* __restrict__ mean, const float* __restrict__ rstd, GeoL g,
+    float slope, float* __restrict__ part) {
+  __shared__ float lds[LDS_L];
+  const int s = blockIdx.x;
+  const Lane l = lane_of(g);
+  const Chn4 h = chn4(gamma, beta, mean, rstd, l);
+  float v[2][4] = {{0.f, 0.f, 0.f, 0.f}, {0.f, 0.f, 0.f, 0.f}};
+  rows_walk(g, l, s, [&](int64_t off) {
+    float xv[4], gv[4];
+    ld<4>(x + off, xv);
+    ld<4>(gz + off, gv);
+#pragma unroll
+    for (int j = 0; j < 4; ++j) {
+      const float gy = fmaf(xv[j], h.scale[j], h.shift[j]) > 0.f ? gv[j] : slope * gv[j];
+      v[0][j] += gy;
+      v[1][j] += gy * ((xv[j] - h.mu[j]) * h.r[j]);
+    }
+  });
+  rows_reduce<2>(v, Sum{}, lds);
+  put_part<2>(part, g, l, s, v);
+}
+
+__global__ __launch_bounds__(BLOCK) void bwd_apply_nhwc_kernel(
+    const float* __restrict__ gz, const float* __restrict__ x, const float* __restrict__ gamma,
+    const float* __restrict__ beta, const float* __restrict__ mean, const float* __restrict__ rstd, GeoL g,
+    float slope, const float* __restrict__ part, float* __restrict__ gx, float* __restrict__ sums,
+    float* __restrict__ dgamma, float* __restrict__ dbeta) {
+  __shared__ float lds[LDS_L];
+  const int s = blockIdx.x;
+  const Lane l = lane_of(g);
+  const Chn4 h = chn4(gamma, beta, mean, rstd, l);
+  float v[2][4];
+  fold_sums_l<2>(part, g, l, v, lds);
+  if (s == 0 && l.r == 0 && l.on) {
+#pragma unroll
+    for (int j = 0; j < 4; ++j) {
+      const int c = l.c0 + j;
+      sums[c] = v[0][j];
+      sums[g.C + c] = v[1][j];
+      if (dbeta) dbeta[c] = v[0][j];
+      if (dgamma) dgamma[c] = v[1][j];
+    }
+  }
+  const float inv_n = 1.f / (float)g.R;
+  float A[4], B[4];
+#pragma unroll
+  for (int j = 0; j < 4; ++j) { A[j] = v[0][j] * inv_n; B[j] = v[1][j] * inv_n; }
+  rows_walk(g, l, s, [&](int64_t off) {
+    float xv[4], gv[4];
+    ld<4>(x + off, xv);
+    ld<4>(gz + off, gv);
+#pragma unroll
+    for (int j = 0; j < 4; ++j) {
+      const float gy = fmaf(xv[j], h.scale[j], h.shift[j]) > 0.f ? gv[j] : slope * gv[j];
+      const float xh = (xv[j] - h.mu[j]) * h.r[j];
+      xv[j] = h.scale[j] * (gy - A[j] - xh * B[j]);
+    }
+    st<4>(gx + off, xv);
+  });
+}
+
+__global__ __launch_bounds__(BLOCK) void bwd_bwd_reduce_nhwc_kernel(
+    const float* __restrict__ ggx, const float* __restrict__ gz, const float* __restrict__ x,
+    const float* __restrict__ gamma, const float* __restrict__ beta, const float* __restrict__ mean,
+    const float* __restrict__ rstd, GeoL g, float slope, float* __restrict__ part) {
+  __shared__ float lds[LDS_L];
+  const int s = blockIdx.x;
+  const Lane l = lane_of(g);
+  const Chn4 h = chn4(gamma, beta, mean, rstd, l);
+  float v[3][4];
+#pragma unroll
+  for (int k = 0; k < 3; ++k)
+#pragma unroll
+    for (int j = 0; j < 4; ++j) v[k][j] = 0.f;
+  rows_walk(g, l, s, [&](int64_t off) {
+    float xv[4], gv[4], qv[4];
+    ld<4>(x + off, xv);
+    ld<4>(gz + off, gv);
+    ld<4>(ggx + off, qv);
+#pragma unroll
+    for (int j = 0; j < 4; ++j) {
+      const float gy = fmaf(xv[j], h.scale[j], h.shift[j]) > 0.f ? gv[j] : slope * gv[j];
+      v[0][j] += qv[j];
+      v[1][j] += qv[j] * ((xv[j] - h.mu[j]) * h.r[j]);
+      v[2][j] += qv[j] * gy;
+    }
+  });
+  rows_reduce<3>(v, Sum{}, lds);
+  put_part<3>(part, g, l, s, v);
+}
+
+__global__ __launch_bounds__(BLOCK) void bwd_bwd_apply_nhwc_kernel(
+    const float* __restrict__ ggx, const float* __restrict__ gg_gamma, const float* __restrict__ gg_beta,
+    const float* __restrict__ gz, const float* __restrict__ x, const float* __restrict__ gamma,
+    const float* __restrict__ beta, const float* __restrict__ mean, const float* __restrict__ rstd,
+    const float* __restrict__ sums, GeoL g, float slope, const float* __restrict__ part, float* __restrict__ g_gz,
+    float* __restrict__ g_x, float* __restrict__ g_gamma) {
+  __shared__ float lds[LDS_L];
+  const int s = blockIdx.x;
+  const Lane l = lane_of(g);
+  const Chn4 h = chn4(gamma, beta, mean, rstd, l);
+  float v[3][4];
+  fold_sums_l<3>(part, g, l, v, lds);
+  const float n = (float)g.R, inv_n = 1.f / n;
+  float A[4], B[4], Cc[4], D[4], ggg[4], ggb[4], k1[4], gr2[4], gr[4];
+#pragma unroll
+  for (int j = 0; j < 4; ++j) {
+    const int c = l.c0 + j;
+    A[j] = l.on ? sums[c] * inv_n : 0.f;
+    B[j] = l.on ? sums[g.C + c] * inv_n : 0.f;
+    Cc[j] = v[0][j] * inv_n;
+    D[j] = v[1][j] * inv_n;
+    const float E = v[2][j] * inv_n;
+    ggg[j] = gg_gamma && l.on ? gg_gamma[c] : 0.f;
+    ggb[j] = gg_beta && l.on ? gg_beta[c] : 0.f;
+    if (s == 0 && l.r == 0 && l.on && g_gamma) g_gamma[c] = n * h.r[j] * (E - A[j] * Cc[j] - B[j] * D[j]);
+    k1[j] = E - A[j] * Cc[j] - 3.f * B[j] * D[j];
+    gr2[j] = h.scale[j] * h.r[j];
+    gr[j] = ggg[j] * h.r[j];
+  }
+  rows_walk(g, l, s, [&](int64_t off) {
+    float xv[4], gv[4], qv[4];
+    ld<4>(x + off, xv);
+    ld<4>(gz + off, gv);
+    ld<4>(ggx + off, qv);
+#pragma unroll
+    for (int j = 0; j < 4; ++j) {
+      const bool pos = fmaf(xv[j], h.scale[j], h.shift[j]) > 0.f;
+      const float gy = pos ? gv[j] : slope * gv[j];
+      const float xh = (xv[j] - h.mu[j]) * h.r[j];
+      const float q = qv[j] - Cc[j];
+      const float t = h.scale[j] * (q - xh * D[j]) + ggg[j] * xh + ggb[j];
+      gv[j] = pos ? t : slope * t;
+      xv[j] = gr[j] * (gy - A[j] - xh * B[j]) - gr2[j] * (xh * k1[j] + B[j] * q + D[j] * (gy - A[j]));
+    }
+    st<4>(g_gz + off, gv);
+    st<4>(g_x + off, xv);
+  });
+}
+
 }
 
 using namespace amk_bn;
@@ -420,3 +785,66 @@
   AMK_CHECK_LAUNCH("amk_bnact_bwd_bwd");
   return AMK_OK;
 }
+
+#define AMK_BN_SHAPE_L(what)                                                                     \
+  AMK_BN_SHAPE(what);                                                                            \
+  AMK_CHECK_SUPPORTED(C % 4 == 0, what ": C %d is not a multiple of 4", C)
+
+static dim3 grid_l(const GeoL& g) { return dim3(g.S, (g.C / 4 + CQ - 1) / CQ); }
+
+extern "C" int64_t amk_bnact_nhwc_ws_floats(int N, int C, int64_t HW) {
+  if (N <= 0 || C <= 0 || HW <= 0) return 0;
+  return (int64_t)C * make_geo_l(N, C, HW).S * 3;
+}
+
+extern "C" int amk_bnact_nhwc_fwd(const float* x, const float* gamma, const float* beta, int N, int C, int64_t HW,
+                                  float eps, float momentum, float slope, float* z, float* mean, float* rstd,
+                                  float* running_mean, float* running_var, float* ws, void* stream) {
+  AMK_CHECK_ARG(x && gamma && beta && z && mean && rstd && ws, "amk_bnact_nhwc_fwd: null pointer");
+  AMK_BN_SHAPE_L("amk_bnact_nhwc_fwd");
+  AMK_CHECK_ARG(N * HW > 1, "amk_bnact_nhwc_fwd: a channel needs more than one value");
+  AMK_CHECK_ARG(a16(x) && a16(z) && a16(ws), "amk_bnact_nhwc_fwd: x, z and ws must be 16-byte aligned");
+  hipStream_t st = static_cast<hipStream_t>(stream);
+  const GeoL g = make_geo_l(N, C, HW);
+  const dim3 grid = grid_l(g), block(BLOCK);
+  hipLaunchKernelGGL(stats_nhwc_kernel, grid, block, 0, st, x, g, ws);
+  hipLaunchKernelGGL(fwd_apply_nhwc_kernel, grid, block, 0, st, x, gamma, beta, g, ws, eps, momentum, slope, z, mean,
+                     rstd, running_mean, running_var);
+  AMK_CHECK_LAUNCH("amk_bnact_nhwc_fwd");
+  return AMK_OK;
+}
+
+extern "C" int amk_bnact_nhwc_bwd(const float* gz, const float* x, const float* gamma, const float* beta,
+                                  const float* mean, const float* rstd, int N, int C, int64_t HW, float slope,
+                                  float* gx, float* sums, float* dgamma, float* dbeta, float* ws, void* stream) {
+  AMK_CHECK_ARG(gz && x && gamma && beta && mean && rstd && gx && sums && ws, "amk_bnact_nhwc_bwd: null pointer");
+  AMK_BN_SHAPE_L("amk_bnact_nhwc_bwd");
+  AMK_CHECK_ARG(a16(gz) && a16(x) && a16(gx) && a16(ws), "amk_bnact_nhwc_bwd: gz, x, gx and ws must be 16-byte aligned");
+  hipStream_t st = static_cast<hipStream_t>(stream);
+  const GeoL g = make_geo_l(N, C, HW);
+  const dim3 grid = grid_l(g), block(BLOCK);
+  hipLaunchKernelGGL(bwd_reduce_nhwc_kernel, grid, block, 0, st, gz, x, gamma, beta, mean, rstd, g, slope, ws);
+  hipLaunchKernelGGL(bwd_apply_nhwc_kernel, grid, block, 0, st, gz, x, gamma, beta, mean, rstd, g, slope, ws, gx, sums,
+                     dgamma, dbeta);
+  AMK_CHECK_LAUNCH("amk_bnact_nhwc_bwd");
+  return AMK_OK;
+}
+
+extern "C" int amk_bnact_nhwc_bwd_bwd(const float* ggx, const float* gg_gamma, const float* gg_beta, const float* gz,
+                                      const float* x, const float* gamma, const float* beta, const float* mean,
+                                      const float* rstd, const float* sums, int N, int C, int64_t HW, float slope,
+                                      float* g_gz, float* g_x, float* g_gamma, float* ws, void* stream) {
+  AMK_CHECK_ARG(ggx && gz && x && gamma && beta && mean && rstd && sums && g_gz && g_x && ws,
+                "amk_bnact_nhwc_bwd_bwd: null pointer");
+  AMK_BN_SHAPE_L("amk_bnact_nhwc_bwd_bwd");
+  AMK_CHECK_ARG(a16(ggx) && a16(gz) && a16(x) && a16(g_gz) && a16(g_x) && a16(ws),
+                "amk_bnact_nhwc_bwd_bwd: ggx, gz, x, g_gz, g_x and ws must be 16-byte aligned");
+  hipStream_t st = static_cast<hipStream_t>(stream);
+  const GeoL g = make_geo_l(N, C, HW);
+  const dim3 grid = grid_l(g), block(BLOCK);
+  hipLaunchKernelGGL(bwd_bwd_reduce_nhwc_kernel, grid, block, 0, st, ggx, gz, x, gamma, beta, mean, rstd, g, slope, ws);
+  hipLaunchKernelGGL(bwd_bwd_apply_nhwc_kernel, grid, block, 0, st, ggx, gg_gamma, gg_beta, gz, x, gamma, beta, mean,
+                     rstd, sums, g, slope, ws, g_gz, g_x, g_gamma);
+  AMK_CHECK_LAUNCH("amk_bnact_nhwc_bwd_bwd");
+  return AMK_OK;
+}
diff --git a/include/amk.h b/include/amk.h
--- a/include/amk.h
+++ b/include/amk.h
@@ -281,6 +281,25 @@
                       int N, int C, int64_t HW, float slope, float* g_gz, float* g_x, float* g_gamma, float* ws,
                       void* stream);
 
+int64_t amk_bnact_nhwc_ws_floats(int N, int C, int64_t HW);
+int amk_bnact_nhwc_fwd(const float* x, const float* gamma, const float* beta, int N, int C, int64_t HW, float eps,
+                       float momentum, float slope, float* z, float* mean, float* rstd, float* running_mean,
+                       float* running_var, float* ws, void* stream);
+int amk_bnact_nhwc_bwd(const float* gz, const float* x, const float* gamma, const float* beta, const float* mean,
+                       const float* rstd, int N, int C, int64_t HW, float slope, float* gx, float* sums, float* dgamma,
+                       float* dbeta, float* ws, void* stream);
+int amk_bnact_nhwc_bwd_bwd(const float* ggx, const float* gg_gamma, const float* gg_beta, const float* gz,
+                           const float* x, const float* gamma, const float* beta, const float* mean, const float* rstd,
+                           const float* sums, int N, int C, int64_t HW, float slope, float* g_gz, float* g_x,
+                           float* g_gamma, float* ws, void* stream);
+
+int64_t amk_conv_c1_ws_floats(int N, int H, int W, int C);
+int amk_conv_c1_fwd(const float* x, const float* w, const float* bias, int N, int H, int W, int C, float* y, float* ws,
+                    void* stream);
+int amk_conv_c1_bwd_data(const float* gy, const float* w, int N, int H, int W, int C, float* gx, void* stream);
+int amk_conv_c1_wgrad(const float* x, const float* gy, int N, int H, int W, int C, float* gw, float* gb, float* ws,
+                      void* stream);
+
 #ifdef __cplusplus
 }
 #endif
```

Measured after the change: 308.3 images/s, median of 6. About the same (+0.4%).
